# mKaloer/TFServingCache

Measured on NVIDIA H100. Metric: predict_qps, higher is better.
Workload: dtype f32

## Files before the change

### tfservingcache_b200/csrc/dense_tc.cu

```cuda
#include <cuda.h>
#include <cuda_runtime.h>

#include <atomic>
#include <cstdlib>
#include <mutex>
#include <unordered_map>

#include "kernels.h"
#include "tc_ptx.cuh"

namespace tfsc {

extern std::atomic<int64_t> g_launches_tc;
std::atomic<int64_t> g_launches_tc{0};

namespace tc {
constexpr int BK = 32;
constexpr int WG_COLS = 64;
constexpr int CONS_WG = 4;
constexpr int STRIP = WG_COLS * CONS_WG;
constexpr int SLABS = STRIP / 32;
constexpr int W_BYTES = SLABS * BK * 128;
constexpr int CONSUMERS = CONS_WG * 128;
constexpr int CONS_WARPS = CONSUMERS / 32;
constexpr int THREADS = CONSUMERS + 32;
}

template <int RP>
struct TcSmem {
  static constexpr int NS = 6;
  static constexpr int B_BYTES = 2 * RP * 128;
  static constexpr int W_TOTAL = NS * tc::W_BYTES;
  static constexpr int TOTAL = W_TOTAL + 2 * B_BYTES + 256 + 1024;
};

template <int RP>
__global__ void __launch_bounds__(tc::THREADS, 1)
dense_tc_kernel(const __grid_constant__ CUtensorMap wmap, const float* __restrict__ x, const float* __restrict__ bias,
                float* __restrict__ y, int rows, int K, int N, int relu, int splits, int chunk_k,
                unsigned int* __restrict__ counters, float* __restrict__ partials) {
  using S = TcSmem<RP>;
  constexpr int NS = S::NS;
  extern __shared__ __align__(1024) uint8_t smem_raw[];
  uint8_t* smem = reinterpret_cast<uint8_t*>((reinterpret_cast<uintptr_t>(smem_raw) + 1023) & ~(uintptr_t)1023);
  uint8_t* bprime = smem + S::W_TOTAL;
  uint64_t* bars = reinterpret_cast<uint64_t*>(bprime + 2 * S::B_BYTES);
  uint64_t* full = bars;
  uint64_t* empty = bars + NS;

  const int warp = threadIdx.x >> 5, lane = threadIdx.x & 31;
  const int wg = __shfl_sync(0xffffffffu, (int)(threadIdx.x >> 7), 0);
  const int strip = blockIdx.x, split = blockIdx.y;
  const int k_begin = split * chunk_k;
  const int k_end = min(K, k_begin + chunk_k);
  const int n_kblocks = (max(0, k_end - k_begin) + tc::BK - 1) / tc::BK;

  if (threadIdx.x == 0) {
    for (int s = 0; s < NS; ++s) {
      mbar_init(&full[s], 1);
      mbar_init(&empty[s], tc::CONS_WARPS);
    }
    asm volatile("fence.mbarrier_init.release.cluster;" ::: "memory");
    asm volatile("prefetch.tensormap [%0];" ::"l"(&wmap) : "memory");
  }
  __syncthreads();
  asm volatile("griddepcontrol.launch_dependents;" ::: "memory");

  if (wg == tc::CONS_WG) {
    for (int kb = 0; kb < n_kblocks; ++kb) {
      const int s = kb % NS, it = kb / NS;
      if (lane == 0) {
        if (it > 0) mbar_wait(&empty[s], (it - 1) & 1);
        mbar_expect_tx(&full[s], tc::W_BYTES);
#pragma unroll
        for (int g = 0; g < tc::BK / 4; ++g)
          tma_load_3d(smem + s * tc::W_BYTES + g * 4096, &wmap, &full[s], 0, k_begin + kb * tc::BK + g * 4, strip * tc::SLABS);
      }
      __syncwarp();
    }
  } else {
    const int ct = threadIdx.x;
    const int wq = warp & 3, g = lane >> 2, t = lane & 3;
    constexpr int XI = (RP * 8 + tc::CONSUMERS - 1) / tc::CONSUMERS;
    float4 xr[2][XI];
    auto load_x = [&](int kb, float4* dst) {
      const int k0 = k_begin + kb * tc::BK;
#pragma unroll
      for (int j = 0; j < XI; ++j) {
        const int idx = ct + j * tc::CONSUMERS;
        const int r = idx >> 3, c = idx & 7;
        float4 v = make_float4(0.f, 0.f, 0.f, 0.f);
        const int kk = k0 + c * 4;
        if (idx < RP * 8 && r < rows) {
          const float* src = x + (size_t)r * K + kk;
          if (kk + 3 < k_end) v = __ldg(reinterpret_cast<const float4*>(src));
          else {
            if (kk < k_end) v.x = __ldg(src);
            if (kk + 1 < k_end) v.y = __ldg(src + 1);
            if (kk + 2 < k_end) v.z = __ldg(src + 2);
          }
        }
        dst[j] = v;
      }
    };
    asm volatile("griddepcontrol.wait;" ::: "memory");
    if (n_kblocks > 0) load_x(0, xr[0]);
    if (n_kblocks > 1) load_x(1, xr[1]);
    const int n0 = wg * tc::WG_COLS + wq * 16 + g, slab = n0 >> 5, row = slab * 4 + t;
    auto w_off = [&](int n) { return (uint32_t)(row * 128 + ((((n & 31) >> 2) ^ (row & 7)) << 4) + (n & 3) * 4); };
    const uint32_t w_base = smem_u32(smem);
    const uint32_t off0 = w_off(n0), off1 = w_off(n0 + 8);
    const uint32_t bp_base = smem_u32(bprime);
    float acc_h[RP / 2], acc_s[RP / 2];
#pragma unroll
    for (int i = 0; i < RP / 2; ++i) acc_h[i] = acc_s[i] = 0.f;
    auto body = [&](int kb, float4* xcur) {
      const int s = kb % NS, it = kb / NS, cb = kb & 1;
      const uint32_t bp = bp_base + cb * S::B_BYTES;
#pragma unroll
      for (int j = 0; j < XI; ++j) {
        const int idx = ct + j * tc::CONSUMERS;
        if (idx < RP * 8) {
          const int r = idx >> 3, c = idx & 7, rl = r + RP;
          const float4 v = xcur[j];
          sts_f4(bp + (uint32_t)(((r >> 3) * 64 + (r & 7) * 8 + (c ^ (r & 7))) * 16), v);
          sts_f4(bp + (uint32_t)(((rl >> 3) * 64 + (rl & 7) * 8 + (c ^ (rl & 7))) * 16),
                 make_float4(tf32_lo(v.x), tf32_lo(v.y), tf32_lo(v.z), tf32_lo(v.w)));
        }
      }
      if (kb + 2 < n_kblocks) load_x(kb + 2, xcur);
      asm volatile("fence.proxy.async.shared::cta;" ::: "memory");
      named_bar_sync(1, tc::CONSUMERS);
      mbar_wait(&full[s], it & 1);
      const uint32_t wst = w_base + (uint32_t)(s * tc::W_BYTES);
      uint32_t hi[tc::BK / 8][4], lo[tc::BK / 8][4];
#pragma unroll
      for (int k8 = 0; k8 < tc::BK / 8; ++k8)
#pragma unroll
        for (int j = 0; j < 4; ++j) {
          const float v = lds_f32(wst + (uint32_t)((k8 * 2 + (j >> 1)) * 4096) + ((j & 1) ? off1 : off0));
          hi[k8][j] = tf32_hi_bits(v);
          lo[k8][j] = __float_as_uint(tf32_lo(v));
        }
      __syncwarp();
      if (lane == 0) mbar_arrive(&empty[s]);
      if constexpr (RP <= 32) {
        fence_regs(hi);
        fence_regs(lo);
      }
      fence_regs(acc_h);
      fence_regs(acc_s);
      wgmma_fence();
#pragma unroll
      for (int k8 = 0; k8 < tc::BK / 8; ++k8) {
        const uint64_t bh = gmma_desc_sw128(bp + k8 * 32), bl = gmma_desc_sw128(bp + RP * 128 + k8 * 32);
        wgmma_tf32_rs<RP>(acc_h, hi[k8], bh);
        wgmma_tf32_rs<RP>(acc_s, hi[k8], bl);
        wgmma_tf32_rs<RP>(acc_s, lo[k8], bh);
      }
      wgmma_commit();
      wgmma_wait_all();
      fence_regs(acc_h);
      fence_regs(acc_s);
    };
    for (int kb = 0; kb < n_kblocks; kb += 2) {
      body(kb, xr[0]);
      if (kb + 1 < n_kblocks) body(kb + 1, xr[1]);
    }
    float* my_partial = partials + ((size_t)(strip * splits + split) * RP) * tc::STRIP;
#pragma unroll
    for (int i = 0; i < RP / 2; ++i) {
      const int ncol = n0 + 8 * ((i >> 1) & 1), r = 8 * (i >> 2) + 2 * t + (i & 1);
      my_partial[(size_t)r * tc::STRIP + ncol] = acc_h[i] + acc_s[i];
    }
  }

  __shared__ unsigned int s_last;
  asm volatile("griddepcontrol.wait;" ::: "memory");
  __threadfence();
  __syncthreads();
  if (threadIdx.x == 0) {
    const unsigned int prev = atomicAdd(&counters[strip], 1u);
    s_last = (prev == (unsigned)splits - 1) ? 1u : 0u;
    if (s_last) counters[strip] = 0u;
  }
  __syncthreads();
  if (!s_last) return;
  __threadfence();
  const float* sp = partials + (size_t)strip * splits * RP * tc::STRIP;
  for (int idx = threadIdx.x; idx < rows * (tc::STRIP / 4); idx += tc::THREADS) {
    const int r = idx / (tc::STRIP / 4), c4 = idx - r * (tc::STRIP / 4);
    const int col = strip * tc::STRIP + c4 * 4;
    if (col >= N) continue;
    float4 acc = __ldcg(reinterpret_cast<const float4*>(sp + (size_t)r * tc::STRIP) + c4);
    for (int s2 = 1; s2 < splits; ++s2) {
      const float4 v = __ldcg(reinterpret_cast<const float4*>(sp + ((size_t)s2 * RP + r) * tc::STRIP) + c4);
      acc.x += v.x; acc.y += v.y; acc.z += v.z; acc.w += v.w;
    }
    const float4 bv = __ldg(reinterpret_cast<const float4*>(bias + col));
    acc.x += bv.x; acc.y += bv.y; acc.z += bv.z; acc.w += bv.w;
    if (relu) { acc.x = fmaxf(acc.x, 0.f); acc.y = fmaxf(acc.y, 0.f); acc.z = fmaxf(acc.z, 0.f); acc.w = fmaxf(acc.w, 0.f); }
    *reinterpret_cast<float4*>(y + (size_t)r * N + col) = acc;
  }
}

EncodeTiledFn tc_encode_fn() {
  static EncodeTiledFn fn = [] {
    void* p = nullptr;
    cudaDriverEntryPointQueryResult q;
    if (cudaGetDriverEntryPoint("cuTensorMapEncodeTiled", &p, cudaEnableDefault, &q) != cudaSuccess) p = nullptr;
    return reinterpret_cast<EncodeTiledFn>(p);
  }();
  return fn;
}

struct MapKey {
  const void* w;
  int k, n;
  bool operator==(const MapKey& o) const { return w == o.w && k == o.k && n == o.n; }
};
struct MapKeyHash {
  size_t operator()(const MapKey& m) const { return std::hash<const void*>()(m.w) ^ ((size_t)m.k * 1315423911u) ^ ((size_t)m.n << 20); }
};

static bool get_wmap(const float* w, int k, int n, CUtensorMap* out) {
  static std::mutex mu;
  static std::unordered_map<MapKey, CUtensorMap, MapKeyHash> cache;
  std::lock_guard<std::mutex> lk(mu);
  auto it = cache.find({w, k, n});
  if (it != cache.end()) {
    *out = it->second;
    return true;
  }
  EncodeTiledFn enc = tc_encode_fn();
  if (!enc) return false;
  CUtensorMap m;
  const cuuint64_t gdim[3] = {32, (cuuint64_t)k, (cuuint64_t)(n / 32)};
  const cuuint64_t gstride[2] = {(cuuint64_t)n * 4, 128};
  const cuuint32_t box[3] = {32, 4, (cuuint32_t)tc::SLABS};
  const cuuint32_t estr[3] = {1, 1, 1};
  CUresult r = enc(&m, CU_TENSOR_MAP_DATA_TYPE_FLOAT32, 3, const_cast<float*>(w), gdim, gstride, box, estr,
                   CU_TENSOR_MAP_INTERLEAVE_NONE, CU_TENSOR_MAP_SWIZZLE_128B, CU_TENSOR_MAP_L2_PROMOTION_L2_256B,
                   CU_TENSOR_MAP_FLOAT_OOB_FILL_NONE);
  if (r != CUDA_SUCCESS) return false;
  if (cache.size() > 4096) cache.clear();
  cache[{w, k, n}] = m;
  *out = m;
  return true;
}

struct TcPlan {
  int strips, splits, chunk_k;
};
static TcPlan plan_tc(int k, int n) {
  TcPlan p;
  p.strips = (n + tc::STRIP - 1) / tc::STRIP;
  int splits = device_sm_count() / p.strips;
  if (splits < 1) splits = 1;
  int max_splits = (k + 4 * tc::BK - 1) / (4 * tc::BK);
  if (splits > max_splits) splits = max_splits;
  if (splits < 1) splits = 1;
  int chunk = (k + splits - 1) / splits;
  chunk = (chunk + tc::BK - 1) / tc::BK * tc::BK;
  p.chunk_k = chunk;
  p.splits = (k + chunk - 1) / chunk;
  return p;
}

bool dense_tc_supported(int rows, int k, int n, const float* w, const float* x, const float* bias, const float* y) {
  return rows >= 1 && rows <= 64 && n % 32 == 0 && k % 4 == 0 && k >= 32 &&
         ((reinterpret_cast<uintptr_t>(w) & 15) == 0) && ((reinterpret_cast<uintptr_t>(x) & 15) == 0) &&
         ((reinterpret_cast<uintptr_t>(bias) & 15) == 0) && ((reinterpret_cast<uintptr_t>(y) & 15) == 0) && tc_encode_fn() != nullptr;
}

size_t dense_tc_workspace_bytes(int k, int n) {
  TcPlan p = plan_tc(k, n);
  size_t counters = ((size_t)p.strips * sizeof(unsigned int) + 255) & ~(size_t)255;
  return counters + (size_t)p.strips * p.splits * 64 * tc::STRIP * sizeof(float);
}

template <int RP>
static cudaError_t launch_tc_rp(const CUtensorMap& map, const float* x, const float* bias, float* y, int rows, int k, int n,
                                bool relu, void* workspace, const TcPlan& p, cudaStream_t s) {
  static bool attr[64] = {};
  int dev = 0;
  cudaGetDevice(&dev);
  if (!attr[dev & 63]) {
    cudaError_t e = cudaFuncSetAttribute(dense_tc_kernel<RP>, cudaFuncAttributeMaxDynamicSharedMemorySize, TcSmem<RP>::TOTAL);
    if (e != cudaSuccess) return e;
    attr[dev & 63] = true;
  }
  unsigned int* counters = static_cast<unsigned int*>(workspace);
  size_t coff = ((size_t)p.strips * sizeof(unsigned int) + 255) & ~(size_t)255;
  float* partials = reinterpret_cast<float*>(static_cast<char*>(workspace) + coff);
  static const bool pdl = [] {
    const char* e = getenv("TFSC_PDL");
    return !e || atoi(e) != 0;
  }();
  cudaLaunchConfig_t cfg = {};
  cfg.gridDim = dim3(p.strips, p.splits);
  cfg.blockDim = dim3(tc::THREADS);
  cfg.dynamicSmemBytes = TcSmem<RP>::TOTAL;
  cfg.stream = s;
  cudaLaunchAttribute at[1];
  at[0].id = cudaLaunchAttributeProgrammaticStreamSerialization;
  at[0].val.programmaticStreamSerializationAllowed = 1;
  cfg.attrs = at;
  cfg.numAttrs = pdl ? 1 : 0;
  cudaError_t e = cudaLaunchKernelEx(&cfg, dense_tc_kernel<RP>, map, x, bias, y, rows, k, n, relu ? 1 : 0, p.splits, p.chunk_k, counters,
                                     partials);
  g_launches_tc++;
  return e != cudaSuccess ? e : cudaGetLastError();
}

cudaError_t launch_dense_tc(const float* x, const float* w, const float* bias, float* y, int rows, int k, int n, bool relu,
                            void* workspace, size_t workspace_bytes, cudaStream_t s) {
  if (workspace_bytes < dense_tc_workspace_bytes(k, n)) return cudaErrorInvalidValue;
  CUtensorMap map;
  if (!get_wmap(w, k, n, &map)) return cudaErrorNotSupported;
  const TcPlan p = plan_tc(k, n);
  if (rows <= 16) return launch_tc_rp<16>(map, x, bias, y, rows, k, n, relu, workspace, p, s);
  if (rows <= 32) return launch_tc_rp<32>(map, x, bias, y, rows, k, n, relu, workspace, p, s);
  if (rows <= 48) return launch_tc_rp<48>(map, x, bias, y, rows, k, n, relu, workspace, p, s);
  return launch_tc_rp<64>(map, x, bias, y, rows, k, n, relu, workspace, p, s);
}

}
```

### tfservingcache_b200/csrc/kernels.cu

```cuda
#include "kernels.h"
#include "tc_ptx.cuh"

#include <atomic>
#include <cstdlib>

namespace tfsc {

static std::atomic<int64_t> g_launches{0};
extern std::atomic<int64_t> g_launches_tc;
extern std::atomic<int64_t> g_launches_nn;
extern std::atomic<int64_t> g_launches_cl;
int64_t kernel_launch_count() { return g_launches.load() + g_launches_tc.load() + g_launches_nn.load() + g_launches_cl.load(); }

int device_sm_count() {
  static std::atomic<int> cache[64] = {};
  int dev = 0;
  cudaGetDevice(&dev);
  int n = cache[dev & 63].load();
  if (n <= 0) {
    if (cudaDeviceGetAttribute(&n, cudaDevAttrMultiProcessorCount, dev) != cudaSuccess || n <= 0) n = 132;
    cache[dev & 63].store(n);
  }
  return n;
}

__global__ void __launch_bounds__(256) affine_kernel(const float* __restrict__ x, float* __restrict__ y, int64_t n,
                                                     const float* __restrict__ pa, const float* __restrict__ pb) {
  const float a = __ldg(pa), b = __ldg(pb);
  int64_t i = (int64_t)blockIdx.x * blockDim.x + threadIdx.x;
  const int64_t stride = (int64_t)gridDim.x * blockDim.x;
  const int64_t n4 = n >> 2;
  const bool vec = ((reinterpret_cast<uintptr_t>(x) | reinterpret_cast<uintptr_t>(y)) & 15) == 0;
  if (vec) {
    const float4* x4 = reinterpret_cast<const float4*>(x);
    float4* y4 = reinterpret_cast<float4*>(y);
    for (int64_t j = i; j < n4; j += stride) {
      float4 v = __ldg(x4 + j);
      v.x = fmaf(a, v.x, b); v.y = fmaf(a, v.y, b); v.z = fmaf(a, v.z, b); v.w = fmaf(a, v.w, b);
      y4[j] = v;
    }
    for (int64_t j = (n4 << 2) + i; j < n; j += stride) y[j] = fmaf(a, x[j], b);
  } else {
    for (int64_t j = i; j < n; j += stride) y[j] = fmaf(a, x[j], b);
  }
}

cudaError_t launch_affine(const float* x, float* y, int64_t n, const float* a, const float* b, cudaStream_t s) {
  if (n <= 0) return cudaSuccess;
  int64_t blocks = (n / 4 + 255) / 256;
  if (blocks < 1) blocks = 1;
  if (blocks > device_sm_count() * 8) blocks = device_sm_count() * 8;
  affine_kernel<<<(unsigned)blocks, 256, 0, s>>>(x, y, n, a, b);
  g_launches++;
  return cudaGetLastError();
}

constexpr int kThreads = 512;
constexpr int kColsPerThread = 8;
constexpr int kColGroups = 64;
constexpr int kStripCols = kColGroups * kColsPerThread;
constexpr int kKLanes = kThreads / kColGroups;
constexpr int kUnroll = 4;
constexpr int kMaxChunkK = 4096;

struct __align__(32) float8 { float v[8]; };

__device__ __forceinline__ float8 ld_stream(const float8* p) {
  float8 r;
  uint64_t pol;
  asm("createpolicy.fractional.L2::evict_first.b64 %0, 1.0;" : "=l"(pol));
  asm volatile("ld.global.nc.L1::no_allocate.L2::cache_hint.v4.f32 {%0,%1,%2,%3}, [%4], %5;"
               : "=f"(r.v[0]), "=f"(r.v[1]), "=f"(r.v[2]), "=f"(r.v[3])
               : "l"(p), "l"(pol));
  asm volatile("ld.global.nc.L1::no_allocate.L2::cache_hint.v4.f32 {%0,%1,%2,%3}, [%4+16], %5;"
               : "=f"(r.v[4]), "=f"(r.v[5]), "=f"(r.v[6]), "=f"(r.v[7])
               : "l"(p), "l"(pol));
  return r;
}

__device__ __forceinline__ void pdl_trigger() { asm volatile("griddepcontrol.launch_dependents;" ::: "memory"); }
__device__ __forceinline__ void pdl_wait() { asm volatile("griddepcontrol.wait;" ::: "memory"); }

template <int R, bool PDL = false>
__global__ void __launch_bounds__(kThreads, 1)
dense_stream_kernel(const float* __restrict__ x, const float* __restrict__ w, const float* __restrict__ bias,
                    float* __restrict__ y, int rows, int K, int N, int relu, int splits, int chunk_k,
                    unsigned int* __restrict__ counters, float* __restrict__ partials) {
  extern __shared__ __align__(32) float smem[];
  float* xs = smem;

  const int strip = blockIdx.x;
  const int split = blockIdx.y;
  const int tid = threadIdx.x;
  const int cg = tid % kColGroups;
  const int kl = tid / kColGroups;
  const int col0 = strip * kStripCols + cg * kColsPerThread;
  const bool col_ok = col0 < N;
  const int k_begin = split * chunk_k;
  const int k_end = min(K, k_begin + chunk_k);
  const int kc = max(0, k_end - k_begin);

  if (PDL) {
    pdl_trigger();
    pdl_wait();
  }
  for (int idx = tid; idx < kc * R; idx += kThreads) {
    const int r = idx / kc, k = idx - r * kc;
    xs[k * R + r] = (r < rows) ? __ldg(x + (size_t)r * K + k_begin + k) : 0.f;
  }
  __syncthreads();

  float acc[R][kColsPerThread];
#pragma unroll
  for (int r = 0; r < R; ++r)
#pragma unroll
    for (int c = 0; c < kColsPerThread; ++c) acc[r][c] = 0.f;

  if (col_ok) {
    const float8* wp = reinterpret_cast<const float8*>(w + (size_t)(k_begin + kl) * N + col0);
    const size_t row_stride8 = (size_t)N / 8 * kKLanes;
    int k = kl;
    for (; k + (kUnroll - 1) * kKLanes < kc; k += kUnroll * kKLanes) {
      float8 wv[kUnroll];
#pragma unroll
      for (int u = 0; u < kUnroll; ++u) wv[u] = ld_stream(wp + (size_t)u * row_stride8);
      wp += (size_t)kUnroll * row_stride8;
#pragma unroll
      for (int u = 0; u < kUnroll; ++u) {
        const float* xr = xs + (k + u * kKLanes) * R;
        float xv[R];
        if (R % 4 == 0) {
#pragma unroll
          for (int q = 0; q < R / 4; ++q) {
            const float4 t = *reinterpret_cast<const float4*>(xr + 4 * q);
            xv[4 * q + 0] = t.x; xv[4 * q + 1] = t.y; xv[4 * q + 2] = t.z; xv[4 * q + 3] = t.w;
          }
        } else if (R == 2) {
          const float2 t = *reinterpret_cast<const float2*>(xr);
          xv[0] = t.x; xv[1] = t.y;
        } else {
#pragma unroll
          for (int r = 0; r < R; ++r) xv[r] = xr[r];
        }
#pragma unroll
        for (int r = 0; r < R; ++r)
#pragma unroll
          for (int c = 0; c < kColsPerThread; ++c) acc[r][c] = fmaf(xv[r], wv[u].v[c], acc[r][c]);
      }
    }
    for (; k < kc; k += kKLanes) {
      const float8 wv = ld_stream(wp);
      wp += row_stride8;
      const float* xr = xs + k * R;
#pragma unroll
      for (int r = 0; r < R; ++r) {
        const float xv = xr[r];
#pragma unroll
        for (int c = 0; c < kColsPerThread; ++c) acc[r][c] = fmaf(xv, wv.v[c], acc[r][c]);
      }
    }
  }

  __syncthreads();
  float* red = smem;
#pragma unroll
  for (int r = 0; r < R; ++r) {
    float4* dst = reinterpret_cast<float4*>(red + ((size_t)(kl * R + r) * kStripCols) + cg * kColsPerThread);
    dst[0] = make_float4(acc[r][0], acc[r][1], acc[r][2], acc[r][3]);
    dst[1] = make_float4(acc[r][4], acc[r][5], acc[r][6], acc[r][7]);
  }
  __syncthreads();

  constexpr int kVecPerRow = kStripCols / 4;
  const float4* red4 = reinterpret_cast<const float4*>(red);
  float4* my_partial = reinterpret_cast<float4*>(partials + ((size_t)(strip * splits + split) * R) * kStripCols);
  for (int idx = tid; idx < R * kVecPerRow; idx += kThreads) {
    const int r = idx / kVecPerRow, c = idx - r * kVecPerRow;
    float4 s = red4[(size_t)(0 * R + r) * kVecPerRow + c];
#pragma unroll
    for (int l = 1; l < kKLanes; ++l) {
      const float4 t = red4[(size_t)(l * R + r) * kVecPerRow + c];
      s.x += t.x; s.y += t.y; s.z += t.z; s.w += t.w;
    }
    if (splits == 1) {
      const int col = strip * kStripCols + c * 4;
      if (r < rows && col < N) {
        const float4 bv = __ldg(reinterpret_cast<const float4*>(bias + col));
        s.x += bv.x; s.y += bv.y; s.z += bv.z; s.w += bv.w;
        if (relu) { s.x = fmaxf(s.x, 0.f); s.y = fmaxf(s.y, 0.f); s.z = fmaxf(s.z, 0.f); s.w = fmaxf(s.w, 0.f); }
        *reinterpret_cast<float4*>(y + (size_t)r * N + col) = s;
      }
    } else {
      my_partial[r * kVecPerRow + c] = s;
    }
  }
  if (splits == 1) return;

  __shared__ unsigned int s_last;
  __threadfence();
  __syncthreads();
  if (tid == 0) {
    const unsigned int prev = atomicAdd(&counters[strip], 1u);
    s_last = (prev == (unsigned)splits - 1) ? 1u : 0u;
    if (s_last) counters[strip] = 0u;
  }
  __syncthreads();
  if (!s_last) return;
  __threadfence();
  const float4* strip_partials = reinterpret_cast<const float4*>(partials + (size_t)strip * splits * R * kStripCols);
  for (int idx = tid; idx < R * kVecPerRow; idx += kThreads) {
    const int r = idx / kVecPerRow, c = idx - r * kVecPerRow;
    const int col = strip * kStripCols + c * 4;
    if (r >= rows || col >= N) continue;
    float4 s = __ldcg(strip_partials + (size_t)(0 * R + r) * kVecPerRow + c);
    for (int sp = 1; sp < splits; ++sp) {
      const float4 t = __ldcg(strip_partials + (size_t)(sp * R + r) * kVecPerRow + c);
      s.x += t.x; s.y += t.y; s.z += t.z; s.w += t.w;
    }
    const float4 bv = __ldg(reinterpret_cast<const float4*>(bias + col));
    s.x += bv.x; s.y += bv.y; s.z += bv.z; s.w += bv.w;
    if (relu) { s.x = fmaxf(s.x, 0.f); s.y = fmaxf(s.y, 0.f); s.z = fmaxf(s.z, 0.f); s.w = fmaxf(s.w, 0.f); }
    *reinterpret_cast<float4*>(y + (size_t)r * N + col) = s;
  }
}

constexpr int kBulkStageRows = 16;
constexpr int kBulkStages = 5;
constexpr int kBulkColGroups = kStripCols / 8;
constexpr int kBulkRingFloats = kBulkStages * kBulkStageRows * kStripCols;
constexpr size_t kBulkMaxSmem = 216 * 1024;

__device__ __forceinline__ void bulk_copy_g2s(void* dst, const void* src, uint32_t bytes, uint64_t* bar, uint64_t policy) {
  asm volatile(
      "cp.async.bulk.shared::cluster.global.mbarrier::complete_tx::bytes.L2::cache_hint [%0], [%1], %2, [%3], %4;" ::"r"(
          smem_u32(dst)),
      "l"(src), "r"(bytes), "r"(smem_u32(bar)), "l"(policy)
      : "memory");
}
__device__ __forceinline__ void lds_2x64(uint32_t saddr, uint64_t& lo, uint64_t& hi) {
  asm volatile("ld.shared.v2.b64 {%0,%1}, [%2];" : "=l"(lo), "=l"(hi) : "r"(saddr));
}
__device__ __forceinline__ void ffma2(uint64_t& acc, float xs, uint64_t w2) {
  float a0, a1, w0, w1;
  asm("mov.b64 {%0, %1}, %2;" : "=f"(a0), "=f"(a1) : "l"(acc));
  asm("mov.b64 {%0, %1}, %2;" : "=f"(w0), "=f"(w1) : "l"(w2));
  asm("mov.b64 %0, {%1, %2};" : "=l"(acc) : "f"(fmaf(xs, w0, a0)), "f"(fmaf(xs, w1, a1)));
}

template <int R>
__device__ __forceinline__ void bulk_row(uint64_t (&acc)[R][4], uint32_t wrow_saddr, const float* xr) {
  uint64_t w0, w1, w2, w3;
  lds_2x64(wrow_saddr, w0, w1);
  lds_2x64(wrow_saddr + (kStripCols / 2) * 4u, w2, w3);
  float xv[R];
  if (R % 4 == 0) {
#pragma unroll
    for (int q = 0; q < R / 4; ++q) {
      const float4 t = *reinterpret_cast<const float4*>(xr + 4 * q);
      xv[4 * q + 0] = t.x; xv[4 * q + 1] = t.y; xv[4 * q + 2] = t.z; xv[4 * q + 3] = t.w;
    }
  } else if (R == 2) {
    const float2 t = *reinterpret_cast<const float2*>(xr);
    xv[0] = t.x; xv[1] = t.y;
  } else {
#pragma unroll
    for (int r = 0; r < R; ++r) xv[r] = xr[r];
  }
#pragma unroll
  for (int r = 0; r < R; ++r) {
    ffma2(acc[r][0], xv[r], w0);
    ffma2(acc[r][1], xv[r], w1);
    ffma2(acc[r][2], xv[r], w2);
    ffma2(acc[r][3], xv[r], w3);
  }
}

template <int R, int KL>
__global__ void __launch_bounds__(kBulkColGroups * KL + 32, 1)
dense_bulk_kernel(const float* __restrict__ x, const float* __restrict__ w, const float* __restrict__ bias,
                  float* __restrict__ y, int rows, int K, int N, int relu, int splits, int chunk_k,
                  unsigned int* __restrict__ counters, float* __restrict__ partials) {
  constexpr int kBulkKLanes = KL, kBulkConsumers = kBulkColGroups * KL, kBulkThreads = kBulkConsumers + 32;
  extern __shared__ __align__(128) float smem_bulk[];
  float* smem = smem_bulk;
  float* ring = smem;
  float* xs = smem + kBulkRingFloats;
  __shared__ __align__(8) uint64_t full[kBulkStages];
  __shared__ __align__(8) uint64_t empty[kBulkStages];
  __shared__ unsigned int s_last;

  const int strip = blockIdx.x;
  const int split = blockIdx.y;
  const int tid = threadIdx.x;
  const int warp = tid >> 5, lane = tid & 31;
  const int k_begin = split * chunk_k;
  const int k_end = min(K, k_begin + chunk_k);
  const int kc = max(0, k_end - k_begin);
  const int strip_cols = min(kStripCols, N - strip * kStripCols);
  const int n_stage = (kc + kBulkStageRows - 1) / kBulkStageRows;

  if (tid == 0) {
#pragma unroll
    for (int s = 0; s < kBulkStages; ++s) {
      mbar_init(&full[s], 1);
      mbar_init(&empty[s], kBulkConsumers / 32);
    }
    asm volatile("fence.mbarrier_init.release.cluster;" ::: "memory");
  }
  __syncthreads();
  pdl_trigger();

  uint64_t acc[R][4];
#pragma unroll
  for (int r = 0; r < R; ++r)
#pragma unroll
    for (int c = 0; c < 4; ++c) acc[r][c] = 0ull;
  const int cg = tid % kBulkColGroups;
  const int kl = (tid / kBulkColGroups) % kBulkKLanes;

  if (warp == kBulkConsumers / 32) {
    uint64_t policy;
    asm volatile("createpolicy.fractional.L2::evict_first.b64 %0, 1.0;" : "=l"(policy));
    const uint32_t row_bytes = (uint32_t)strip_cols * 4u;
    const float* src0 = w + (size_t)k_begin * N + (size_t)strip * kStripCols;
    for (int it = 0; it < n_stage; ++it) {
      const int s = it % kBulkStages;
      if (it >= kBulkStages) mbar_wait(&empty[s], ((it / kBulkStages) - 1) & 1);
      const int rows_here = min(kBulkStageRows, kc - it * kBulkStageRows);
      if (lane == 0) mbar_expect_tx(&full[s], (uint32_t)rows_here * row_bytes);
      __syncwarp();
      if (lane < rows_here)
        bulk_copy_g2s(ring + ((size_t)s * kBulkStageRows + lane) * kStripCols,
                      src0 + (size_t)(it * kBulkStageRows + lane) * N, row_bytes, &full[s], policy);
    }
    pdl_wait();
  } else {
    pdl_wait();
    for (int idx = tid; idx < kc * R; idx += kBulkConsumers) {
      const int r = idx / kc, k = idx - r * kc;
      xs[k * R + r] = (r < rows) ? __ldg(x + (size_t)r * K + k_begin + k) : 0.f;
    }
    asm volatile("bar.sync 1, %0;" ::"r"(kBulkConsumers) : "memory");
    const uint32_t ring_s = smem_u32(ring) + (uint32_t)cg * 16u;
    for (int it = 0; it < n_stage; ++it) {
      const int s = it % kBulkStages;
      mbar_wait(&full[s], (it / kBulkStages) & 1);
      const int kk0 = it * kBulkStageRows + kl;
      const uint32_t base = ring_s + (uint32_t)((s * kBulkStageRows + kl) * kStripCols) * 4u;
      if (it * kBulkStageRows + kBulkStageRows <= kc) {
#pragma unroll
        for (int j = 0; j < kBulkStageRows / KL; ++j)
          bulk_row<R>(acc, base + (uint32_t)(j * KL * kStripCols) * 4u, xs + (size_t)(kk0 + j * KL) * R);
      } else {
#pragma unroll
        for (int j = 0; j < kBulkStageRows / KL; ++j)
          if (kk0 + j * KL < kc) bulk_row<R>(acc, base + (uint32_t)(j * KL * kStripCols) * 4u, xs + (size_t)(kk0 + j * KL) * R);
      }
      __syncwarp();
      if (lane == 0) mbar_arrive(&empty[s]);
    }
  }

  __syncthreads();
  float* red = smem;
  if (warp < kBulkConsumers / 32) {
#pragma unroll
    for (int r = 0; r < R; ++r) {
      float* dst = red + ((size_t)(kl * R + r) * kStripCols) + cg * 4;
      *reinterpret_cast<ulonglong2*>(dst) = make_ulonglong2(acc[r][0], acc[r][1]);
      *reinterpret_cast<ulonglong2*>(dst + kStripCols / 2) = make_ulonglong2(acc[r][2], acc[r][3]);
    }
  }
  __syncthreads();

  constexpr int kVecPerRow = kStripCols / 4;
  const float4* red4 = reinterpret_cast<const float4*>(red);
  float4* my_partial = reinterpret_cast<float4*>(partials + ((size_t)(strip * splits + split) * R) * kStripCols);
  for (int idx = tid; idx < R * kVecPerRow; idx += kBulkThreads) {
    const int r = idx / kVecPerRow, c = idx - r * kVecPerRow;
    float4 s = red4[(size_t)(0 * R + r) * kVecPerRow + c];
#pragma unroll
    for (int l = 1; l < kBulkKLanes; ++l) {
      const float4 t = red4[(size_t)(l * R + r) * kVecPerRow + c];
      s.x += t.x; s.y += t.y; s.z += t.z; s.w += t.w;
    }
    if (splits == 1) {
      const int col = strip * kStripCols + c * 4;
      if (r < rows && col < N) {
        const float4 bv = __ldg(reinterpret_cast<const float4*>(bias + col));
        s.x += bv.x; s.y += bv.y; s.z += bv.z; s.w += bv.w;
        if (relu) { s.x = fmaxf(s.x, 0.f); s.y = fmaxf(s.y, 0.f); s.z = fmaxf(s.z, 0.f); s.w = fmaxf(s.w, 0.f); }
        *reinterpret_cast<float4*>(y + (size_t)r * N + col) = s;
      }
    } else {
      my_partial[r * kVecPerRow + c] = s;
    }
  }
  if (splits == 1) return;

  __threadfence();
  __syncthreads();
  if (tid == 0) {
    const unsigned int prev = atomicAdd(&counters[strip], 1u);
    s_last = (prev == (unsigned)splits - 1) ? 1u : 0u;
    if (s_last) counters[strip] = 0u;
  }
  __syncthreads();
  if (!s_last) return;
  __threadfence();
  const float4* strip_partials = reinterpret_cast<const float4*>(partials + (size_t)strip * splits * R * kStripCols);
  for (int idx = tid; idx < R * kVecPerRow; idx += kBulkThreads) {
    const int r = idx / kVecPerRow, c = idx - r * kVecPerRow;
    const int col = strip * kStripCols + c * 4;
    if (r >= rows || col >= N) continue;
    float4 s = __ldcg(strip_partials + (size_t)(0 * R + r) * kVecPerRow + c);
#pragma unroll 8
    for (int sp = 1; sp < splits; ++sp) {
      const float4 t = __ldcg(strip_partials + (size_t)(sp * R + r) * kVecPerRow + c);
      s.x += t.x; s.y += t.y; s.z += t.z; s.w += t.w;
    }
    const float4 bv = __ldg(reinterpret_cast<const float4*>(bias + col));
    s.x += bv.x; s.y += bv.y; s.z += bv.z; s.w += bv.w;
    if (relu) { s.x = fmaxf(s.x, 0.f); s.y = fmaxf(s.y, 0.f); s.z = fmaxf(s.z, 0.f); s.w = fmaxf(s.w, 0.f); }
    *reinterpret_cast<float4*>(y + (size_t)r * N + col) = s;
  }
}

__global__ void __launch_bounds__(256)
dense_generic_kernel(const float* __restrict__ x, const float* __restrict__ w, const float* __restrict__ bias,
                     float* __restrict__ y, int rows, int K, int N, int relu) {
  const int n = blockIdx.x * blockDim.x + threadIdx.x;
  const int r = blockIdx.y;
  if (n >= N || r >= rows) return;
  float acc = 0.f;
  const float* xr = x + (size_t)r * K;
  for (int k = 0; k < K; ++k) acc = fmaf(__ldg(xr + k), __ldg(w + (size_t)k * N + n), acc);
  acc += __ldg(bias + n);
  if (relu) acc = fmaxf(acc, 0.f);
  y[(size_t)r * N + n] = acc;
}

struct DensePlan {
  int strips, splits, chunk_k;
};

static DensePlan plan_dense(int k, int n) {
  DensePlan p;
  p.strips = (n + kStripCols - 1) / kStripCols;
  int splits = device_sm_count() / p.strips;
  if (splits < 1) splits = 1;
  int min_splits = (k + kMaxChunkK - 1) / kMaxChunkK;
  if (splits < min_splits) splits = min_splits;
  if (splits > k / 64 && k >= 64) splits = k / 64;
  if (splits < 1) splits = 1;
  int chunk = (k + splits - 1) / splits;
  chunk = (chunk + kKLanes - 1) / kKLanes * kKLanes;
  p.chunk_k = chunk;
  p.splits = (k + chunk - 1) / chunk;
  return p;
}

static size_t stream_workspace_bytes(int k, int n) {
  DensePlan p = plan_dense(k, n);
  size_t counters = ((size_t)p.strips * sizeof(unsigned int) + 255) & ~(size_t)255;
  size_t partials = (size_t)p.strips * p.splits * kMaxRowsPerLaunch * kStripCols * sizeof(float);
  return counters + partials;
}

size_t dense_workspace_bytes(int rows, int k, int n) {
  (void)rows;
  size_t a = stream_workspace_bytes(k, n), b = dense_tc_workspace_bytes(k, n);
  return a > b ? a : b;
}

static int tc_min_rows() {
  static int v = [] {
    const char* e = getenv("TFSC_TC_MIN_ROWS");
    return e ? atoi(e) : 9;
  }();
  return v;
}

static bool pdl_enabled() {
  static bool v = [] {
    const char* e = getenv("TFSC_PDL");
    return e && atoi(e) != 0;
  }();
  return v;
}

template <typename... KArgs, typename... Args>
static cudaError_t launch_maybe_pdl(void (*kernel)(KArgs...), dim3 grid, int threads, size_t smem, cudaStream_t s, Args... args) {
  cudaLaunchConfig_t cfg = {};
  cfg.gridDim = grid;
  cfg.blockDim = dim3(threads);
  cfg.dynamicSmemBytes = smem;
  cfg.stream = s;
  cudaLaunchAttribute at[1];
  at[0].id = cudaLaunchAttributeProgrammaticStreamSerialization;
  at[0].val.programmaticStreamSerializationAllowed = 1;
  cfg.attrs = at;
  cfg.numAttrs = pdl_enabled() ? 1 : 0;
  return cudaLaunchKernelEx(&cfg, kernel, static_cast<KArgs>(args)...);
}

template <int R>
static cudaError_t launch_dense_r(const float* x, const float* w, const float* bias, float* y, int rows, int k, int n,
                                  bool relu, void* workspace, const DensePlan& p, cudaStream_t s) {
  size_t xs_bytes = (size_t)p.chunk_k * R * sizeof(float);
  size_t red_bytes = (size_t)kKLanes * R * kStripCols * sizeof(float);
  size_t smem = xs_bytes > red_bytes ? xs_bytes : red_bytes;
  static bool attr_set[64] = {};
  int dev = 0;
  cudaGetDevice(&dev);
  if (!attr_set[dev & 63]) {
    cudaError_t e = cudaFuncSetAttribute(dense_stream_kernel<R>, cudaFuncAttributeMaxDynamicSharedMemorySize, 200 * 1024);
    if (e != cudaSuccess) return e;
    attr_set[dev & 63] = true;
  }
  unsigned int* counters = static_cast<unsigned int*>(workspace);
  size_t coff = ((size_t)p.strips * sizeof(unsigned int) + 255) & ~(size_t)255;
  float* partials = reinterpret_cast<float*>(static_cast<char*>(workspace) + coff);
  dim3 grid(p.strips, p.splits);
  if (pdl_enabled()) {
    static bool attr_set_pdl[64] = {};
    if (!attr_set_pdl[dev & 63]) {
      cudaError_t e = cudaFuncSetAttribute(dense_stream_kernel<R, true>, cudaFuncAttributeMaxDynamicSharedMemorySize, 200 * 1024);
      if (e != cudaSuccess) return e;
      attr_set_pdl[dev & 63] = true;
    }
    cudaError_t le = launch_maybe_pdl(dense_stream_kernel<R, true>, grid, kThreads, smem, s, x, w, bias, y, rows, k, n, relu ? 1 : 0,
                                      p.splits, p.chunk_k, counters, partials);
    g_launches++;
    return le != cudaSuccess ? le : cudaGetLastError();
  }
  dense_stream_kernel<R><<<grid, kThreads, smem, s>>>(x, w, bias, y, rows, k, n, relu ? 1 : 0, p.splits, p.chunk_k,
                                                      counters, partials);
  g_launches++;
  return cudaGetLastError();
}

static bool bulk_fits(int R, const DensePlan& p) {
  return (size_t)kBulkRingFloats * sizeof(float) + (size_t)p.chunk_k * R * sizeof(float) <= kBulkMaxSmem;
}

template <int R, int KL>
static cudaError_t launch_dense_bulk_r(const float* x, const float* w, const float* bias, float* y, int rows, int k, int n,
                                       bool relu, void* workspace, const DensePlan& p, cudaStream_t s) {
  const size_t smem = (size_t)kBulkRingFloats * sizeof(float) + (size_t)p.chunk_k * R * sizeof(float);
  static bool attr_set[64] = {};
  int dev = 0;
  cudaGetDevice(&dev);
  if (!attr_set[dev & 63]) {
    cudaError_t e = cudaFuncSetAttribute(dense_bulk_kernel<R, KL>, cudaFuncAttributeMaxDynamicSharedMemorySize, (int)kBulkMaxSmem);
    if (e != cudaSuccess) return e;
    attr_set[dev & 63] = true;
  }
  unsigned int* counters = static_cast<unsigned int*>(workspace);
  size_t coff = ((size_t)p.strips * sizeof(unsigned int) + 255) & ~(size_t)255;
  float* partials = reinterpret_cast<float*>(static_cast<char*>(workspace) + coff);
  dim3 grid(p.strips, p.splits);
  cudaError_t le = launch_maybe_pdl(dense_bulk_kernel<R, KL>, grid, kBulkColGroups * KL + 32, smem, s, x, w, bias, y, rows, k, n,
                                    relu ? 1 : 0, p.splits, p.chunk_k, counters, partials);
  g_launches++;
  return le != cudaSuccess ? le : cudaGetLastError();
}

static int dense_variant_default() {
  static int v = [] {
    const char* e = getenv("TFSC_DENSE_VARIANT");
    return e ? atoi(e) : 0;
  }();
  return v;
}

cudaError_t launch_dense(const float* x, const float* w, const float* bias, float* y, int rows, int k, int n,
                         bool relu, void* workspace, size_t workspace_bytes, cudaStream_t s, int variant) {
  if (rows <= 0 || n <= 0) return cudaSuccess;
  if (variant == 0) variant = dense_variant_default();
  const bool stream_ok = (n % 8 == 0) && ((reinterpret_cast<uintptr_t>(w) & 31) == 0) &&
                         ((reinterpret_cast<uintptr_t>(bias) & 15) == 0) && ((reinterpret_cast<uintptr_t>(y) & 15) == 0) &&
                         k >= 1 && workspace && workspace_bytes >= dense_workspace_bytes(rows, k, n);
  if (!stream_ok) {
    for (int r0 = 0; r0 < rows; r0 += 65535) {
      int rr = rows - r0 < 65535 ? rows - r0 : 65535;
      dim3 grid((n + 255) / 256, rr);
      dense_generic_kernel<<<grid, 256, 0, s>>>(x + (size_t)r0 * k, w, bias, y + (size_t)r0 * n, rr, k, n, relu ? 1 : 0);
      g_launches++;
    }
    return cudaGetLastError();
  }
  const DensePlan p = plan_dense(k, n);
  int r_done = 0;
  const int tc_rows = variant == 3 ? 1 : tc_min_rows();
  if (variant != 1 && tc_rows > 0 && rows >= tc_rows && dense_tc_supported(rows > 64 ? 64 : rows, k, n, w, x, bias, y)) {
    while (rows - r_done >= tc_rows) {
      const int rr = rows - r_done < 64 ? rows - r_done : 64;
      cudaError_t e = launch_dense_tc(x + (size_t)r_done * k, w, bias, y + (size_t)r_done * n, rr, k, n, relu, workspace,
                                      workspace_bytes, s);
      if (e != cudaSuccess) return e;
      r_done += rr;
    }
  }
  for (int r0 = r_done; r0 < rows; r0 += kMaxRowsPerLaunch) {
    const int rr = rows - r0 < kMaxRowsPerLaunch ? rows - r0 : kMaxRowsPerLaunch;
    const float* xp = x + (size_t)r0 * k;
    float* yp = y + (size_t)r0 * n;
    cudaError_t e;
    if ((variant == 0 || variant == 5) && dense_cluster_supported(rr, k, n, w, xp, bias, yp)) {
      e = launch_dense_cluster(xp, w, bias, yp, rr, k, n, relu, s);
      if (e != cudaSuccess) return e;
      continue;
    }
    if ((variant == 2 || variant == 4) && bulk_fits(rr <= 2 ? rr : (rr <= 4 ? 4 : 8), p)) {
      if (variant == 2) {
        if (rr == 1) e = launch_dense_bulk_r<1, 8>(xp, w, bias, yp, rr, k, n, relu, workspace, p, s);
        else if (rr == 2) e = launch_dense_bulk_r<2, 8>(xp, w, bias, yp, rr, k, n, relu, workspace, p, s);
        else if (rr <= 4) e = launch_dense_bulk_r<4, 8>(xp, w, bias, yp, rr, k, n, relu, workspace, p, s);
        else e = launch_dense_bulk_r<8, 8>(xp, w, bias, yp, rr, k, n, relu, workspace, p, s);
      } else {
        if (rr == 1) e = launch_dense_bulk_r<1, 4>(xp, w, bias, yp, rr, k, n, relu, workspace, p, s);
        else if (rr == 2) e = launch_dense_bulk_r<2, 4>(xp, w, bias, yp, rr, k, n, relu, workspace, p, s);
        else if (rr <= 4) e = launch_dense_bulk_r<4, 4>(xp, w, bias, yp, rr, k, n, relu, workspace, p, s);
        else e = launch_dense_bulk_r<8, 4>(xp, w, bias, yp, rr, k, n, relu, workspace, p, s);
      }
      if (e != cudaSuccess) return e;
      continue;
    }
    if (rr == 1) e = launch_dense_r<1>(xp, w, bias, yp, rr, k, n, relu, workspace, p, s);
    else if (rr == 2) e = launch_dense_r<2>(xp, w, bias, yp, rr, k, n, relu, workspace, p, s);
    else if (rr <= 4) e = launch_dense_r<4>(xp, w, bias, yp, rr, k, n, relu, workspace, p, s);
    else e = launch_dense_r<8>(xp, w, bias, yp, rr, k, n, relu, workspace, p, s);
    if (e != cudaSuccess) return e;
  }
  return cudaSuccess;
}

}

extern "C" {
int64_t tfsc_kernel_launches(void) { return tfsc::kernel_launch_count(); }
}
```

### tfservingcache_b200/csrc/server.cu

```cuda
#include <cuda_runtime.h>

#include <chrono>
#include <cmath>
#include <map>
#include <memory>
#include <mutex>
#include <new>
#include <stdexcept>

#include "forward.h"
#include "inputs.h"
#include "json.h"
#include "kernels.h"
#include "node.h"
#include "parse.h"
#include "provider.h"
#include "ring.h"
#include "wire.h"

using namespace tfsc;

struct tfsc_server {
  Json cfg;
  std::unique_ptr<ModelProvider> provider;
  std::vector<std::unique_ptr<Node>> nodes;
  std::vector<std::string> local_members;
  std::mutex ring_mu;
  Ring ring;
  std::map<std::string, int> member_node;
  std::vector<std::string> member_list;
  std::map<std::string, int> member_rank;
  int replicas = 1;
  std::mutex pick_mu;
  std::unique_ptr<ReplicaPicker> picker;
  std::atomic<int64_t> req_rest{0}, req_grpc{0}, fail_rest{0}, fail_grpc{0};
  std::unique_ptr<Forwarder> fwd;
};

static int route(tfsc_server* s, const std::string& name, const std::string& version, std::vector<int>* nodes,
                 int* picked, std::vector<int>* ranks = nullptr) {
  std::vector<std::string> members;
  const std::string key = name + "##" + version;
  int n_members = 0;
  {
    std::lock_guard<std::mutex> lk(s->ring_mu);
    if (!s->ring.get_n(key, s->replicas < 1 ? 1 : s->replicas, &members)) return fail(TFSC_E_EMPTY_RING, "empty circle");
    n_members = s->ring.members();
    nodes->clear();
    for (auto& m : members) {
      auto it = s->member_node.find(m);
      nodes->push_back(it == s->member_node.end() ? -1 : it->second);
      if (ranks) {
        auto rt = s->member_rank.find(m);
        ranks->push_back(rt == s->member_rank.end() ? -1 : rt->second);
      }
    }
  }
  std::vector<int> ids;
  for (auto& m : members) ids.push_back((int)(crc32_ieee(m.data(), m.size()) & 0x7FFFFFFF));
  std::lock_guard<std::mutex> lk(s->pick_mu);
  *picked = s->picker->pick_ids(key, ids.data(), (int)nodes->size(), n_members);
  return (int)nodes->size();
}

static void set_members(tfsc_server* s, const std::vector<std::string>& members) {
  std::lock_guard<std::mutex> lk(s->ring_mu);
  s->ring.set(members);
  s->member_list = members;
  s->member_node.clear();
  for (size_t i = 0; i < s->local_members.size(); ++i) s->member_node[s->local_members[i]] = (int)i;
  s->member_rank.clear();
  if (s->fwd)
    for (size_t i = 0; i < members.size() && (int)i < s->fwd->world(); ++i)
      if (!s->member_node.count(members[i])) s->member_rank[members[i]] = (int)i;
}

template <typename F>
static int guarded(const char* what, F&& f) {
  try {
    return f();
  } catch (const std::bad_alloc&) {
    return fail(TFSC_E_EXHAUSTED, "%s: out of host memory", what);
  } catch (const std::length_error&) {
    return fail(TFSC_E_EXHAUSTED, "%s: request too large", what);
  } catch (const std::exception& e) {
    return fail(TFSC_E_INTERNAL, "%s: %s", what, e.what());
  } catch (...) {
    return fail(TFSC_E_INTERNAL, "%s: unknown exception", what);
  }
}

extern "C" {

static tfsc_server* server_create_impl(const char* config_json) {
  auto s = std::make_unique<tfsc_server>();
  std::string err;
  if (!config_json || !json_parse(config_json, &s->cfg, &err) || s->cfg.type != Json::Obj) {
    fail(TFSC_E_INVALID, "config: %s", err.empty() ? "expected a JSON object" : err.c_str());
    return nullptr;
  }
  int n_dev = 0;
  cudaError_t ce = cudaGetDeviceCount(&n_dev);
  if (ce != cudaSuccess || n_dev == 0) {
    cudaGetLastError();
    fail(TFSC_E_NO_DEVICE, "no CUDA device available (%s): this library has no CPU fallback",
         ce == cudaSuccess ? "device count is 0" : cudaGetErrorString(ce));
    return nullptr;
  }
  s->provider = create_provider(s->cfg, &err);
  if (!s->provider) {
    fail(TFSC_E_INVALID, "%s", err.c_str());
    return nullptr;
  }
  std::vector<int> devices;
  if (const Json* d = s->cfg.get("gpu.devices")) {
    for (auto& v : d->arr) devices.push_back((int)v.integer());
  }
  if (devices.empty())
    for (int i = 0; i < n_dev; ++i) devices.push_back(i);
  for (int d : devices) {
    cudaDeviceProp prop;
    if (d < 0 || d >= n_dev || cudaGetDeviceProperties(&prop, d) != cudaSuccess) {
      fail(TFSC_E_NO_DEVICE, "gpu.devices: device %d not present", d);
      return nullptr;
    }
    if (prop.major != 9 || prop.minor != 0) {
      fail(TFSC_E_NO_DEVICE, "device %d is sm_%d%d; this library is built for sm_90a (H100) only", d, prop.major,
           prop.minor);
      return nullptr;
    }
  }
  if (s->cfg.get_int("gpu.blockingSync", 1)) {
    for (int d : devices) {
      DeviceGuard g(d);
      if (cudaSetDeviceFlags(cudaDeviceScheduleBlockingSync) != cudaSuccess) cudaGetLastError();
    }
  }
  s->replicas = (int)std::max(s->cfg.get_num("proxy.replicasPerModel", 1), 1.0);
  const std::string policy = s->cfg.get_str("proxy.replicaPick", "random");
  if (policy != "random" && policy != "first" && policy != "hot-spread" && policy != "balanced" && policy != "hash") {
    fail(TFSC_E_INVALID, "unknown proxy.replicaPick '%s'", policy.c_str());
    return nullptr;
  }
  int64_t seed = s->cfg.get_int("proxy.seed", -1);
  s->picker = std::make_unique<ReplicaPicker>(
      policy, seed >= 0 ? (uint64_t)seed : (uint64_t)std::chrono::steady_clock::now().time_since_epoch().count(),
      s->cfg.get_num("proxy.hotFraction", 0.5));
  if (const Json* lm = s->cfg.get("gpu.localMembers"))
    for (auto& v : lm->arr) s->local_members.push_back(v.string());
  for (size_t i = 0; i < devices.size(); ++i) {
    NodeConfig nc;
    nc.device = devices[i];
    nc.host_cache_bytes = s->cfg.get_int("modelCache.size", (int64_t)1 << 40);
    nc.max_concurrent_models = (int)s->cfg.get_int("serving.maxConcurrentModels", 1 << 30);
    nc.arena_bytes = s->cfg.get_int("gpu.arenaBytes", 0);
    nc.max_batch = (int)s->cfg.get_int("gpu.maxBatch", 8);
    nc.max_request_rows = (int)s->cfg.get_int("gpu.maxRequestRows", 1024);
    nc.fetch_timeout_s = s->cfg.get_num("serving.modelFetchTimeout", 10.0);
    nc.slots = (int)s->cfg.get_int("gpu.stagingSlots", 4);
    nc.tick_us = (int)s->cfg.get_int("gpu.tickMicros", 0);
    auto node = std::make_unique<Node>(nc, s->provider.get());
    if (!node->init(&err)) {
      fail(TFSC_E_NO_DEVICE, "node %zu (device %d): %s", i, devices[i], err.c_str());
      return nullptr;
    }
    s->nodes.push_back(std::move(node));
    if (s->local_members.size() <= i) s->local_members.push_back("gpu" + std::to_string(devices[i]) + ":0:0");
  }
  for (int a : devices)
    for (int b : devices) {
      if (a == b) continue;
      int can = 0;
      if (cudaDeviceCanAccessPeer(&can, a, b) == cudaSuccess && can) {
        DeviceGuard g(a);
        cudaError_t pe = cudaDeviceEnablePeerAccess(b, 0);
        if (pe != cudaSuccess && pe != cudaErrorPeerAccessAlreadyEnabled) cudaGetLastError();
        else if (pe == cudaErrorPeerAccessAlreadyEnabled) cudaGetLastError();
      }
    }
  std::vector<std::string> members;
  if (const Json* m = s->cfg.get("gpu.members"))
    for (auto& v : m->arr) members.push_back(v.string());
  if (members.empty()) members = s->local_members;
  if (const Json* eps = s->cfg.get("cluster.endpoints")) {
    FwdConfig fc;
    for (auto& v : eps->arr) fc.endpoints.push_back(v.string());
    fc.rank = (int)s->cfg.get_int("cluster.rank", 0);
    fc.slot_bytes = (size_t)s->cfg.get_int("cluster.slotBytes", 1 << 20);
    fc.slots = (int)s->cfg.get_int("cluster.windowSlots", 128);
    fc.timeout_s = s->cfg.get_num("proxy.grpcTimeout", 10.0);
    fc.workers = (int)s->cfg.get_int("cluster.forwardWorkers", 8);
    if (fc.endpoints.size() != members.size()) {
      fail(TFSC_E_INVALID, "cluster.endpoints must list one endpoint per entry of gpu.members (%zu vs %zu)", fc.endpoints.size(),
           members.size());
      return nullptr;
    }
    s->fwd = std::make_unique<Forwarder>(fc, s->nodes[0].get());
    if (!s->fwd->init(&err)) {
      fail(TFSC_E_INVALID, "%s", err.c_str());
      return nullptr;
    }
  }
  set_members(s.get(), members);
  return s.release();
}

void tfsc_server_destroy(tfsc_server* s) { delete s; }
int tfsc_server_num_nodes(const tfsc_server* s) { return s ? (int)s->nodes.size() : 0; }

int tfsc_server_set_members(tfsc_server* s, const char* const* members, int n) {
  if (!s || n < 0) return fail(TFSC_E_INVALID, "set_members: bad arguments");
  std::vector<std::string> v;
  for (int i = 0; i < n; ++i) v.emplace_back(members[i]);
  set_members(s, v);
  return n;
}

int tfsc_route(tfsc_server* s, const char* model_name, const char* version, int* nodes, int cap, int* picked) {
  if (!s || !model_name || !version) return fail(TFSC_E_INVALID, "route: bad arguments");
  std::vector<int> v;
  int p = 0;
  int rc = route(s, model_name, version, &v, &p);
  if (rc < 0) return rc;
  for (int i = 0; i < rc && i < cap; ++i) nodes[i] = v[i];
  if (picked) *picked = p;
  return rc;
}

static int check_device_early() {
  int n = 0;
  if (cudaGetDeviceCount(&n) != cudaSuccess || n == 0) {
    cudaGetLastError();
    return fail(TFSC_E_NO_DEVICE, "no CUDA device available: this library has no CPU fallback");
  }
  return 0;
}

static Node* node_at(tfsc_server* s, int node) {
  if (!s || node < 0 || node >= (int)s->nodes.size()) {
    fail(TFSC_E_INVALID, "node index %d out of range", node);
    return nullptr;
  }
  return s->nodes[node].get();
}

int tfsc_model_ensure(tfsc_server* s, int node, const char* model_name, int64_t version) {
  Node* n = node_at(s, node);
  if (!n || !model_name) return TFSC_E_INVALID;
  std::string err;
  int rc = n->fetch({model_name, version}, nullptr, &err);
  if (rc < 0) return fail(rc, "%s", err.c_str());
  return rc;
}

int tfsc_model_ensure_async(tfsc_server* s, int node, const char* model_name, int64_t version) {
  Node* n = node_at(s, node);
  if (!n || !model_name) return TFSC_E_INVALID;
  std::string err;
  std::shared_ptr<DeviceModel> dm;
  int rc = n->fetch({model_name, version}, &dm, &err);
  if (rc < 0) return fail(rc, "%s", err.c_str());
  n->unpin(dm);
  return rc;
}

int tfsc_model_status(tfsc_server* s, int node, const char* model_name, int64_t version) {
  Node* n = node_at(s, node);
  if (!n || !model_name) return TFSC_E_INVALID;
  return n->status({model_name, version});
}

int tfsc_resident_list(tfsc_server* s, int node, char* buf, size_t cap) {
  Node* n = node_at(s, node);
  if (!n) return TFSC_E_INVALID;
  std::string l = n->resident_lines();
  int rc = copy_out(l, buf, cap);
  if (rc < 0) return rc;
  int c = 0;
  for (char ch : l) c += ch == '\n';
  return c;
}

int tfsc_host_list(tfsc_server* s, int node, char* buf, size_t cap) {
  Node* n = node_at(s, node);
  if (!n) return TFSC_E_INVALID;
  std::string l = n->host_lines();
  int rc = copy_out(l, buf, cap);
  if (rc < 0) return rc;
  int c = 0;
  for (char ch : l) c += ch == '\n';
  return c;
}

static int resolve(tfsc_server* s, const std::string& name, const std::string& version, Node** node, ModelId* id,
                   int* remote = nullptr) {
  std::vector<int> nodes, ranks;
  int picked = 0;
  int rc = route(s, name, version, &nodes, &picked, &ranks);
  if (rc < 0) return rc;
  int local = nodes[picked];
  if (remote) *remote = -1;
  if (local < 0) {
    if (!remote || ranks[picked] < 0)
      return fail(TFSC_E_NOT_FOUND, "owner of %s##%s is not a GPU of this process", name.c_str(), version.c_str());
    *remote = ranks[picked];
  }
  int64_t v;
  if (!parse_int64(version, &v))
    return fail(TFSC_E_INVALID, "strconv.ParseInt: parsing \"%s\": invalid syntax", version.c_str());
  *node = local >= 0 ? s->nodes[local].get() : nullptr;
  *id = {name, v};
  return 0;
}

static int run_predict(tfsc_server* s, Node* node, int remote, const ModelId& id, const std::vector<InTensor>& ts,
                       const InputLayout& l, const Node::OutAllocFn& alloc, std::string* err, int64_t deadline_ns = 0) {
  if (node) return node->predict_host(id, ts, l, alloc, nullptr, nullptr, err, deadline_ns);
  return s->fwd->forward(remote, id.name, id.version, ts, l, alloc, nullptr, deadline_ns, err);
}
static int run_predict_one(tfsc_server* s, Node* node, int remote, const ModelId& id, const void* x, int64_t n, int dtype,
                           const Node::OutAllocFn& alloc, std::string* err, int64_t deadline_ns = 0) {
  std::vector<InTensor> ts(1);
  ts[0].dtype = dtype;
  ts[0].data = x;
  ts[0].n = n;
  const InputLayout l = layout_inputs(&ts);
  return run_predict(s, node, remote, id, ts, l, alloc, err, deadline_ns);
}

static int abi_inputs(const tfsc_tensor* in, int n_in, bool need_data, std::vector<InTensor>* ts, InputLayout* l) {
  for (int i = 0; i < n_in; ++i) {
    const tfsc_tensor& x = in[i];
    if ((x.dtype != TFSC_DT_FLOAT && x.dtype != TFSC_DT_INT32) || x.rank < 0 || x.rank > 8)
      return fail(TFSC_E_INVALID, "predict: input must be DT_FLOAT or DT_INT32, rank <= 8");
    if (n_in > 1 && !x.name) return fail(TFSC_E_INVALID, "predict: every input needs a name when n_in > 1 (got %d inputs)", n_in);
    InTensor t;
    t.name = x.name ? x.name : "";
    t.dtype = x.dtype;
    t.data = x.data;
    t.shape.assign(x.shape, x.shape + x.rank);
    int64_t n = 1;
    for (auto d : t.shape) {
      if (d < 0 || (d != 0 && n > ((int64_t)1 << 40) / d)) return fail(TFSC_E_INVALID, "predict: bad input shape");
      n *= d;
    }
    if ((size_t)n * 4 != x.nbytes || (need_data && !x.data)) return fail(TFSC_E_INVALID, "predict: input nbytes does not match shape");
    t.n = x.data ? n : 0;
    ts->push_back(std::move(t));
  }
  *l = layout_inputs(ts);
  return 0;
}

static bool out_shape(const ModelDesc& d, int64_t rows, const std::vector<int64_t>& in_shape, std::vector<int64_t>* shape,
                      std::string* why) {
  shape->clear();
  int64_t per_row = 1;
  if (d.tmpl == Template::Affine) {
    *shape = in_shape;
  } else if (d.tmpl == Template::Graph) {
    if (in_shape.size() > d.input_shape.size())
      for (size_t i = 0; i + d.input_shape.size() < in_shape.size(); ++i) shape->push_back(in_shape[i]);
    for (auto v : d.output_shape) shape->push_back(v);
    per_row = d.out_dim;
  } else {
    if (in_shape.size() <= 1) {
      if (rows != 1 || in_shape.empty()) shape->push_back(rows);
    } else {
      for (size_t i = 0; i + 1 < in_shape.size(); ++i) shape->push_back(in_shape[i]);
    }
    shape->push_back(d.out_dim);
    per_row = d.out_dim;
  }
  int64_t on = 1;
  for (auto v : *shape) {
    if (v < 0 || (v != 0 && on > ((int64_t)1 << 40) / v)) {
      on = -1;
      break;
    }
    on *= v;
  }
  if (on != rows * per_row) {
    std::string sh = "[";
    for (size_t i = 0; i < in_shape.size(); ++i) sh += (i ? "," : "") + std::to_string(in_shape[i]);
    *why = "input shape " + sh + "] does not match the model signature: the trailing dimensions must hold exactly " +
           std::to_string(d.tmpl == Template::Affine ? 1 : d.in_dim) + " elements per row";
    return false;
  }
  return true;
}


struct OutputPlan {
  std::vector<ModelOutput> sel;
  std::vector<std::vector<int64_t>> shapes;
  int64_t out_dim = 0, rows = 0;
};

static int64_t product(const std::vector<int64_t>& v) {
  int64_t n = 1;
  for (auto x : v) n *= x;
  return n;
}

static bool batch_dims(const ModelDesc& d, int64_t rows, const std::vector<int64_t>& in_shape, std::vector<int64_t>* dims,
                       std::string* why) {
  dims->clear();
  if (d.tmpl == Template::Graph) {
    if (in_shape.size() > d.input_shape.size())
      for (size_t i = 0; i + d.input_shape.size() < in_shape.size(); ++i) dims->push_back(in_shape[i]);
  } else if (in_shape.size() <= 1) {
    if (rows != 1 || in_shape.empty()) dims->push_back(rows);
  } else {
    for (size_t i = 0; i + 1 < in_shape.size(); ++i) dims->push_back(in_shape[i]);
  }
  int64_t on = 1;
  for (auto v : *dims) {
    if (v < 0 || (v != 0 && on > ((int64_t)1 << 40) / v)) return false;
    on *= v;
  }
  if (on != rows) {
    std::string sh = "[";
    for (size_t i = 0; i < in_shape.size(); ++i) sh += (i ? "," : "") + std::to_string(in_shape[i]);
    *why = "input shape " + sh + "] does not match the model signature: the trailing dimensions must hold exactly " +
           std::to_string(d.in_dim) + " elements per row";
    return false;
  }
  return true;
}

static bool plan_outputs(const ModelDesc& d, int64_t rows, const std::vector<int64_t>& in_shape, const std::vector<std::string>& names,
                         OutputPlan* p, std::string* why) {
  std::vector<int64_t> dims;
  if (!batch_dims(d, rows, in_shape, &dims, why)) return false;
  p->sel.clear();
  p->shapes.clear();
  p->out_dim = d.out_dim;
  p->rows = rows;
  std::vector<std::string> want = names;
  if (want.empty())
    for (auto& o : d.outputs) want.push_back(o.name);
  for (size_t i = 0; i < want.size(); ++i) {
    const ModelOutput* o = d.output(want[i]);
    for (size_t j = 0; o && j < i; ++j)
      if (want[j] == want[i]) {
        *why = "output '" + want[i] + "' is requested twice; model outputs: " + expected_outputs(d);
        return false;
      }
    if (!o) {
      *why = "unknown output '" + want[i] + "'; model outputs: " + expected_outputs(d);
      return false;
    }
    p->sel.push_back(*o);
    std::vector<int64_t> sh = dims;
    const OutputForm f = output_form(o->kind, d.head_n, d.head_k);
    for (int r = 0; r < f.rank; ++r) sh.push_back(f.dims[r]);
    p->shapes.push_back(sh);
  }
  return true;
}

static void split_output(const OutputPlan& p, size_t i, const void* packed, void* dst) {
  const ModelOutput& o = p.sel[i];
  const char* src = static_cast<const char*>(packed);
  char* out = static_cast<char*>(dst);
  for (int64_t r = 0; r < p.rows; ++r)
    memcpy(out + (size_t)(r * o.width) * 4, src + (size_t)(r * p.out_dim + o.offset) * 4, (size_t)o.width * 4);
}

static std::string dtype_name(int dt) { return dt == TFSC_DT_INT64 ? "DT_INT64" : dt == TFSC_DT_INT32 ? "DT_INT32" : "DT_FLOAT"; }

static void* abi_outputs_alloc(const ModelDesc& d, int64_t rows, const std::vector<int64_t>& in_shape, const tfsc_tensor* out,
                               int n_out, OutputPlan* plan, std::vector<float>* packed, std::string* bad) {
  std::vector<std::string> names;
  for (int i = 0; i < n_out; ++i) {
    if (!out[i].name) {
      *bad = "predict: the model has several outputs, every out[i].name must name one of " + expected_outputs(d);
      return nullptr;
    }
    names.push_back(out[i].name);
  }
  if (!plan_outputs(d, rows, in_shape, names, plan, bad)) return nullptr;
  for (size_t i = 0; i < plan->sel.size(); ++i)
    if (!out[i].data || out[i].nbytes < (size_t)(rows * plan->sel[i].width) * 4 || plan->shapes[i].size() > 8) return nullptr;
  packed->assign((size_t)(rows * d.out_dim), 0.f);
  return packed->data();
}

static void abi_outputs_deliver(const OutputPlan& plan, const void* packed, tfsc_tensor* out) {
  for (size_t i = 0; i < plan.sel.size(); ++i) {
    split_output(plan, i, packed, out[i].data);
    out[i].dtype = output_dtype(plan.sel[i].kind);
    out[i].rank = (int32_t)plan.shapes[i].size();
    for (size_t j = 0; j < plan.shapes[i].size(); ++j) out[i].shape[j] = plan.shapes[i][j];
    out[i].nbytes = (size_t)(plan.rows * plan.sel[i].width) * 4;
  }
}

static int resolve_member(tfsc_server* s, int member, const std::string& name, const std::string& version, Node** node,
                          ModelId* id, int* remote) {
  std::string m;
  {
    std::lock_guard<std::mutex> lk(s->ring_mu);
    if (member < 0 || member >= (int)s->member_list.size()) return fail(TFSC_E_INVALID, "member index %d out of range", member);
    m = s->member_list[member];
    auto it = s->member_node.find(m);
    *node = it == s->member_node.end() ? nullptr : s->nodes[it->second].get();
    auto rt = s->member_rank.find(m);
    *remote = rt == s->member_rank.end() ? -1 : rt->second;
  }
  if (!*node && *remote < 0) return fail(TFSC_E_NOT_FOUND, "member %s is not served by this process and has no cluster endpoint", m.c_str());
  int64_t v;
  if (!parse_int64(version, &v)) return fail(TFSC_E_INVALID, "strconv.ParseInt: parsing \"%s\": invalid syntax", version.c_str());
  *id = {name, v};
  return 0;
}

static int predict_impl(tfsc_server* s, const char* model_name, const char* version, const tfsc_tensor* in, int n_in,
                        tfsc_tensor* out, int n_out, int64_t deadline_ns, int member = -1) {
  if (!s || !model_name || !version || !in || n_in < 1 || !out || n_out < 1)
    return fail(TFSC_E_INVALID, "predict: bad arguments");
  Node* node;
  ModelId id;
  int remote = -1;
  int rc = member >= 0 ? resolve_member(s, member, model_name, version, &node, &id, &remote)
                       : resolve(s, model_name, version, &node, &id, &remote);
  if (rc < 0) return rc;
  std::vector<InTensor> ts;
  InputLayout layout;
  if ((rc = abi_inputs(in, n_in, false, &ts, &layout)) < 0) return rc;
  const tfsc_tensor& x = in[0];
  const std::vector<int64_t>& ishape = ts[0].shape;
  std::string err, bad;
  tfsc_tensor* o = &out[0];
  OutputPlan plan;
  std::vector<float> packed;
  auto alloc = [&](const ModelDesc& d, int64_t rows) -> void* {
    if (d.inputs.empty() && x.name && d.input_name != x.name) {
      bad = "input '" + std::string(x.name) + "' does not match the model signature (expects '" + d.input_name + "')";
      return nullptr;
    }
    if (!d.outputs.empty()) return abi_outputs_alloc(d, rows, ishape, out, n_out, &plan, &packed, &bad);
    std::vector<int64_t> sh;
    if (!out_shape(d, rows, ishape, &sh, &bad)) return nullptr;
    int64_t on = 1;
    for (auto v : sh) on *= v;
    if (!o->data || o->nbytes < (size_t)on * 4 || sh.size() > 8) return nullptr;
    o->dtype = TFSC_DT_FLOAT;
    o->rank = (int32_t)sh.size();
    for (size_t i = 0; i < sh.size(); ++i) o->shape[i] = sh[i];
    o->nbytes = (size_t)on * 4;
    return o->data;
  };
  rc = run_predict(s, node, remote, id, ts, layout, alloc, &err, deadline_ns);
  if (rc < 0 && !bad.empty()) return fail(TFSC_E_INVALID, "%s", bad.c_str());
  if (rc < 0) return fail(rc, "%s", err.c_str());
  abi_outputs_deliver(plan, packed.data(), out);
  return 0;
}

static void set_resp_bytes(const std::string& body, void** resp, size_t* resp_len);

static int grpc_predict_impl(tfsc_server* s, const void* req, size_t req_len, void** resp, size_t* resp_len) {
  if (!s || !req || !resp || !resp_len) return fail(TFSC_E_INVALID, "grpc_predict: bad arguments");
  s->req_grpc++;
  PredictRequestView view;
  std::string err;
  if (!decode_predict_request(req, req_len, &view, &err)) {
    s->fail_grpc++;
    return fail(TFSC_E_INVALID, "%s", err.c_str());
  }
  const std::string version = std::to_string(view.version);
  Node* node;
  ModelId id;
  int remote = -1;
  int rc = resolve(s, view.model_name, version, &node, &id, &remote);
  if (rc < 0) {
    s->fail_grpc++;
    return rc;
  }
  if (view.inputs.empty()) {
    rc = node ? node->fetch(id, nullptr, &err) : 0;
    s->fail_grpc++;
    if (rc < 0) return fail(rc, "%s", err.c_str());
    return fail(TFSC_E_INVALID, "PredictRequest has no inputs");
  }
  const size_t n_in = view.inputs.size();
  std::vector<InTensor> ts(n_in);
  std::vector<std::vector<float>> scratch(n_in);
  std::vector<std::vector<int32_t>> iscratch(n_in);
  bool input_ok = true;
  for (size_t i = 0; i < n_in && input_ok; ++i) {
    const TensorView& v = view.inputs[i];
    ts[i].name = v.name;
    ts[i].shape = v.shape;
    if (v.dtype == TFSC_DT_INT32) {
      const int32_t* ip = nullptr;
      input_ok = tensor_i32(v, &ip, &ts[i].n, &iscratch[i], &err);
      ts[i].data = ip;
      ts[i].dtype = TFSC_DT_INT32;
    } else {
      const float* fp = nullptr;
      input_ok = tensor_f32(v, &fp, &ts[i].n, &scratch[i], &err);
      ts[i].data = fp;
      ts[i].dtype = TFSC_DT_FLOAT;
    }
  }
  const InputLayout layout = layout_inputs(&ts);
  const TensorView& tv = view.inputs[0];
  char* buf = nullptr;
  size_t total = 0;
  std::string bad_sig;
  OutputPlan plan;
  std::vector<float> packed;
  auto alloc = [&](const ModelDesc& d, int64_t rows) -> void* {
    if (d.inputs.empty() && (n_in != 1 || tv.name != d.input_name)) {
      bad_sig = "input keys do not match the model signature (expects '" + d.input_name + "')";
      return nullptr;
    }
    if (!d.outputs.empty()) {
      std::set<std::string> sel;
      for (auto& a : view.output_filter) {
        if (!d.output(a)) {
          std::string set;
          for (auto& o : d.outputs) set += (set.empty() ? "" : ",") + o.name;
          bad_sig = "output tensor alias not found in signature: " + a + " Outputs expected to be in the set {" + set + "}.";
          return nullptr;
        }
        if (!sel.insert(a).second) {
          bad_sig = "duplicate output tensor alias: " + a;
          return nullptr;
        }
      }
      if (!plan_outputs(d, rows, ts[0].shape, std::vector<std::string>(sel.begin(), sel.end()), &plan, &bad_sig)) return nullptr;
      packed.assign((size_t)(rows * d.out_dim), 0.f);
      return packed.data();
    }
    std::vector<int64_t> sh;
    if (!out_shape(d, rows, ts[0].shape, &sh, &bad_sig)) return nullptr;
    std::string prefix, suffix;
    predict_response_frame(view.model_name, id.version, view.signature_name.empty() ? "serving_default" : view.signature_name,
                           d.output_name, sh, &prefix, &suffix);
    int64_t on = 1;
    for (auto v : sh) on *= v;
    total = prefix.size() + (size_t)on * 4 + suffix.size();
    buf = (char*)malloc(total ? total : 1);
    if (!buf) return nullptr;
    memcpy(buf, prefix.data(), prefix.size());
    memcpy(buf + prefix.size() + (size_t)on * 4, suffix.data(), suffix.size());
    return buf + prefix.size();
  };
  if (!input_ok) {
    std::string e2;
    rc = node ? node->fetch(id, nullptr, &e2) : 0;
    s->fail_grpc++;
    if (rc < 0) return fail(rc, "%s", e2.c_str());
    return fail(TFSC_E_INVALID, "%s", err.c_str());
  }
  rc = run_predict(s, node, remote, id, ts, layout, alloc, &err);
  if (rc < 0) {
    free(buf);
    s->fail_grpc++;
    if (!bad_sig.empty()) return fail(TFSC_E_INVALID, "%s", bad_sig.c_str());
    return fail(rc, "%s", err.c_str());
  }
  if (!plan.sel.empty()) {
    std::vector<std::vector<char>> vals(plan.sel.size());
    std::vector<OutTensor> outs(plan.sel.size());
    for (size_t i = 0; i < plan.sel.size(); ++i) {
      vals[i].resize((size_t)(plan.rows * plan.sel[i].width) * 4);
      split_output(plan, i, packed.data(), vals[i].data());
      outs[i].name = plan.sel[i].name;
      outs[i].dtype = output_dtype(plan.sel[i].kind);
      outs[i].shape = plan.shapes[i];
      outs[i].data = vals[i].data();
      outs[i].n = product(plan.shapes[i]);
    }
    set_resp_bytes(encode_predict_response(view.model_name, id.version,
                                           view.signature_name.empty() ? "serving_default" : view.signature_name, outs),
                   resp, resp_len);
    return 0;
  }
  *resp = buf;
  *resp_len = total;
  return 0;
}

static void set_resp_bytes(const std::string& body, void** resp, size_t* resp_len) {
  char* b = (char*)malloc(body.size() + 1);
  memcpy(b, body.data(), body.size());
  b[body.size()] = 0;
  *resp = b;
  *resp_len = body.size();
}

static int run_examples(tfsc_server* s, const ExampleRequestView& view, int method, std::vector<float>* scores, int64_t* n_out,
                        int64_t* per_out, ModelId* id_out, std::string* sig_out, std::string* err, int* code) {
  const std::string version = std::to_string(view.version);
  Node* node;
  ModelId id;
  int remote = -1;
  int rc = resolve(s, view.model_name, version, &node, &id, &remote);
  if (rc < 0) {
    *err = tfsc_last_error();
    return rc;
  }
  if (!node) {
    *err = "model " + view.model_name + " is owned by rank " + std::to_string(remote) + "; Classify / Regress are served by the owner";
    return TFSC_E_NOT_FOUND;
  }
  ModelDesc d;
  rc = node->describe(id, &d, nullptr, err);
  if (rc < 0) return rc;
  if (!d.inputs.empty()) {
    *err = std::string(method == 1 ? "Classify" : "Regress") + " serves single-input models; " + view.model_name + " has inputs " +
           expected_inputs(d) + " (use Predict)";
    return TFSC_E_INVALID;
  }
  if (!d.outputs.empty()) {
    *err = std::string(method == 1 ? "Classify" : "Regress") + " serves single-output models; " + view.model_name + " has outputs " +
           expected_outputs(d) + " (use Predict)";
    return TFSC_E_INVALID;
  }
  const std::string want = view.signature_name.empty() ? "serving_default" : view.signature_name;
  const ExtraSignature* sg = nullptr;
  for (auto& e : d.extra_sigs)
    if (e.name == want) sg = &e;
  const char* mname = method == 1 ? "tensorflow/serving/classify" : "tensorflow/serving/regress";
  if (!sg) {
    if (want == "serving_default")
      *err = std::string("Expected ") + (method == 1 ? "classification" : "regression") + " signature method_name to be " + mname +
             ". Was: tensorflow/serving/predict";
    else
      *err = "Serving signature name: \"" + want + "\" not found in signature def";
    return TFSC_E_INVALID;
  }
  if (sg->method != method) {
    *err = std::string("Expected ") + (method == 1 ? "classification" : "regression") + " signature method_name to be " + mname +
           ". Was: " + (sg->method == 1 ? "tensorflow/serving/classify" : "tensorflow/serving/regress");
    return TFSC_E_INVALID;
  }
  if (view.examples.empty()) {
    *err = "Input is empty";
    return TFSC_E_INVALID;
  }
  const int64_t per_row = d.tmpl == Template::Affine ? 1 : d.in_dim;
  if (d.input_dtype != TFSC_DT_FLOAT) {
    *err = "the model's input is not a float tensor: no tf.Example signature";
    return TFSC_E_INVALID;
  }
  std::vector<float> x;
  x.reserve((size_t)view.examples.size() * per_row);
  for (size_t i = 0; i < view.examples.size(); ++i) {
    const std::vector<float>* f = view.examples[i].find(sg->feature);
    if (!f || (int64_t)f->size() != per_row) {
      *err = "example " + std::to_string(i) + ": feature '" + sg->feature + "' must hold " + std::to_string(per_row) +
             " float value(s), found " + (f ? std::to_string(f->size()) : std::string("none"));
      return TFSC_E_INVALID;
    }
    x.insert(x.end(), f->begin(), f->end());
  }
  const int64_t n = (int64_t)view.examples.size();
  const int64_t per = d.tmpl == Template::Affine ? 1 : d.out_dim;
  if (method == 2 && per != 1) {
    *err = "Expected output Tensor shape to be either [batch_size] or [batch_size, 1] but got [" + std::to_string(n) + "," +
           std::to_string(per) + "]";
    return TFSC_E_INVALID;
  }
  scores->assign((size_t)(n * per), 0.f);
  auto alloc = [&](const ModelDesc&, int64_t rows) -> void* { return rows == n ? scores->data() : nullptr; };
  rc = node->predict_host(id, x.data(), (int64_t)x.size(), TFSC_DT_FLOAT, alloc, nullptr, nullptr, err);
  if (rc < 0) return rc;
  *n_out = n;
  *per_out = per;
  *id_out = id;
  *sig_out = want;
  (void)code;
  return 0;
}

static int grpc_examples_impl(tfsc_server* s, int method, const void* req, size_t req_len, void** resp, size_t* resp_len) {
  if (!s || !req || !resp || !resp_len) return fail(TFSC_E_INVALID, "grpc_classify/regress: bad arguments");
  s->req_grpc++;
  ExampleRequestView view;
  std::string err;
  if (!decode_example_request(req, req_len, &view, &err)) {
    s->fail_grpc++;
    return fail(TFSC_E_INVALID, "%s", err.c_str());
  }
  std::vector<float> scores;
  int64_t n = 0, per = 0;
  ModelId id;
  std::string sig;
  int rc = run_examples(s, view, method, &scores, &n, &per, &id, &sig, &err, nullptr);
  if (rc < 0) {
    s->fail_grpc++;
    return fail(rc, "%s", err.c_str());
  }
  const std::string out = method == 1 ? encode_classification_response(view.model_name, id.version, sig, scores.data(), n, per)
                                      : encode_regression_response(view.model_name, id.version, sig, scores.data(), n);
  set_resp_bytes(out, resp, resp_len);
  return 0;
}

static int grpc_session_run_impl(tfsc_server* s, const void* req, size_t req_len, void** resp, size_t* resp_len) {
  if (!s || !req || !resp || !resp_len) return fail(TFSC_E_INVALID, "grpc_session_run: bad arguments");
  s->req_grpc++;
  SessionRunView view;
  std::string err;
  if (!decode_session_run_request(req, req_len, &view, &err)) {
    s->fail_grpc++;
    return fail(TFSC_E_INVALID, "%s", err.c_str());
  }
  Node* node;
  ModelId id;
  int remote = -1;
  int rc = resolve(s, view.model_name, std::to_string(view.version), &node, &id, &remote);
  if (rc < 0) {
    s->fail_grpc++;
    return rc;
  }
  auto strip = [](const std::string& t) { return t.size() > 2 && t.compare(t.size() - 2, 2, ":0") == 0 ? t.substr(0, t.size() - 2) : t; };
  if (view.feeds.size() != 1 || view.fetch.size() != 1 || !view.target.empty()) {
    ModelDesc d;
    const bool known = node && node->describe(id, &d, nullptr, &err) >= 0;
    s->fail_grpc++;
    if (known && !d.inputs.empty())
      return fail(TFSC_E_INVALID, "SessionRun serves single-input models; %s has inputs %s (use Predict)", view.model_name.c_str(),
                  expected_inputs(d).c_str());
    return fail(TFSC_E_INVALID, "SessionRun on a model template takes exactly one feed (the signature input) and one fetch (its output)");
  }
  const TensorView& tv = view.feeds[0];
  const void* xdata = nullptr;
  int64_t n = 0;
  std::vector<float> scratch;
  std::vector<int32_t> iscratch;
  bool ok;
  if (tv.dtype == TFSC_DT_INT32) {
    const int32_t* ip = nullptr;
    ok = tensor_i32(tv, &ip, &n, &iscratch, &err);
    xdata = ip;
  } else {
    const float* fp = nullptr;
    ok = tensor_f32(tv, &fp, &n, &scratch, &err);
    xdata = fp;
  }
  if (!ok) {
    s->fail_grpc++;
    return fail(TFSC_E_INVALID, "%s", err.c_str());
  }
  char* buf = nullptr;
  size_t total = 0;
  std::string bad;
  OutputPlan plan;
  std::vector<float> packed;
  auto alloc = [&](const ModelDesc& d, int64_t rows) -> void* {
    if (!d.outputs.empty()) {
      if (strip(tv.name) != d.input_name || !d.output(strip(view.fetch[0]))) {
        bad = "feed / fetch do not name the model's tensors (feed '" + d.input_name + ":0', fetch one of " + expected_outputs(d) + ")";
        return nullptr;
      }
      if (!plan_outputs(d, rows, tv.shape, {strip(view.fetch[0])}, &plan, &bad)) return nullptr;
      packed.assign((size_t)(rows * d.out_dim), 0.f);
      return packed.data();
    }
    if (strip(tv.name) != d.input_name || strip(view.fetch[0]) != d.output_name) {
      bad = "feed / fetch do not name the model's tensors (feed '" + d.input_name + ":0', fetch '" + d.output_name + ":0')";
      return nullptr;
    }
    std::vector<int64_t> sh;
    if (!out_shape(d, rows, tv.shape, &sh, &bad)) return nullptr;
    std::string prefix, suffix;
    session_run_response_frame(view.model_name, id.version, view.signature_name, view.fetch[0], sh, &prefix, &suffix);
    int64_t on = 1;
    for (auto v : sh) on *= v;
    total = prefix.size() + (size_t)on * 4 + suffix.size();
    buf = (char*)malloc(total ? total : 1);
    if (!buf) return nullptr;
    memcpy(buf, prefix.data(), prefix.size());
    memcpy(buf + prefix.size() + (size_t)on * 4, suffix.data(), suffix.size());
    return buf + prefix.size();
  };
  rc = run_predict_one(s, node, remote, id, xdata, n, tv.dtype == TFSC_DT_INT32 ? TFSC_DT_INT32 : TFSC_DT_FLOAT, alloc, &err);
  if (rc < 0) {
    free(buf);
    s->fail_grpc++;
    if (!bad.empty()) return fail(TFSC_E_INVALID, "%s", bad.c_str());
    return fail(rc, "%s", err.c_str());
  }
  if (!plan.sel.empty()) {
    std::vector<char> vals((size_t)(plan.rows * plan.sel[0].width) * 4);
    split_output(plan, 0, packed.data(), vals.data());
    OutTensor t;
    t.name = view.fetch[0];
    t.dtype = output_dtype(plan.sel[0].kind);
    t.shape = plan.shapes[0];
    t.data = vals.data();
    t.n = product(plan.shapes[0]);
    set_resp_bytes(encode_session_run_response(view.model_name, id.version, view.signature_name, t), resp, resp_len);
    return 0;
  }
  *resp = buf;
  *resp_len = total;
  return 0;
}

static const char* state_name(int st) {
  switch (st) {
    case TFSC_STATE_START: return "START";
    case TFSC_STATE_LOADING: return "LOADING";
    case TFSC_STATE_AVAILABLE: return "AVAILABLE";
    case TFSC_STATE_UNLOADING: return "UNLOADING";
    case TFSC_STATE_END: return "END";
    default: return "UNKNOWN";
  }
}

static int http_for(int rc) {
  switch (rc) {
    case TFSC_E_INVALID: return 400;
    case TFSC_E_NOT_FOUND: return 404;
    case TFSC_E_TIMEOUT: return 504;
    case TFSC_E_EXHAUSTED: return 507;
    case TFSC_E_EMPTY_RING: return 503;
    default: return 500;
  }
}

static void set_resp(const std::string& body, void** resp, size_t* resp_len) {
  char* b = (char*)malloc(body.size() + 1);
  memcpy(b, body.data(), body.size());
  b[body.size()] = 0;
  *resp = b;
  *resp_len = body.size();
}

static std::string error_json(const std::string& msg) {
  std::string s = "{ \"error\": ";
  json_escape(msg, &s);
  s += " }";
  return s;
}

static bool flatten(const Json& j, size_t depth, std::vector<int64_t>* shape, std::vector<float>* out, std::string* err) {
  if (j.type == Json::Num) {
    if (shape->size() > depth) {
      *err = "ragged tensor";
      return false;
    }
    out->push_back((float)j.num);
    return true;
  }
  if (j.type != Json::Arr) {
    *err = "tensor values must be numbers or nested arrays of numbers";
    return false;
  }
  if (shape->size() == depth) shape->push_back((int64_t)j.arr.size());
  else if ((*shape)[depth] != (int64_t)j.arr.size()) {
    *err = "ragged tensor";
    return false;
  }
  for (auto& e : j.arr)
    if (!flatten(e, depth + 1, shape, out, err)) return false;
  return true;
}

static void write_tensor_json(const float* v, const std::vector<int64_t>& shape, size_t dim, size_t* idx, std::string* s) {
  if (dim == shape.size()) {
    json_float(v[(*idx)++], s);
    return;
  }
  *s += "[";
  for (int64_t i = 0; i < shape[dim]; ++i) {
    if (i) *s += ", ";
    write_tensor_json(v, shape, dim + 1, idx, s);
  }
  *s += "]";
}

static void json_word_value(OutputKind k, const uint32_t* w, std::string* s) {
  const int dt = output_dtype(k);
  if (dt == TFSC_DT_INT64) {
    *s += std::to_string((int64_t)((uint64_t)w[0] | ((uint64_t)w[1] << 32)));
  } else if (dt == TFSC_DT_INT32) {
    *s += std::to_string((int32_t)w[0]);
  } else {
    float f;
    memcpy(&f, w, 4);
    json_float(f, s);
  }
}

static void json_nested(OutputKind k, const uint32_t* w, const std::vector<int64_t>& dims, size_t dim, int64_t* idx, int step,
                        std::string* s) {
  if (dim == dims.size()) {
    json_word_value(k, w + *idx * step, s);
    ++*idx;
    return;
  }
  *s += "[";
  for (int64_t i = 0; i < dims[dim]; ++i) {
    if (i) *s += ", ";
    json_nested(k, w, dims, dim + 1, idx, step, s);
  }
  *s += "]";
}

static std::string rest_multi_output_json(const OutputPlan& p, const float* packed, bool row_format) {
  const uint32_t* words = reinterpret_cast<const uint32_t*>(packed);
  std::string b = std::string("{\n    \"") + (row_format ? "predictions" : "outputs") + "\": " + (row_format ? "[" : "{");
  if (row_format) {
    for (int64_t r = 0; r < p.rows; ++r) {
      b += r ? ", {" : "{";
      for (size_t i = 0; i < p.sel.size(); ++i) {
        const ModelOutput& o = p.sel[i];
        if (i) b += ", ";
        json_escape(o.name, &b);
        b += ": ";
        const uint32_t* w = words + r * p.out_dim + o.offset;
        const size_t rank = (size_t)output_form(o.kind, 0, 0).rank;
        if (rank == 0) {
          json_word_value(o.kind, w, &b);
        } else {
          const std::vector<int64_t>& sh = p.shapes[i];
          int64_t idx = 0;
          json_nested(o.kind, w, std::vector<int64_t>(sh.end() - (ptrdiff_t)rank, sh.end()), 0, &idx, 1, &b);
        }
      }
      b += "}";
    }
    b += "]\n}";
    return b;
  }
  for (size_t i = 0; i < p.sel.size(); ++i) {
    const ModelOutput& o = p.sel[i];
    std::vector<uint32_t> vals((size_t)(p.rows * o.width));
    split_output(p, i, packed, vals.data());
    if (i) b += ", ";
    json_escape(o.name, &b);
    b += ": ";
    int64_t idx = 0;
    json_nested(o.kind, vals.data(), p.shapes[i], 0, &idx, output_dtype(o.kind) == TFSC_DT_INT64 ? 2 : 1, &b);
  }
  b += "}\n}";
  return b;
}

static int rest_handle_impl(tfsc_server* s, const char* method, const char* url, const void* body, size_t body_len,
                            int* http_status, void** resp, size_t* resp_len) {
  if (!s || !method || !url || !http_status || !resp || !resp_len) return fail(TFSC_E_INVALID, "rest_handle: bad arguments");
  s->req_rest++;
  std::string name, version;
  const std::string u(url);
  int st = match_rest_url(u, &name, &version);
  if (st != 200) {
    s->fail_rest++;
    *http_status = st;
    set_resp(rest_error_body(st), resp, resp_len);
    return 0;
  }
  size_t vpos = u.find(version, u.find('/', 11));
  std::string tail = u.substr(vpos + version.size());
  size_t qpos = tail.find('?');
  if (qpos != std::string::npos) tail.resize(qpos);
  Node* node;
  ModelId id;
  int remote = -1;
  int rc = resolve(s, name, version, &node, &id, &remote);
  auto fail_http = [&](int code, const std::string& msg) {
    s->fail_rest++;
    *http_status = code;
    set_resp(error_json(msg), resp, resp_len);
    return 0;
  };
  if (rc < 0) return fail_http(http_for(rc), tfsc_last_error());
  std::string err;
  const std::string m(method);
  if (!node && !(m == "POST" && tail == ":predict"))
    return fail_http(404, "model " + name + " is owned by rank " + std::to_string(remote) + "; ask that rank for " + tail);
  if (m == "GET" && (tail.empty() || tail == "/")) {
    rc = node->fetch(id, nullptr, &err);
    if (rc < 0) return fail_http(http_for(rc), err);
    int stt = node->status(id);
    std::string b = "{\n \"model_version_status\": [\n  {\n   \"version\": \"" + std::to_string(id.version) +
                    "\",\n   \"state\": \"" + state_name(stt) +
                    "\",\n   \"status\": {\n    \"error_code\": \"OK\",\n    \"error_message\": \"\"\n   }\n  }\n ]\n}\n";
    *http_status = 200;
    set_resp(b, resp, resp_len);
    return 0;
  }
  if (m == "POST" && tail == ":predict") {
    Json req;
    bool parsed = json_parse(std::string((const char*)body, body_len), &req, &err) && req.type == Json::Obj;
    const Json* instances = parsed ? req.get("instances") : nullptr;
    const Json* inputs = parsed ? req.get("inputs") : nullptr;
    std::vector<int64_t> shape;
    std::vector<float> flat;
    std::string input_key;
    std::vector<std::pair<std::string, Json>> columns;
    bool ok = parsed && ((instances != nullptr) != (inputs != nullptr));
    if (parsed && !ok) err = "JSON body must contain exactly one of 'instances' (row format) or 'inputs' (columnar)";
    if (ok && instances && instances->type == Json::Arr && !instances->arr.empty() && instances->arr[0].type == Json::Obj &&
        instances->arr[0].obj.size() > 1) {
      for (auto& kv : instances->arr[0].obj) {
        columns.emplace_back(kv.first, Json());
        columns.back().second.type = Json::Arr;
      }
      for (auto& inst : instances->arr) {
        if (inst.type != Json::Obj || inst.obj.size() != columns.size()) {
          ok = false;
          err = "every instance object must name the same inputs";
          break;
        }
        for (auto& col : columns) {
          const Json* v = inst.get(col.first);
          if (!v) {
            ok = false;
            err = "every instance object must name the same inputs (one lacks '" + col.first + "')";
            break;
          }
          col.second.arr.push_back(*v);
        }
        if (!ok) break;
      }
    } else if (ok && inputs && inputs->type == Json::Obj && inputs->obj.size() > 1) {
      for (auto& kv : inputs->obj) columns.emplace_back(kv.first, kv.second);
    } else if (ok && instances) {
      const Json* src = instances;
      Json unwrapped;
      if (instances->type == Json::Arr && !instances->arr.empty() && instances->arr[0].type == Json::Obj) {
        unwrapped.type = Json::Arr;
        for (auto& inst : instances->arr) {
          if (inst.type != Json::Obj || inst.obj.size() != 1) {
            ok = false;
            err = "each instance object must name exactly one input";
            break;
          }
          input_key = inst.obj[0].first;
          unwrapped.arr.push_back(inst.obj[0].second);
        }
        src = &unwrapped;
      }
      if (ok) ok = flatten(*src, 0, &shape, &flat, &err);
    } else if (ok) {
      const Json* src = inputs;
      if (inputs->type == Json::Obj) {
        if (inputs->obj.size() != 1) {
          ok = false;
          err = "'inputs' object must name exactly one input";
        } else {
          input_key = inputs->obj[0].first;
          src = &inputs->obj[0].second;
        }
      }
      if (ok) ok = flatten(*src, 0, &shape, &flat, &err);
    }
    std::vector<std::vector<int64_t>> col_shape(columns.size());
    std::vector<std::vector<int32_t>> col_ints(columns.size());
    for (size_t i = 0; ok && i < columns.size(); ++i) {
      std::vector<float> vals;
      ok = flatten(columns[i].second, 0, &col_shape[i], &vals, &err);
      if (ok && vals.empty()) {
        ok = false;
        err = "input '" + columns[i].first + "' is empty";
      }
      col_ints[i].resize(vals.size());
      for (size_t k = 0; k < vals.size(); ++k) col_ints[i][k] = (int32_t)llround((double)vals[k]);
    }
    if (!ok || (flat.empty() && columns.empty())) {
      std::string e2;
      rc = node ? node->fetch(id, nullptr, &e2) : 0;
      if (rc < 0) return fail_http(http_for(rc), e2);
      return fail_http(400, err.empty() ? "empty request" : err);
    }
    std::vector<float> y;
    std::vector<int64_t> oshape;
    std::string bad_sig;
    OutputPlan plan;
    std::vector<InTensor> ts(columns.size());
    for (size_t i = 0; i < columns.size(); ++i) {
      ts[i].name = columns[i].first;
      ts[i].dtype = TFSC_DT_INT32;
      ts[i].data = col_ints[i].data();
      ts[i].shape = col_shape[i];
      ts[i].n = (int64_t)col_ints[i].size();
    }
    const InputLayout layout = layout_inputs(&ts);
    if (!ts.empty()) shape = ts[0].shape;
    auto alloc = [&](const ModelDesc& d, int64_t rows) -> void* {
      if (d.inputs.empty() && !input_key.empty() && input_key != d.input_name) {
        bad_sig = "input '" + input_key + "' does not match the model signature (expects '" + d.input_name + "')";
        return nullptr;
      }
      if (!d.outputs.empty()) {
        if (!plan_outputs(d, rows, shape, {}, &plan, &bad_sig)) return nullptr;
        y.assign((size_t)(rows * d.out_dim), 0.f);
        return y.data();
      }
      if (!out_shape(d, rows, shape, &oshape, &bad_sig)) return nullptr;
      int64_t on = 1;
      for (auto v : oshape) on *= v;
      y.resize((size_t)on);
      return y.data();
    };
    if (!ts.empty()) rc = run_predict(s, node, remote, id, ts, layout, alloc, &err);
    else rc = run_predict_one(s, node, remote, id, flat.data(), (int64_t)flat.size(), TFSC_DT_FLOAT, alloc, &err);
    if (ts.empty() && rc == TFSC_E_INVALID && err.find("input dtype") == 0) {
      std::vector<int32_t> ints(flat.size());
      for (size_t i = 0; i < flat.size(); ++i) ints[i] = (int32_t)llround((double)flat[i]);
      err.clear();
      rc = run_predict_one(s, node, remote, id, ints.data(), (int64_t)ints.size(), TFSC_DT_INT32, alloc, &err);
    }
    if (rc < 0) return fail_http(bad_sig.empty() ? http_for(rc) : 400, bad_sig.empty() ? err : bad_sig);
    if (!plan.sel.empty()) {
      *http_status = 200;
      set_resp(rest_multi_output_json(plan, y.data(), instances != nullptr), resp, resp_len);
      return 0;
    }
    std::string b = std::string("{\n    \"") + (instances ? "predictions" : "outputs") + "\": ";
    size_t idx = 0;
    if (oshape.empty()) {
      json_float(y[0], &b);
      b += "\n}";
    } else {
      std::string t;
      write_tensor_json(y.data(), oshape, 0, &idx, &t);
      t.pop_back();
      b += t + "\n    ]\n}";
    }
    *http_status = 200;
    set_resp(b, resp, resp_len);
    return 0;
  }
  if (m == "GET" && tail == "/metadata") {
    ModelDesc d;
    rc = node->describe(id, &d, nullptr, &err);
    if (rc < 0) return fail_http(http_for(rc), err);
    std::string dim = d.tmpl == Template::Affine ? "" : std::to_string(d.in_dim);
    std::string odim = d.tmpl == Template::Affine ? "" : std::to_string(d.out_dim);
    auto tensor_info = [](const std::string& key, const std::vector<std::string>& dims, const char* dtype) {
      std::string t = "\"" + key + "\": {\"dtype\": \"" + dtype + "\", \"tensor_shape\": {\"dim\": [{\"size\": \"-1\", \"name\": \"\"}";
      for (auto& dim : dims) t += ", {\"size\": \"" + dim + "\", \"name\": \"\"}";
      t += "], \"unknown_rank\": false}, \"name\": \"" + key + ":0\"}";
      return t;
    };
    std::string ins;
    for (auto& mi : d.inputs)
      ins += (ins.empty() ? "" : ", ") + tensor_info(mi.name, {std::to_string(d.in_dim / (int64_t)d.inputs.size())}, "DT_INT32");
    if (d.inputs.empty())
      ins = tensor_info(d.input_name, dim.empty() ? std::vector<std::string>{} : std::vector<std::string>{dim},
                        d.input_dtype == TFSC_DT_INT32 ? "DT_INT32" : "DT_FLOAT");
    std::string outs;
    for (auto& mo : d.outputs) {
      const OutputForm f = output_form(mo.kind, d.head_n, d.head_k);
      std::vector<std::string> dims;
      for (int r = 0; r < f.rank; ++r) dims.push_back(std::to_string(f.dims[r]));
      outs += (outs.empty() ? "" : ", ") + tensor_info(mo.name, dims, dtype_name(f.dtype).c_str());
    }
    if (d.outputs.empty())
      outs = tensor_info(d.output_name, odim.empty() ? std::vector<std::string>{} : std::vector<std::string>{odim}, "DT_FLOAT");
    std::string b = "{\n\"model_spec\": {\"name\": ";
    json_escape(name, &b);
    b += ", \"signature_name\": \"\", \"version\": \"" + std::to_string(id.version) + "\"},\n\"metadata\": {\"signature_def\": {\"signature_def\": {\"serving_default\": {\"inputs\": {" +
         ins + "}, \"outputs\": {" + outs + "}, \"method_name\": \"tensorflow/serving/predict\"}}}}\n}\n";
    *http_status = 200;
    set_resp(b, resp, resp_len);
    return 0;
  }
  if (m == "POST" && (tail == ":classify" || tail == ":regress")) {
    const int method = tail == ":classify" ? 1 : 2;
    Json req;
    bool parsed = json_parse(std::string((const char*)body, body_len), &req, &err) && req.type == Json::Obj;
    const Json* examples = parsed ? req.get("examples") : nullptr;
    if (!parsed || !examples || examples->type != Json::Arr) {
      std::string e2;
      rc = node->fetch(id, nullptr, &e2);
      if (rc < 0) return fail_http(http_for(rc), e2);
      return fail_http(400, parsed ? "JSON body must contain an 'examples' list" : err);
    }
    ExampleRequestView view;
    view.model_name = name;
    view.version = id.version;
    view.has_version = true;
    view.signature_name = req.get_str("signature_name", "");
    auto add_features = [&](const Json& obj, ExampleView* ex) {
      if (obj.type != Json::Obj) return false;
      for (auto& kv : obj.obj) {
        std::vector<float> vals;
        if (kv.second.type == Json::Num) vals.push_back((float)kv.second.num);
        else if (kv.second.type == Json::Arr) {
          for (auto& e : kv.second.arr)
            if (e.type == Json::Num) vals.push_back((float)e.num);
            else return false;
        } else continue;
        if (!ex->find(kv.first)) ex->features.emplace_back(kv.first, vals);
      }
      return true;
    };
    bool ok = true;
    for (auto& e : examples->arr) {
      ExampleView ex;
      ok = ok && add_features(e, &ex);
      if (const Json* ctx = req.get("context")) ok = ok && add_features(*ctx, &ex);
      view.examples.push_back(std::move(ex));
    }
    if (!ok) return fail_http(400, "examples must be objects mapping feature names to numbers or lists of numbers");
    std::vector<float> scores;
    int64_t n = 0, per = 0;
    ModelId rid;
    std::string sig;
    rc = run_examples(s, view, method, &scores, &n, &per, &rid, &sig, &err, nullptr);
    if (rc < 0) return fail_http(rc == TFSC_E_INVALID ? 400 : http_for(rc), err);
    std::string b = "{\n    \"results\": [";
    for (int64_t i = 0; i < n; ++i) {
      if (i) b += ", ";
      if (method == 2) {
        json_float(scores[(size_t)i], &b);
      } else {
        b += "[";
        for (int64_t k = 0; k < per; ++k) {
          if (k) b += ", ";
          b += "[\"\", ";
          json_float(scores[(size_t)(i * per + k)], &b);
          b += "]";
        }
        b += "]";
      }
    }
    b += "]\n}";
    *http_status = 200;
    set_resp(b, resp, resp_len);
    return 0;
  }
  return fail_http(400, "Malformed request: " + m + " " + u);
}

tfsc_server* tfsc_server_create(const char* config_json) {
  tfsc_server* out = nullptr;
  guarded("server_create", [&] {
    out = server_create_impl(config_json);
    return 0;
  });
  return out;
}
int tfsc_predict(tfsc_server* s, const char* model_name, const char* version, const tfsc_tensor* in, int n_in,
                 tfsc_tensor* out, int n_out) {
  return guarded("predict", [&] { return predict_impl(s, model_name, version, in, n_in, out, n_out, 0); });
}
int tfsc_predict_deadline(tfsc_server* s, const char* model_name, const char* version, const tfsc_tensor* in, int n_in,
                          tfsc_tensor* out, int n_out, int64_t deadline_ns) {
  return guarded("predict", [&] { return predict_impl(s, model_name, version, in, n_in, out, n_out, deadline_ns); });
}
int tfsc_predict_member(tfsc_server* s, int member, const char* model_name, const char* version, const tfsc_tensor* in, int n_in,
                        tfsc_tensor* out, int n_out, int64_t deadline_ns) {
  return guarded("predict", [&] { return predict_impl(s, model_name, version, in, n_in, out, n_out, deadline_ns, member); });
}
int64_t tfsc_now_ns(void) { return Node::now_ns(); }
int tfsc_grpc_predict(tfsc_server* s, const void* req, size_t req_len, void** resp, size_t* resp_len) {
  return guarded("grpc_predict", [&] { return grpc_predict_impl(s, req, req_len, resp, resp_len); });
}
int tfsc_grpc_classify(tfsc_server* s, const void* req, size_t req_len, void** resp, size_t* resp_len) {
  return guarded("grpc_classify", [&] { return grpc_examples_impl(s, 1, req, req_len, resp, resp_len); });
}
int tfsc_grpc_regress(tfsc_server* s, const void* req, size_t req_len, void** resp, size_t* resp_len) {
  return guarded("grpc_regress", [&] { return grpc_examples_impl(s, 2, req, req_len, resp, resp_len); });
}
int tfsc_grpc_session_run(tfsc_server* s, const void* req, size_t req_len, void** resp, size_t* resp_len) {
  return guarded("grpc_session_run", [&] { return grpc_session_run_impl(s, req, req_len, resp, resp_len); });
}
int tfsc_rest_handle(tfsc_server* s, const char* method, const char* url, const void* body, size_t body_len,
                     int* http_status, void** resp, size_t* resp_len) {
  return guarded("rest_handle", [&] { return rest_handle_impl(s, method, url, body, body_len, http_status, resp, resp_len); });
}

struct tfsc_ticket {
  tfsc_server* srv = nullptr;
  Node* node = nullptr;
  PredictRequest req;
  char* staging = nullptr;
  size_t staging_bytes = 0, in_al = 0, out_bytes = 0;
  tfsc_tensor* out = nullptr;
  int n_out = 0;
  std::vector<int64_t> oshape;
  OutputPlan plan;
  std::vector<float> packed;
  std::thread remote_thread;
  std::mutex mu;
  std::condition_variable cv;
  int remote_rc = 1;
  std::string remote_err;
  std::vector<std::vector<char>> remote_x;
  std::vector<InTensor> remote_ts;
  InputLayout remote_l;
  bool delivered = false;
};

static int submit_impl(tfsc_server* s, const char* model_name, const char* version, const tfsc_tensor* in, int n_in,
                       tfsc_tensor* out, int n_out, int64_t deadline_ns, tfsc_ticket** ticket) {
  if (!s || !model_name || !version || !in || n_in < 1 || !out || n_out < 1 || !ticket)
    return fail(TFSC_E_INVALID, "predict_submit: bad arguments");
  *ticket = nullptr;
  Node* node;
  ModelId id;
  int remote = -1;
  int rc = resolve(s, model_name, version, &node, &id, &remote);
  if (rc < 0) return rc;
  std::vector<InTensor> ts;
  InputLayout layout;
  if ((rc = abi_inputs(in, n_in, true, &ts, &layout)) < 0) return rc;
  const tfsc_tensor& x = in[0];
  const std::vector<int64_t> ishape = ts[0].shape;
  auto t = std::make_unique<tfsc_ticket>();
  t->srv = s;
  t->node = node;
  t->out = &out[0];
  t->n_out = n_out;
  std::string err;
  if (!node) {
    for (auto& c : ts) {
      const char* p = static_cast<const char*>(c.data);
      t->remote_x.emplace_back(p, p + (size_t)c.n * 4);
      c.data = t->remote_x.back().data();
    }
    t->remote_ts = ts;
    t->remote_l = layout;
    tfsc_ticket* tp = t.get();
    const std::string xname = x.name ? x.name : "";
    const bool has_name = x.name != nullptr;
    t->remote_thread = std::thread([tp, s, remote, id, ishape, xname, has_name, deadline_ns] {
      std::string e2, bad;
      auto alloc = [&](const ModelDesc& d, int64_t rows) -> void* {
        if (d.inputs.empty() && has_name && d.input_name != xname) {
          bad = "input '" + xname + "' does not match the model signature (expects '" + d.input_name + "')";
          return nullptr;
        }
        if (!d.outputs.empty()) {
          void* y = abi_outputs_alloc(d, rows, ishape, tp->out, tp->n_out, &tp->plan, &tp->packed, &bad);
          tp->out_bytes = tp->packed.size() * 4;
          return y;
        }
        if (!out_shape(d, rows, ishape, &tp->oshape, &bad)) return nullptr;
        int64_t on = 1;
        for (auto v : tp->oshape) on *= v;
        if (!tp->out->data || tp->out->nbytes < (size_t)on * 4 || tp->oshape.size() > 8) return nullptr;
        tp->out_bytes = (size_t)on * 4;
        return tp->out->data;
      };
      int r = s->fwd->forward(remote, id.name, id.version, tp->remote_ts, tp->remote_l, alloc, nullptr, deadline_ns, &e2);
      std::lock_guard<std::mutex> lk(tp->mu);
      tp->remote_rc = r < 0 && !bad.empty() ? TFSC_E_INVALID : r;
      tp->remote_err = !bad.empty() ? bad : e2;
      tp->cv.notify_all();
    });
    *ticket = t.release();
    return 0;
  }
  rc = node->prepare(id, layout, &t->req, nullptr, &err);
  if (rc < 0) return fail(rc, "%s", err.c_str());
  const ModelDesc& d = t->req.dm->desc;
  std::string bad;
  if (d.inputs.empty() && x.name && d.input_name != x.name)
    bad = "input '" + std::string(x.name) + "' does not match the model signature (expects '" + d.input_name + "')";
  bool buffers_ok = true;
  if (bad.empty() && !d.outputs.empty()) {
    buffers_ok = abi_outputs_alloc(d, t->req.rows, ishape, out, n_out, &t->plan, &t->packed, &bad) != nullptr;
  } else if (bad.empty()) {
    out_shape(d, t->req.rows, ishape, &t->oshape, &bad);
  }
  if (!bad.empty()) {
    node->abandon(&t->req);
    return fail(TFSC_E_INVALID, "%s", bad.c_str());
  }
  int64_t on = 1;
  for (auto v : t->oshape) on *= v;
  t->out_bytes = d.outputs.empty() ? (size_t)on * 4 : t->packed.size() * 4;
  if (d.outputs.empty() ? (!out[0].data || out[0].nbytes < t->out_bytes || t->oshape.size() > 8) : !buffers_ok) {
    node->abandon(&t->req);
    return fail(TFSC_E_BUFFER, "output buffer too small");
  }
  t->in_al = ((size_t)layout.n_elems * 4 + 255) & ~(size_t)255;
  t->staging_bytes = t->in_al + t->out_bytes;
  t->staging = static_cast<char*>(node->staging_alloc(t->staging_bytes));
  if (!t->staging) {
    node->abandon(&t->req);
    return fail(TFSC_E_EXHAUSTED, "cannot pin %zu bytes of request staging", t->staging_bytes);
  }
  pack_rows(ts, layout, t->req.rows, t->staging);
  t->req.x = t->staging;
  t->req.y = t->staging + t->in_al;
  t->req.host_staged = true;
  t->req.deadline_ns = deadline_ns;
  node->enqueue(&t->req);
  *ticket = t.release();
  return 0;
}

static int wait_impl(tfsc_ticket* t, int64_t timeout_ns) {
  if (!t) return fail(TFSC_E_INVALID, "predict_wait: null ticket");
  int rc;
  std::string err;
  if (!t->node) {
    std::unique_lock<std::mutex> lk(t->mu);
    auto pred = [&] { return t->remote_rc != 1; };
    if (timeout_ns < 0) t->cv.wait(lk, pred);
    else if (!t->cv.wait_for(lk, std::chrono::nanoseconds(timeout_ns), pred))
      return fail(TFSC_E_TIMEOUT, "predict_wait: request still in flight");
    rc = t->remote_rc;
    err = t->remote_err;
  } else {
    std::unique_lock<std::mutex> lk(t->req.mu);
    auto pred = [&] { return t->req.rc != 1; };
    if (timeout_ns < 0) t->req.cv.wait(lk, pred);
    else if (!t->req.cv.wait_for(lk, std::chrono::nanoseconds(timeout_ns), pred))
      return fail(TFSC_E_TIMEOUT, "predict_wait: request still in flight");
    rc = t->req.rc;
    err = t->req.err;
    if (rc == 0 && !t->delivered)
      memcpy(t->plan.sel.empty() ? t->out->data : (void*)t->packed.data(), t->staging + t->in_al, t->out_bytes);
  }
  if (rc < 0) return fail(rc, "%s", err.c_str());
  if (!t->delivered && !t->plan.sel.empty()) {
    abi_outputs_deliver(t->plan, t->packed.data(), t->out);
    t->delivered = true;
  }
  if (!t->delivered) {
    t->out->dtype = TFSC_DT_FLOAT;
    t->out->rank = (int32_t)t->oshape.size();
    for (size_t i = 0; i < t->oshape.size(); ++i) t->out->shape[i] = t->oshape[i];
    t->out->nbytes = t->out_bytes;
    t->delivered = true;
  }
  return 0;
}

int tfsc_predict_submit(tfsc_server* s, const char* model_name, const char* version, const tfsc_tensor* in, int n_in,
                        tfsc_tensor* out, int n_out, int64_t deadline_ns, tfsc_ticket** ticket) {
  return guarded("predict_submit", [&] { return submit_impl(s, model_name, version, in, n_in, out, n_out, deadline_ns, ticket); });
}
int tfsc_predict_wait(tfsc_ticket* t, int64_t timeout_ns) {
  return guarded("predict_wait", [&] { return wait_impl(t, timeout_ns); });
}
void tfsc_predict_release(tfsc_ticket* t) {
  if (!t) return;
  if (t->node) {
    {
      std::unique_lock<std::mutex> lk(t->req.mu);
      t->req.cv.wait(lk, [&] { return t->req.rc != 1; });
    }
    t->node->staging_free(t->staging, t->staging_bytes);
  } else if (t->remote_thread.joinable()) {
    t->remote_thread.join();
  }
  delete t;
}

int tfsc_fwd_window(tfsc_server* s, void** dev_ptr, size_t* bytes, size_t* slot_bytes) {
  if (!s || !s->fwd) return fail(TFSC_E_INVALID, "fwd_window: the server has no cluster.endpoints");
  if (dev_ptr) *dev_ptr = s->fwd->window();
  if (bytes) *bytes = s->fwd->window_bytes();
  if (slot_bytes) *slot_bytes = s->fwd->slot_bytes();
  return s->fwd->rank();
}
int tfsc_device_memcpy(void* dst, const void* src, size_t nbytes) {
  cudaError_t e = cudaMemcpy(dst, src, nbytes, cudaMemcpyDefault);
  if (e != cudaSuccess) {
    cudaGetLastError();
    return fail(TFSC_E_INTERNAL, "device_memcpy: %s", cudaGetErrorString(e));
  }
  return 0;
}
int tfsc_fwd_peer_window(tfsc_server* s, int peer_rank, void** dev_ptr, size_t* bytes) {
  if (!s || !s->fwd || !dev_ptr) return fail(TFSC_E_INVALID, "fwd_peer_window: bad arguments / no cluster.endpoints");
  return guarded("fwd_peer_window", [&] {
    std::string err;
    char* p = s->fwd->peer_window(peer_rank, bytes, &err);
    if (!p) return fail(TFSC_E_INTERNAL, "%s", err.c_str());
    *dev_ptr = p;
    return 0;
  });
}

int tfsc_predict_device(tfsc_server* s, int node, const char* model_name, int64_t version, const void* x,
                        int64_t rows, void* y, void* stream) {
  Node* n = node_at(s, node);
  if (!n || !model_name) return TFSC_E_INVALID;
  std::string err;
  int rc = n->predict_device({model_name, version}, x, rows, y, (cudaStream_t)stream, &err);
  if (rc < 0) return fail(rc, "%s", err.c_str());
  return 0;
}

int tfsc_node_set_max_resident(tfsc_server* s, int node, int max_concurrent_models) {
  Node* n = node_at(s, node);
  if (!n) return TFSC_E_INVALID;
  if (max_concurrent_models < 1) return fail(TFSC_E_INVALID, "serving.maxConcurrentModels must be >= 1");
  n->set_max_concurrent_models(max_concurrent_models);
  return 0;
}

int tfsc_k_copy_segments(const tfsc_copy_seg* segs, int n, void* stream) {
  if (int rc = check_device_early()) return rc;
  if (!segs || n < 0) return fail(TFSC_E_INVALID, "copy_segments: bad arguments");
  static_assert(sizeof(tfsc_copy_seg) == sizeof(CopySeg), "ABI struct mirrors the kernel's segment");
  cudaError_t e = launch_copy_segments(reinterpret_cast<const CopySeg*>(segs), n, (cudaStream_t)stream);
  return e == cudaSuccess ? 0 : fail(TFSC_E_INTERNAL, "copy_segments: %s", cudaGetErrorString(e));
}

int tfsc_node_sync(tfsc_server* s, int node) {
  Node* n = node_at(s, node);
  if (!n) return TFSC_E_INVALID;
  return n->sync();
}

int tfsc_get_stats(tfsc_server* s, int node, tfsc_stats* out) {
  if (!s || !out) return fail(TFSC_E_INVALID, "get_stats: bad arguments");
  memset(out, 0, sizeof *out);
  if (node >= 0) {
    Node* n = node_at(s, node);
    if (!n) return TFSC_E_INVALID;
    n->stats(out);
  } else {
    for (auto& n : s->nodes) n->stats(out);
  }
  out->proxy_requests_rest = s->req_rest;
  out->proxy_requests_grpc = s->req_grpc;
  out->proxy_failures_rest = s->fail_rest;
  out->proxy_failures_grpc = s->fail_grpc;
  out->kernel_launches = kernel_launch_count();
  if (s->fwd) {
    const FwdStats& f = s->fwd->stats();
    out->fwd_out_requests = f.out_requests;
    out->fwd_in_requests = f.in_requests;
    out->fwd_out_failures = f.out_failures;
    out->fwd_peer_bytes_read = f.peer_bytes_read;
    out->fwd_peer_bytes_written = f.peer_bytes_written;
    out->fwd_rtt_seconds_sum = (double)f.rtt_ns_sum * 1e-9;
  }
  return 0;
}

static int check_device() {
  int n = 0;
  if (cudaGetDeviceCount(&n) != cudaSuccess || n == 0) {
    cudaGetLastError();
    return fail(TFSC_E_NO_DEVICE, "no CUDA device available: this library has no CPU fallback");
  }
  return 0;
}

int tfsc_k_affine(const float* x, float* y, int64_t n, const float* a, const float* b, void* stream) {
  if (int rc = check_device()) return rc;
  cudaError_t e = launch_affine(x, y, n, a, b, (cudaStream_t)stream);
  return e == cudaSuccess ? 0 : fail(TFSC_E_INTERNAL, "affine: %s", cudaGetErrorString(e));
}

int tfsc_k_dense(const float* x, const float* w, const float* b, float* y, int rows, int k, int n, int relu,
                 float* workspace, size_t workspace_bytes, void* stream) {
  if (int rc = check_device()) return rc;
  cudaError_t e = launch_dense(x, w, b, y, rows, k, n, relu != 0, workspace, workspace_bytes, (cudaStream_t)stream);
  return e == cudaSuccess ? 0 : fail(TFSC_E_INTERNAL, "dense: %s", cudaGetErrorString(e));
}

size_t tfsc_k_dense_workspace(int rows, int k, int n) { return dense_workspace_bytes(rows, k, n); }

int tfsc_k_dense_variant(int variant, const float* x, const float* w, const float* b, float* y, int rows, int k, int n,
                         int relu, float* workspace, size_t workspace_bytes, void* stream) {
  if (int rc = check_device()) return rc;
  if (variant < 0 || variant > 5) return fail(TFSC_E_INVALID, "dense: variant %d not in 0..5", variant);
  cudaError_t e = launch_dense(x, w, b, y, rows, k, n, relu != 0, workspace, workspace_bytes, (cudaStream_t)stream, variant);
  return e == cudaSuccess ? 0 : fail(TFSC_E_INTERNAL, "dense(variant %d): %s", variant, cudaGetErrorString(e));
}

int tfsc_k_dense_cluster_grid(int rows, int n, int* active_clusters, int* strip_cols) {
  if (int rc = check_device()) return rc;
  if (rows < 1 || rows > 8 || n < 1 || !active_clusters || !strip_cols) return fail(TFSC_E_INVALID, "dense_cluster_grid: rows in 1..8, n >= 1");
  cudaError_t e = dense_cluster_grid(rows, n, active_clusters, strip_cols);
  return e == cudaSuccess ? 0 : fail(TFSC_E_INTERNAL, "dense_cluster_grid: %s", cudaGetErrorString(e));
}

int tfsc_k_dense_tc(const float* x, const float* w, const float* b, float* y, int rows, int k, int n, int relu,
                    float* workspace, size_t workspace_bytes, void* stream) {
  if (int rc = check_device()) return rc;
  if (!dense_tc_supported(rows, k, n, w, x, b, y))
    return fail(TFSC_E_INVALID, "dense_tc: unsupported shape/alignment (rows<=64, n%%32==0, k%%4==0, 16B-aligned)");
  cudaError_t e = launch_dense_tc(x, w, b, y, rows, k, n, relu != 0, workspace, workspace_bytes, (cudaStream_t)stream);
  return e == cudaSuccess ? 0 : fail(TFSC_E_INTERNAL, "dense_tc: %s", cudaGetErrorString(e));
}

int tfsc_k_gemm(const float* a, const float* b, const float* bias, const float* r, float* c, int m, int n, int k, int lda,
                int act, void* stream) {
  if (int rc = check_device()) return rc;
  cudaError_t e = launch_gemm(a, b, bias, r, c, m, n, k, lda, act, (cudaStream_t)stream);
  return e == cudaSuccess ? 0 : fail(TFSC_E_INTERNAL, "gemm: %s", cudaGetErrorString(e));
}
int tfsc_k_gemm_tc(const float* a, const float* b, const float* bias, const float* r, float* c, int m, int n, int k, int lda,
                   int act, void* stream) {
  if (int rc = check_device()) return rc;
  if (!gemm_tc_supported(a, b, bias, r, c, m, n, k, lda))
    return fail(TFSC_E_INVALID, "gemm_tc: unsupported shape/alignment (m>=64, n>=64, n%%32==0, k>=32, lda%%4==0, 16B-aligned)");
  cudaError_t e = launch_gemm_tc(a, b, bias, r, c, m, n, k, lda, act, (cudaStream_t)stream);
  return e == cudaSuccess ? 0 : fail(TFSC_E_INTERNAL, "gemm_tc: %s", cudaGetErrorString(e));
}
int tfsc_k_conv_tc(const float* x, const float* w, const float* bias, const float* r, float* y, int batch, int h, int wd, int c,
                   int kh, int kw, int stride, int pad, int cout, int act, void* stream) {
  if (int rc = check_device()) return rc;
  const int oh = (h + 2 * pad - kh) / stride + 1, ow = (wd + 2 * pad - kw) / stride + 1;
  if (!conv_tc_supported(x, w, bias, r, y, batch, h, wd, c, kh, kw, stride, pad, oh, ow, cout))
    return fail(TFSC_E_INVALID, "conv_tc: unsupported shape/alignment (c %% 32 == 0, cout >= 64 and %% 32 == 0, batch*oh*ow >= 64, 16B-aligned)");
  cudaError_t e = launch_conv_tc(x, w, bias, r, y, batch, h, wd, c, kh, kw, stride, pad, oh, ow, cout, act, (cudaStream_t)stream);
  return e == cudaSuccess ? 0 : fail(TFSC_E_INTERNAL, "conv_tc: %s", cudaGetErrorString(e));
}
int tfsc_k_im2col(const float* x, float* col, int batch, int h, int w, int c, int kh, int kw, int stride, int pad, int ldc,
                  void* stream) {
  if (int rc = check_device()) return rc;
  const int oh = (h + 2 * pad - kh) / stride + 1, ow = (w + 2 * pad - kw) / stride + 1;
  cudaError_t e = launch_im2col(x, col, batch, h, w, c, kh, kw, stride, pad, oh, ow, ldc, (cudaStream_t)stream);
  return e == cudaSuccess ? 0 : fail(TFSC_E_INTERNAL, "im2col: %s", cudaGetErrorString(e));
}
int tfsc_k_maxpool(const float* x, float* y, int batch, int h, int w, int c, int kh, int kw, int stride, int pad, void* stream) {
  if (int rc = check_device()) return rc;
  const int oh = (h + 2 * pad - kh) / stride + 1, ow = (w + 2 * pad - kw) / stride + 1;
  cudaError_t e = launch_maxpool(x, y, batch, h, w, c, kh, kw, stride, pad, oh, ow, (cudaStream_t)stream);
  return e == cudaSuccess ? 0 : fail(TFSC_E_INTERNAL, "maxpool: %s", cudaGetErrorString(e));
}
int tfsc_k_avgpool(const float* x, float* y, int batch, int hw, int c, void* stream) {
  if (int rc = check_device()) return rc;
  cudaError_t e = launch_avgpool(x, y, batch, hw, c, (cudaStream_t)stream);
  return e == cudaSuccess ? 0 : fail(TFSC_E_INTERNAL, "avgpool: %s", cudaGetErrorString(e));
}
int tfsc_k_attention(const float* qkv, const int* ids, float* ctx, int batch, int seq, int hidden, int heads, void* stream) {
  if (int rc = check_device()) return rc;
  const bool al = ((reinterpret_cast<uintptr_t>(qkv) | reinterpret_cast<uintptr_t>(ctx)) & 15) == 0;
  if (!qkv || !ctx || batch < 1 || (int64_t)batch * heads > 65535 || !attention_supported(seq, hidden, heads, al))
    return fail(TFSC_E_INVALID, "attention: no kernel for batch %d, seq %d, hidden %d, heads %d", batch, seq, hidden, heads);
  cudaError_t e = launch_attention(qkv, ids, seq, ctx, batch, seq, hidden, heads, (cudaStream_t)stream);
  return e == cudaSuccess ? 0 : fail(TFSC_E_INTERNAL, "attention: %s", cudaGetErrorString(e));
}
int tfsc_k_attention_mask(const float* qkv, const int* mask, int mask_stride, float* ctx, int batch, int seq, int hidden, int heads,
                          void* stream) {
  if (int rc = check_device()) return rc;
  const bool al = ((reinterpret_cast<uintptr_t>(qkv) | reinterpret_cast<uintptr_t>(ctx)) & 15) == 0;
  if (!qkv || !ctx || batch < 1 || (int64_t)batch * heads > 65535 || !attention_supported(seq, hidden, heads, al))
    return fail(TFSC_E_INVALID, "attention_mask: no kernel for batch %d, seq %d, hidden %d, heads %d", batch, seq, hidden, heads);
  if (mask && mask_stride < seq) return fail(TFSC_E_INVALID, "attention_mask: mask_stride %d is below seq %d", mask_stride, seq);
  cudaError_t e = launch_attention(qkv, mask, mask_stride, ctx, batch, seq, hidden, heads, (cudaStream_t)stream);
  return e == cudaSuccess ? 0 : fail(TFSC_E_INTERNAL, "attention_mask: %s", cudaGetErrorString(e));
}
int tfsc_k_embed(const int* ids, const int* types, int stride, const float* word, const float* pos, const float* type,
                 const float* gamma, const float* beta, float* y, int batch, int seq, int hidden, int vocab, float eps, void* stream) {
  if (int rc = check_device()) return rc;
  if (!ids || !word || !pos || !type || !gamma || !beta || !y || batch < 0 || seq < 1 || vocab < 1 ||
      (int64_t)batch * seq > 0x7fffffff || !layernorm_supported(hidden))
    return fail(TFSC_E_INVALID, "embed: no kernel for batch %d, seq %d, hidden %d, vocab %d (hidden in 1..12272)", batch, seq, hidden,
                vocab);
  if (stride < seq) return fail(TFSC_E_INVALID, "embed: stride %d is below seq %d", stride, seq);
  cudaError_t e = launch_layernorm(nullptr, nullptr, ids, types, stride, word, pos, type, gamma, beta, y, batch * seq, seq, hidden,
                                   vocab, eps, (cudaStream_t)stream);
  return e == cudaSuccess ? 0 : fail(TFSC_E_INTERNAL, "embed: %s", cudaGetErrorString(e));
}
int tfsc_k_layernorm(const float* x, const float* res, const float* gamma, const float* beta, float* y, int tokens, int hidden,
                     float eps, void* stream) {
  if (int rc = check_device()) return rc;
  if (!x || !gamma || !beta || !y || tokens < 0 || !layernorm_supported(hidden))
    return fail(TFSC_E_INVALID, "layernorm: no kernel for %d tokens of hidden %d (hidden in 1..12272)", tokens, hidden);
  cudaError_t e = launch_layernorm(x, res, nullptr, nullptr, 0, nullptr, nullptr, nullptr, gamma, beta, y, tokens, 1, hidden, 0, eps,
                                   (cudaStream_t)stream);
  return e == cudaSuccess ? 0 : fail(TFSC_E_INTERNAL, "layernorm: %s", cudaGetErrorString(e));
}
int tfsc_k_classify_head(const float* logits, int rows, int n, int k, float* probs, int64_t* classes, int32_t* topk_idx,
                         float* topk_prob, void* stream) {
  if (int rc = check_device()) return rc;
  if (!logits || rows < 0 || !head_supported(n, k))
    return fail(TFSC_E_INVALID, "classify_head: no kernel for %d rows of %d logits, k = %d (1 <= n <= %d, 1 <= k <= min(n, %d))", rows,
                n, k, kHeadMaxN, kHeadMaxK);
  HeadOutputs o;
  o.probs = probs;
  o.probs_ld = n;
  o.classes = reinterpret_cast<int*>(classes);
  o.classes_ld = 2;
  o.topk_idx = topk_idx;
  o.topk_idx_ld = k;
  o.topk_prob = topk_prob;
  o.topk_prob_ld = k;
  cudaError_t e = launch_classify_head(logits, rows, n, k, o, (cudaStream_t)stream);
  return e == cudaSuccess ? 0 : fail(TFSC_E_INTERNAL, "classify_head: %s", cudaGetErrorString(e));
}
int tfsc_k_span_head(const float* logits, const int32_t* ids, const int32_t* mask, const int32_t* types, int stride, int rows, int S,
                     int max_answer_length, int k, int sep_id, float* start_logits, float* end_logits, int32_t* span_starts,
                     int32_t* span_ends, float* span_scores, void* stream) {
  if (int rc = check_device()) return rc;
  const bool spans = span_starts || span_ends || span_scores;
  if (!logits || rows < 0 || !span_supported(S, spans ? max_answer_length : 1, spans ? k : 1))
    return fail(TFSC_E_INVALID, "span_head: no kernel for %d rows of S = %d, max_answer_length = %d, k = %d (1 <= S <= %d, "
                "1 <= max_answer_length <= S, 1 <= k <= %d)", rows, S, max_answer_length, k, kSpanMaxS, kSpanMaxK);
  if (spans && (!ids || !types || stride < S))
    return fail(TFSC_E_INVALID, "span_head: spans need the ids and the segment ids, stride >= S (%d < %d)", stride, S);
  SpanInputs in;
  in.ids = ids;
  in.mask = mask;
  in.types = types;
  in.stride = stride;
  in.sep_id = sep_id < 0 ? -1 : sep_id;
  SpanOutputs o;
  o.start_logits = start_logits;
  o.start_ld = S;
  o.end_logits = end_logits;
  o.end_ld = S;
  o.starts = span_starts;
  o.starts_ld = k;
  o.ends = span_ends;
  o.ends_ld = k;
  o.scores = span_scores;
  o.scores_ld = k;
  cudaError_t e = launch_span_head(logits, in, rows, S, max_answer_length, k, o, (cudaStream_t)stream);
  return e == cudaSuccess ? 0 : fail(TFSC_E_INTERNAL, "span_head: %s", cudaGetErrorString(e));
}
int tfsc_k_encoder_head(const float* hidden, const float* pooled, const int32_t* ids, const int32_t* mask, int stride, int rows, int S,
                        int H, int normalize_cls, int normalize_mean, float* sequence_output, float* pooled_output,
                        float* cls_embedding, float* mean_embedding, void* stream) {
  if (int rc = check_device()) return rc;
  if (rows < 0 || !encoder_head_supported(S, H))
    return fail(TFSC_E_INVALID, "encoder_head: no kernel for %d rows of S = %d, H = %d (1 <= S <= %d, 1 <= H <= %d)", rows, S, H,
                kEncoderMaxS, kEncoderMaxH);
  if (!hidden && (sequence_output || cls_embedding || mean_embedding))
    return fail(TFSC_E_INVALID, "encoder_head: sequence_output, cls_embedding and mean_embedding need the hidden states");
  if (!pooled && pooled_output) return fail(TFSC_E_INVALID, "encoder_head: pooled_output needs the pooler output");
  if (mean_embedding && (!ids || stride < S))
    return fail(TFSC_E_INVALID, "encoder_head: mean_embedding needs the ids, stride >= S (%d < %d)", stride, S);
  EncoderInputs in;
  in.ids = ids;
  in.mask = mask;
  in.stride = stride;
  EncoderOutputs o;
  o.sequence = sequence_output;
  o.sequence_ld = (int64_t)S * H;
  o.pooled = pooled_output;
  o.pooled_ld = H;
  o.cls = cls_embedding;
  o.cls_ld = H;
  o.mean = mean_embedding;
  o.mean_ld = H;
  o.normalize_cls = normalize_cls != 0;
  o.normalize_mean = normalize_mean != 0;
  cudaError_t e = launch_encoder_head(hidden, pooled, in, rows, S, H, o, (cudaStream_t)stream);
  return e == cudaSuccess ? 0 : fail(TFSC_E_INTERNAL, "encoder_head: %s", cudaGetErrorString(e));
}
int tfsc_k_mask_gather(const float* hidden, const int32_t* ids, const int32_t* mask, int stride, int rows, int S, int H, int slots,
                       int mask_token_id, int32_t* positions, float* gathered, void* stream) {
  if (int rc = check_device()) return rc;
  if (rows < 0 || !mask_gather_supported(S, H, slots))
    return fail(TFSC_E_INVALID, "mask_gather: no kernel for %d rows of S = %d, H = %d, M = %d (1 <= M <= S <= %d, 1 <= H <= %d)",
                rows, S, H, slots, kMaskGatherMaxS, kMaskGatherMaxH);
  if (!ids || stride < S) return fail(TFSC_E_INVALID, "mask_gather: needs the ids, stride >= S (%d < %d)", stride, S);
  if (gathered && !hidden) return fail(TFSC_E_INVALID, "mask_gather: the gathered rows need the hidden states");
  cudaError_t e = launch_mask_gather(hidden, ids, mask, stride, rows, S, H, slots, mask_token_id, positions, gathered,
                                     (cudaStream_t)stream);
  return e == cudaSuccess ? 0 : fail(TFSC_E_INTERNAL, "mask_gather: %s", cudaGetErrorString(e));
}
int tfsc_k_fill_mask_head(const float* logits, int64_t ld, const int32_t* positions, int rows, int slots, int vocab, int k,
                          int32_t* top_ids, float* top_probs, float* top_logits, void* stream) {
  if (int rc = check_device()) return rc;
  if (rows < 0 || !fill_mask_supported(slots, vocab, k))
    return fail(TFSC_E_INVALID, "fill_mask_head: no kernel for %d rows of M = %d, vocab = %d, k = %d (1 <= M <= %d, 1 <= vocab <= %d, "
                "1 <= k <= min(vocab, %d))", rows, slots, vocab, k, kMaskGatherMaxS, kHeadMaxN, kHeadMaxK);
  if (!positions || ((top_ids || top_probs || top_logits) && (!logits || ld < vocab)))
    return fail(TFSC_E_INVALID, "fill_mask_head: needs the positions and the logits, ld >= vocab (%lld < %d)", (long long)ld, vocab);
  FillMaskOutputs o;
  o.ids = top_ids;
  o.ids_ld = (int64_t)slots * k;
  o.probs = top_probs;
  o.probs_ld = (int64_t)slots * k;
  o.logits = top_logits;
  o.logits_ld = (int64_t)slots * k;
  cudaError_t e = launch_fill_mask_head(logits, ld, positions, rows, slots, vocab, k, o, (cudaStream_t)stream);
  return e == cudaSuccess ? 0 : fail(TFSC_E_INTERNAL, "fill_mask_head: %s", cudaGetErrorString(e));
}
int tfsc_debug_gemm_trace(long long*) {
  return fail(TFSC_E_UNIMPLEMENTED, "no GEMM clock trace: the persistent GEMM kernel it timed is not part of the sm_90a build");
}

}
```

### tfservingcache_b200/csrc/tc_ptx.cuh

```cuda
#pragma once
#include <cuda.h>
#include <cuda_runtime.h>

#include <cstdint>

namespace tfsc {

__device__ __forceinline__ uint32_t smem_u32(const void* p) { return (uint32_t)__cvta_generic_to_shared(p); }
__device__ __forceinline__ void mbar_init(uint64_t* bar, uint32_t count) {
  asm volatile("mbarrier.init.shared::cta.b64 [%0], %1;" ::"r"(smem_u32(bar)), "r"(count));
}
__device__ __forceinline__ void mbar_expect_tx(uint64_t* bar, uint32_t bytes) {
  asm volatile("mbarrier.arrive.expect_tx.shared::cta.b64 _, [%0], %1;" ::"r"(smem_u32(bar)), "r"(bytes) : "memory");
}
__device__ __forceinline__ void mbar_arrive(uint64_t* bar) {
  asm volatile("mbarrier.arrive.shared::cta.b64 _, [%0];" ::"r"(smem_u32(bar)) : "memory");
}
__device__ __forceinline__ void mbar_wait(uint64_t* bar, uint32_t parity) {
  asm volatile(
      "{\n\t.reg .pred p;\n\t"
      "WAIT_%=:\n\t"
      "mbarrier.try_wait.parity.shared::cta.b64 p, [%0], %1;\n\t"
      "@p bra DONE_%=;\n\t"
      "bra WAIT_%=;\n\t"
      "DONE_%=:\n\t}" ::"r"(smem_u32(bar)),
      "r"(parity)
      : "memory");
}
__device__ __forceinline__ void tma_load_3d(void* dst, const CUtensorMap* map, uint64_t* bar, int c0, int c1, int c2) {
  asm volatile(
      "cp.async.bulk.tensor.3d.shared::cluster.global.mbarrier::complete_tx::bytes [%0], [%1, {%3, %4, %5}], [%2];" ::"r"(
          smem_u32(dst)),
      "l"(map), "r"(smem_u32(bar)), "r"(c0), "r"(c1), "r"(c2)
      : "memory");
}
__device__ __forceinline__ void tma_load_2d(void* dst, const CUtensorMap* map, uint64_t* bar, int c0, int c1) {
  asm volatile(
      "cp.async.bulk.tensor.2d.shared::cluster.global.mbarrier::complete_tx::bytes [%0], [%1, {%3, %4}], [%2];" ::"r"(
          smem_u32(dst)),
      "l"(map), "r"(smem_u32(bar)), "r"(c0), "r"(c1)
      : "memory");
}
__device__ __forceinline__ float lds_f32(uint32_t saddr) {
  float v;
  asm volatile("ld.shared.f32 %0, [%1];" : "=f"(v) : "r"(saddr));
  return v;
}
__device__ __forceinline__ float4 lds_f4(uint32_t saddr) {
  float4 v;
  asm volatile("ld.shared.v4.f32 {%0,%1,%2,%3}, [%4];" : "=f"(v.x), "=f"(v.y), "=f"(v.z), "=f"(v.w) : "r"(saddr));
  return v;
}
__device__ __forceinline__ void sts_f4(uint32_t saddr, float4 v) {
  asm volatile("st.shared.v4.f32 [%0], {%1,%2,%3,%4};" ::"r"(saddr), "f"(v.x), "f"(v.y), "f"(v.z), "f"(v.w) : "memory");
}
__device__ __forceinline__ float tf32_lo(float v) { return v - __uint_as_float(__float_as_uint(v) & 0xFFFFE000u); }
__device__ __forceinline__ uint32_t tf32_hi_bits(float v) { return __float_as_uint(v) & 0xFFFFE000u; }

__device__ __forceinline__ uint64_t gmma_desc_sw128(uint32_t saddr) {
  uint64_t d = 0;
  d |= (uint64_t)((saddr >> 4) & 0x3FFF);
  d |= (uint64_t)1 << 16;
  d |= (uint64_t)(1024 >> 4) << 32;
  d |= (uint64_t)1 << 62;
  return d;
}
__device__ __forceinline__ void wgmma_fence() { asm volatile("wgmma.fence.sync.aligned;" ::: "memory"); }
__device__ __forceinline__ void wgmma_commit() { asm volatile("wgmma.commit_group.sync.aligned;" ::: "memory"); }
__device__ __forceinline__ void wgmma_wait_all() { asm volatile("wgmma.wait_group.sync.aligned 0;" ::: "memory"); }
template <int NR>
__device__ __forceinline__ void fence_regs(float (&d)[NR]) {
#pragma unroll
  for (int i = 0; i < NR; ++i) asm volatile("" : "+f"(d[i])::"memory");
}

template <int K8>
__device__ __forceinline__ void fence_regs(uint32_t (&a)[K8][4]) {
#pragma unroll
  for (int k = 0; k < K8; ++k)
#pragma unroll
    for (int i = 0; i < 4; ++i) asm volatile("" : "+r"(a[k][i])::"memory");
}

__device__ __forceinline__ void wgmma_tf32_rs_n16(float (&d)[8], const uint32_t (&a)[4], uint64_t desc_b) {
  asm volatile(
      "{\n\t.reg .pred p;\n\tsetp.ne.b32 p, %13, 0;\n\t"
      "wgmma.mma_async.sync.aligned.m64n16k8.f32.tf32.tf32 {%0,%1,%2,%3,%4,%5,%6,%7}, {%8,%9,%10,%11}, %12, p, 1, 1;\n\t}"
      : "+f"(d[0]), "+f"(d[1]), "+f"(d[2]), "+f"(d[3]), "+f"(d[4]), "+f"(d[5]), "+f"(d[6]), "+f"(d[7])
      : "r"(a[0]), "r"(a[1]), "r"(a[2]), "r"(a[3]), "l"(desc_b), "r"(1));
}
__device__ __forceinline__ void wgmma_tf32_rs_n32(float (&d)[16], const uint32_t (&a)[4], uint64_t desc_b) {
  asm volatile(
      "{\n\t.reg .pred p;\n\tsetp.ne.b32 p, %21, 0;\n\t"
      "wgmma.mma_async.sync.aligned.m64n32k8.f32.tf32.tf32 {%0,%1,%2,%3,%4,%5,%6,%7,%8,%9,%10,%11,%12,%13,%14,%15}, {%16,%17,%18,%19}, %20, p, 1, 1;\n\t}"
      : "+f"(d[0]), "+f"(d[1]), "+f"(d[2]), "+f"(d[3]), "+f"(d[4]), "+f"(d[5]), "+f"(d[6]), "+f"(d[7]), "+f"(d[8]), "+f"(d[9]), "+f"(d[10]), "+f"(d[11]), "+f"(d[12]), "+f"(d[13]), "+f"(d[14]), "+f"(d[15])
      : "r"(a[0]), "r"(a[1]), "r"(a[2]), "r"(a[3]), "l"(desc_b), "r"(1));
}
__device__ __forceinline__ void wgmma_tf32_rs_n48(float (&d)[24], const uint32_t (&a)[4], uint64_t desc_b) {
  asm volatile(
      "{\n\t.reg .pred p;\n\tsetp.ne.b32 p, %29, 0;\n\t"
      "wgmma.mma_async.sync.aligned.m64n48k8.f32.tf32.tf32 {%0,%1,%2,%3,%4,%5,%6,%7,%8,%9,%10,%11,%12,%13,%14,%15,%16,%17,%18,%19,%20,%21,%22,%23}, {%24,%25,%26,%27}, %28, p, 1, 1;\n\t}"
      : "+f"(d[0]), "+f"(d[1]), "+f"(d[2]), "+f"(d[3]), "+f"(d[4]), "+f"(d[5]), "+f"(d[6]), "+f"(d[7]), "+f"(d[8]), "+f"(d[9]), "+f"(d[10]), "+f"(d[11]), "+f"(d[12]), "+f"(d[13]), "+f"(d[14]), "+f"(d[15]), "+f"(d[16]), "+f"(d[17]), "+f"(d[18]), "+f"(d[19]), "+f"(d[20]), "+f"(d[21]), "+f"(d[22]), "+f"(d[23])
      : "r"(a[0]), "r"(a[1]), "r"(a[2]), "r"(a[3]), "l"(desc_b), "r"(1));
}
__device__ __forceinline__ void wgmma_tf32_rs_n64(float (&d)[32], const uint32_t (&a)[4], uint64_t desc_b) {
  asm volatile(
      "{\n\t.reg .pred p;\n\tsetp.ne.b32 p, %37, 0;\n\t"
      "wgmma.mma_async.sync.aligned.m64n64k8.f32.tf32.tf32 {%0,%1,%2,%3,%4,%5,%6,%7,%8,%9,%10,%11,%12,%13,%14,%15,%16,%17,%18,%19,%20,%21,%22,%23,%24,%25,%26,%27,%28,%29,%30,%31}, {%32,%33,%34,%35}, %36, p, 1, 1;\n\t}"
      : "+f"(d[0]), "+f"(d[1]), "+f"(d[2]), "+f"(d[3]), "+f"(d[4]), "+f"(d[5]), "+f"(d[6]), "+f"(d[7]), "+f"(d[8]), "+f"(d[9]), "+f"(d[10]), "+f"(d[11]), "+f"(d[12]), "+f"(d[13]), "+f"(d[14]), "+f"(d[15]), "+f"(d[16]), "+f"(d[17]), "+f"(d[18]), "+f"(d[19]), "+f"(d[20]), "+f"(d[21]), "+f"(d[22]), "+f"(d[23]), "+f"(d[24]), "+f"(d[25]), "+f"(d[26]), "+f"(d[27]), "+f"(d[28]), "+f"(d[29]), "+f"(d[30]), "+f"(d[31])
      : "r"(a[0]), "r"(a[1]), "r"(a[2]), "r"(a[3]), "l"(desc_b), "r"(1));
}
__device__ __forceinline__ void wgmma_tf32_rs_n128(float (&d)[64], const uint32_t (&a)[4], uint64_t desc_b) {
  asm volatile(
      "{\n\t.reg .pred p;\n\tsetp.ne.b32 p, %69, 0;\n\t"
      "wgmma.mma_async.sync.aligned.m64n128k8.f32.tf32.tf32 {%0,%1,%2,%3,%4,%5,%6,%7,%8,%9,%10,%11,%12,%13,%14,%15,%16,%17,%18,%19,%20,%21,%22,%23,%24,%25,%26,%27,%28,%29,%30,%31,%32,%33,%34,%35,%36,%37,%38,%39,%40,%41,%42,%43,%44,%45,%46,%47,%48,%49,%50,%51,%52,%53,%54,%55,%56,%57,%58,%59,%60,%61,%62,%63}, {%64,%65,%66,%67}, %68, p, 1, 1;\n\t}"
      : "+f"(d[0]), "+f"(d[1]), "+f"(d[2]), "+f"(d[3]), "+f"(d[4]), "+f"(d[5]), "+f"(d[6]), "+f"(d[7]), "+f"(d[8]), "+f"(d[9]), "+f"(d[10]), "+f"(d[11]), "+f"(d[12]), "+f"(d[13]), "+f"(d[14]), "+f"(d[15]), "+f"(d[16]), "+f"(d[17]), "+f"(d[18]), "+f"(d[19]), "+f"(d[20]), "+f"(d[21]), "+f"(d[22]), "+f"(d[23]), "+f"(d[24]), "+f"(d[25]), "+f"(d[26]), "+f"(d[27]), "+f"(d[28]), "+f"(d[29]), "+f"(d[30]), "+f"(d[31]), "+f"(d[32]), "+f"(d[33]), "+f"(d[34]), "+f"(d[35]), "+f"(d[36]), "+f"(d[37]), "+f"(d[38]), "+f"(d[39]), "+f"(d[40]), "+f"(d[41]), "+f"(d[42]), "+f"(d[43]), "+f"(d[44]), "+f"(d[45]), "+f"(d[46]), "+f"(d[47]), "+f"(d[48]), "+f"(d[49]), "+f"(d[50]), "+f"(d[51]), "+f"(d[52]), "+f"(d[53]), "+f"(d[54]), "+f"(d[55]), "+f"(d[56]), "+f"(d[57]), "+f"(d[58]), "+f"(d[59]), "+f"(d[60]), "+f"(d[61]), "+f"(d[62]), "+f"(d[63])
      : "r"(a[0]), "r"(a[1]), "r"(a[2]), "r"(a[3]), "l"(desc_b), "r"(1));
}

template <int N>
__device__ __forceinline__ void wgmma_tf32_rs(float (&d)[N / 2], const uint32_t (&a)[4], uint64_t desc_b) {
  if constexpr (N == 16) wgmma_tf32_rs_n16(d, a, desc_b);
  else if constexpr (N == 32) wgmma_tf32_rs_n32(d, a, desc_b);
  else if constexpr (N == 48) wgmma_tf32_rs_n48(d, a, desc_b);
  else if constexpr (N == 64) wgmma_tf32_rs_n64(d, a, desc_b);
  else {
    static_assert(N == 128, "wgmma_tf32_rs: N in {16, 32, 48, 64, 128}");
    wgmma_tf32_rs_n128(d, a, desc_b);
  }
}
template <int N>
__device__ __forceinline__ void regs_release() { asm volatile("setmaxnreg.dec.sync.aligned.u32 %0;" ::"n"(N)); }
template <int N>
__device__ __forceinline__ void regs_acquire() { asm volatile("setmaxnreg.inc.sync.aligned.u32 %0;" ::"n"(N)); }
__device__ __forceinline__ void named_bar_sync(int id, int threads) {
  asm volatile("bar.sync %0, %1;" ::"r"(id), "r"(threads) : "memory");
}

typedef CUresult (*EncodeTiledFn)(CUtensorMap*, CUtensorMapDataType, cuuint32_t, void*, const cuuint64_t*,
                                  const cuuint64_t*, const cuuint32_t*, const cuuint32_t*, CUtensorMapInterleave,
                                  CUtensorMapSwizzle, CUtensorMapL2promotion, CUtensorMapFloatOOBfill);
EncodeTiledFn tc_encode_fn();

}
```

Baseline: 37840.

## Add stream-K persistent TF32 wgmma kernel with TMA x loads and larger row tiles

Adds a new dense TF32 tensor-core kernel. It spreads k-block work units evenly across CTAs in stream-K fashion, loads activations through a TMA tensor map with a separate warp computing the tf32 low parts, and keeps one wgmma group in flight. It also supports up to 128 rows per pass. The old kernel is kept as tc17 for small row counts, and the caller now splits rows into passes of at most 128. The aim is better SM load balance, fewer passes for large batches and overlap of fragment loads with MMA. The cost is much more complex fold/counter logic and heavier register pressure.

New measurement: 39180 (median of 6 runs). 3.6% higher.

```diff
diff --git a/tfservingcache_b200/csrc/dense_tc.cu b/tfservingcache_b200/csrc/dense_tc.cu
--- a/tfservingcache_b200/csrc/dense_tc.cu
+++ b/tfservingcache_b200/csrc/dense_tc.cu
@@ -15,6 +15,275 @@
 std::atomic<int64_t> g_launches_tc{0};
 
 namespace tc {
+constexpr int BK = 32;
+constexpr int WG_COLS = 64;
+constexpr int CONS_WG = 2;
+constexpr int STRIP = WG_COLS * CONS_WG;
+constexpr int SLABS = STRIP / 32;
+constexpr int KG_BYTES = SLABS * 512;
+constexpr int W_BYTES = (BK / 4) * KG_BYTES;
+constexpr int MAX_RP = 128;
+constexpr int CHAIN = 96;
+constexpr int MAX_FOLDS = 8;
+constexpr int MAX_SEGS = 8;
+constexpr int CONSUMERS = CONS_WG * 128;
+constexpr int CONS_WARPS = CONSUMERS / 32;
+constexpr int THREADS = CONSUMERS + 128;
+constexpr int LO_THREADS = 64;
+constexpr int PRODUCER_REGS = 56, CONSUMER_REGS = 224;
+constexpr int SMEM_MAX = 232448;
+}
+
+template <int RP>
+struct TcSmem {
+  static constexpr int B_BYTES = 2 * RP * 128;
+  static constexpr int NSB = RP <= 64 ? 4 : 3;
+  static constexpr int FREE = tc::SMEM_MAX - 1024 - 256 - 64 - NSB * B_BYTES;
+  static constexpr int NSW = FREE / tc::W_BYTES > 10 ? 10 : FREE / tc::W_BYTES;
+  static constexpr int W_TOTAL = NSW * tc::W_BYTES;
+  static constexpr int TOTAL = W_TOTAL + NSB * B_BYTES + 256 + 1024;
+  static_assert(RP % 16 == 0 && RP <= tc::MAX_RP, "RP: a multiple of 16 up to 128");
+  static_assert((2 * NSW + 3 * NSB) * 8 <= 256, "mbarriers");
+};
+
+__host__ __device__ __forceinline__ int tc_unit_begin(int c, int units, int ctas) { return (int)((long long)c * units / ctas); }
+__host__ __device__ __forceinline__ int tc_unit_owner(int u, int units, int ctas) {
+  return (int)(((long long)(u + 1) * ctas - 1) / units);
+}
+
+__host__ __device__ __forceinline__ int tc_segment_end(int u, int u1, int kbps) {
+  const int strip_end = (u / kbps + 1) * kbps, e = u + tc::CHAIN;
+  return min(u1, min(strip_end, e));
+}
+
+__device__ __noinline__ void tc_fold(int strip, int pt, int rows, int N, int relu, int kbps, int units, int ctas, int maxseg,
+                                     const float* __restrict__ bias, float* __restrict__ y, const float* __restrict__ partials) {
+  const int c_first = tc_unit_owner(strip * kbps, units, ctas), c_last = tc_unit_owner(strip * kbps + kbps - 1, units, ctas);
+  constexpr size_t SLOT = (size_t)tc::MAX_RP * tc::STRIP;
+  __threadfence();
+  for (int idx = pt; idx < rows * (tc::STRIP / 4); idx += 128) {
+    const int r = idx / (tc::STRIP / 4), c4 = idx - r * (tc::STRIP / 4);
+    const int col = strip * tc::STRIP + c4 * 4;
+    if (col >= N) continue;
+    const float* p = partials + (size_t)r * tc::STRIP + c4 * 4;
+    float4 acc = make_float4(0.f, 0.f, 0.f, 0.f);
+    bool first = true;
+    for (int c = c_first; c <= c_last; ++c) {
+      const int u1 = tc_unit_begin(c + 1, units, ctas);
+      for (int u = tc_unit_begin(c, units, ctas), j = 0; u < u1 && u < (strip + 1) * kbps; u = tc_segment_end(u, u1, kbps), ++j) {
+        if (u < strip * kbps) continue;
+        const float4 v = __ldcg(reinterpret_cast<const float4*>(p + (size_t)(c * maxseg + j) * SLOT));
+        if (first) acc = v;
+        else { acc.x += v.x; acc.y += v.y; acc.z += v.z; acc.w += v.w; }
+        first = false;
+      }
+    }
+    const float4 bv = __ldg(reinterpret_cast<const float4*>(bias + col));
+    acc.x += bv.x; acc.y += bv.y; acc.z += bv.z; acc.w += bv.w;
+    if (relu) { acc.x = fmaxf(acc.x, 0.f); acc.y = fmaxf(acc.y, 0.f); acc.z = fmaxf(acc.z, 0.f); acc.w = fmaxf(acc.w, 0.f); }
+    *reinterpret_cast<float4*>(y + (size_t)r * N + col) = acc;
+  }
+}
+
+template <int RP>
+__global__ void __launch_bounds__(tc::THREADS, 1)
+dense_tc_kernel(const __grid_constant__ CUtensorMap wmap, const __grid_constant__ CUtensorMap xmap,
+                const float* __restrict__ bias, float* __restrict__ y, int rows, int N, int relu, int kbps, int units,
+                int maxseg, unsigned int* __restrict__ counters, float* __restrict__ partials) {
+  using S = TcSmem<RP>;
+  constexpr int NSW = S::NSW, NSB = S::NSB;
+  extern __shared__ __align__(1024) uint8_t smem_raw[];
+  __shared__ int s_fold[tc::MAX_FOLDS];
+  __shared__ int s_nfold;
+  uint8_t* smem = reinterpret_cast<uint8_t*>((reinterpret_cast<uintptr_t>(smem_raw) + 1023) & ~(uintptr_t)1023);
+  uint8_t* bprime = smem + S::W_TOTAL;
+  uint64_t* bars = reinterpret_cast<uint64_t*>(bprime + NSB * S::B_BYTES);
+  uint64_t* wfull = bars;
+  uint64_t* wempty = wfull + NSW;
+  uint64_t* xfull = wempty + NSW;
+  uint64_t* xready = xfull + NSB;
+  uint64_t* xempty = xready + NSB;
+
+  const int warp = threadIdx.x >> 5, lane = threadIdx.x & 31;
+  const int wg = __shfl_sync(0xffffffffu, (int)(threadIdx.x >> 7), 0);
+  const int ctas = (int)gridDim.x, cta = (int)blockIdx.x;
+  const int u0 = tc_unit_begin(cta, units, ctas), nq = tc_unit_begin(cta + 1, units, ctas) - u0;
+
+  if (threadIdx.x == 0) {
+    for (int s = 0; s < NSW; ++s) {
+      mbar_init(&wfull[s], 1);
+      mbar_init(&wempty[s], tc::CONS_WARPS);
+    }
+    for (int s = 0; s < NSB; ++s) {
+      mbar_init(&xfull[s], 1);
+      mbar_init(&xready[s], tc::LO_THREADS);
+      mbar_init(&xempty[s], tc::CONS_WARPS);
+    }
+    asm volatile("fence.mbarrier_init.release.cluster;" ::: "memory");
+    asm volatile("prefetch.tensormap [%0];" ::"l"(&wmap) : "memory");
+    asm volatile("prefetch.tensormap [%0];" ::"l"(&xmap) : "memory");
+    s_nfold = 0;
+  }
+  __syncthreads();
+  asm volatile("griddepcontrol.launch_dependents;" ::: "memory");
+
+  if (wg == tc::CONS_WG) {
+    regs_release<tc::PRODUCER_REGS>();
+    if (warp == tc::CONS_WARPS) {
+      if (lane == 0)
+        for (int q = 0; q < nq; ++q) {
+          const int s = q % NSW, u = u0 + q, strip = u / kbps, kb = u - strip * kbps;
+          if (q >= NSW) mbar_wait(&wempty[s], (q / NSW - 1) & 1);
+          mbar_expect_tx(&wfull[s], tc::W_BYTES);
+#pragma unroll
+          for (int g = 0; g < tc::BK / 4; ++g)
+            tma_load_3d(smem + s * tc::W_BYTES + g * tc::KG_BYTES, &wmap, &wfull[s], 0, kb * tc::BK + g * 4, strip * tc::SLABS);
+        }
+    } else if (warp == tc::CONS_WARPS + 1) {
+      asm volatile("griddepcontrol.wait;" ::: "memory");
+      if (lane == 0)
+        for (int q = 0; q < nq; ++q) {
+          const int s = q % NSB, kb = (u0 + q) % kbps;
+          if (q >= NSB) mbar_wait(&xempty[s], (q / NSB - 1) & 1);
+          mbar_expect_tx(&xfull[s], RP * 128);
+          tma_load_2d(bprime + s * S::B_BYTES, &xmap, &xfull[s], kb * tc::BK, 0);
+        }
+    } else {
+      const int lt = threadIdx.x - (tc::CONSUMERS + 64);
+      const uint32_t bp_base = smem_u32(bprime);
+      for (int q = 0; q < nq; ++q) {
+        const int s = q % NSB;
+        mbar_wait(&xfull[s], (q / NSB) & 1);
+        const uint32_t bp = bp_base + (uint32_t)(s * S::B_BYTES);
+#pragma unroll 4
+        for (int i = lt; i < RP * 8; i += tc::LO_THREADS) {
+          const float4 v = lds_f4(bp + (uint32_t)(i * 16));
+          sts_f4(bp + (uint32_t)(RP * 128 + i * 16), make_float4(tf32_lo(v.x), tf32_lo(v.y), tf32_lo(v.z), tf32_lo(v.w)));
+        }
+        asm volatile("fence.proxy.async.shared::cta;" ::: "memory");
+        mbar_arrive(&xready[s]);
+      }
+    }
+    named_bar_sync(2, tc::THREADS);
+    for (int f = 0; f < s_nfold; ++f)
+      tc_fold(s_fold[f], threadIdx.x - tc::CONSUMERS, rows, N, relu, kbps, units, ctas, maxseg, bias, y, partials);
+  } else {
+    regs_acquire<tc::CONSUMER_REGS>();
+    asm volatile("griddepcontrol.wait;" ::: "memory");
+    const int ct = threadIdx.x;
+    const int wq = warp & 3, g = lane >> 2, t = lane & 3;
+    const int n0 = wg * tc::WG_COLS + wq * 16 + g, row = (n0 >> 5) * 4 + t;
+    auto w_off = [&](int n) { return (uint32_t)(row * 128 + ((((n & 31) >> 2) ^ (row & 7)) << 4) + (n & 3) * 4); };
+    const uint32_t w_base = smem_u32(smem), bp_base = smem_u32(bprime);
+    const uint32_t off0 = w_off(n0), off1 = w_off(n0 + 8);
+    float acc_h[RP / 2], acc_s[RP / 2];
+#pragma unroll
+    for (int i = 0; i < RP / 2; ++i) acc_h[i] = acc_s[i] = 0.f;
+
+    auto load_frags = [&](int q, uint32_t (&hi)[tc::BK / 8][4], uint32_t (&lo)[tc::BK / 8][4]) {
+      const int s = q % NSW;
+      mbar_wait(&wfull[s], (q / NSW) & 1);
+      const uint32_t wst = w_base + (uint32_t)(s * tc::W_BYTES);
+#pragma unroll
+      for (int k8 = 0; k8 < tc::BK / 8; ++k8)
+#pragma unroll
+        for (int j = 0; j < 4; ++j) {
+          const float v = lds_f32(wst + (uint32_t)((k8 * 2 + (j >> 1)) * tc::KG_BYTES) + ((j & 1) ? off1 : off0));
+          hi[k8][j] = tf32_hi_bits(v);
+          lo[k8][j] = __float_as_uint(tf32_lo(v));
+        }
+      __syncwarp();
+      if (lane == 0) mbar_arrive(&wempty[s]);
+    };
+
+    int seg_begin = 0, seg_end = tc_segment_end(u0, u0 + nq, kbps) - u0, strip = u0 / kbps, seg = 0, pending = -1;
+    auto write_partial = [&]() {
+      float* my_partial = partials + (size_t)(cta * maxseg + seg) * tc::MAX_RP * tc::STRIP;
+#pragma unroll
+      for (int i = 0; i < RP / 2; ++i) {
+        const int ncol = n0 + 8 * ((i >> 1) & 1), r = 8 * (i >> 2) + 2 * t + (i & 1);
+        if (r < rows) my_partial[(size_t)r * tc::STRIP + ncol] = acc_h[i] + acc_s[i];
+      }
+    };
+    auto release_x = [&](int q) {
+      __syncwarp();
+      if (lane == 0) mbar_arrive(&xempty[q % NSB]);
+    };
+    auto finish_segment = [&]() {
+      const int len = seg_end - seg_begin;
+      if (len == kbps) {
+#pragma unroll
+        for (int i = 0; i < RP / 2; ++i) {
+          const int col = strip * tc::STRIP + n0 + 8 * ((i >> 1) & 1), r = 8 * (i >> 2) + 2 * t + (i & 1);
+          if (r < rows && col < N) {
+            float v = acc_h[i] + acc_s[i] + __ldg(bias + col);
+            if (relu) v = fmaxf(v, 0.f);
+            y[(size_t)r * N + col] = v;
+          }
+        }
+      } else {
+        write_partial();
+        __threadfence();
+        named_bar_sync(1, tc::CONSUMERS);
+        if (ct == 0 && atomicAdd(&counters[strip], (unsigned)len) + (unsigned)len == (unsigned)kbps) {
+          counters[strip] = 0u;
+          s_fold[s_nfold++] = strip;
+        }
+      }
+#pragma unroll
+      for (int i = 0; i < RP / 2; ++i) acc_h[i] = acc_s[i] = 0.f;
+      seg_begin = seg_end;
+      seg_end = tc_segment_end(u0 + seg_begin, u0 + nq, kbps) - u0;
+      strip = (u0 + seg_begin) / kbps;
+      ++seg;
+    };
+
+    auto step = [&](int q, uint32_t (&hi)[tc::BK / 8][4], uint32_t (&lo)[tc::BK / 8][4], uint32_t (&nhi)[tc::BK / 8][4],
+                    uint32_t (&nlo)[tc::BK / 8][4]) {
+      const int sb = q % NSB;
+      mbar_wait(&xready[sb], (q / NSB) & 1);
+      const uint32_t bp = bp_base + (uint32_t)(sb * S::B_BYTES);
+      fence_regs(hi);
+      fence_regs(lo);
+      fence_regs(acc_h);
+      fence_regs(acc_s);
+      wgmma_fence();
+#pragma unroll
+      for (int k8 = 0; k8 < tc::BK / 8; ++k8) {
+        const uint64_t bh = gmma_desc_sw128(bp + k8 * 32), bl = gmma_desc_sw128(bp + RP * 128 + k8 * 32);
+        wgmma_tf32_rs<RP>(acc_h, hi[k8], bh);
+        wgmma_tf32_rs<RP>(acc_s, hi[k8], bl);
+        wgmma_tf32_rs<RP>(acc_s, lo[k8], bh);
+      }
+      wgmma_commit();
+      wgmma_wait_one();
+      fence_regs(acc_h);
+      fence_regs(acc_s);
+      if (pending >= 0) release_x(pending);
+      pending = q;
+      if (q + 1 < nq) load_frags(q + 1, nhi, nlo);
+      if (q + 1 == seg_end) {
+        wgmma_wait_all();
+        fence_regs(acc_h);
+        fence_regs(acc_s);
+        release_x(q);
+        pending = -1;
+        finish_segment();
+      }
+    };
+
+    uint32_t hi0[tc::BK / 8][4], lo0[tc::BK / 8][4], hi1[tc::BK / 8][4], lo1[tc::BK / 8][4];
+    load_frags(0, hi0, lo0);
+    for (int q = 0; q < nq; q += 2) {
+      step(q, hi0, lo0, hi1, lo1);
+      if (q + 1 < nq) step(q + 1, hi1, lo1, hi0, lo0);
+    }
+    asm volatile("bar.arrive 2, %0;" ::"n"(tc::THREADS) : "memory");
+  }
+
+}
+
+namespace tc17 {
 constexpr int BK = 32;
 constexpr int WG_COLS = 64;
 constexpr int CONS_WG = 4;
@@ -27,19 +296,19 @@
 }
 
 template <int RP>
-struct TcSmem {
+struct Tc17Smem {
   static constexpr int NS = 6;
   static constexpr int B_BYTES = 2 * RP * 128;
-  static constexpr int W_TOTAL = NS * tc::W_BYTES;
+  static constexpr int W_TOTAL = NS * tc17::W_BYTES;
   static constexpr int TOTAL = W_TOTAL + 2 * B_BYTES + 256 + 1024;
 };
 
 template <int RP>
-__global__ void __launch_bounds__(tc::THREADS, 1)
-dense_tc_kernel(const __grid_constant__ CUtensorMap wmap, const float* __restrict__ x, const float* __restrict__ bias,
+__global__ void __launch_bounds__(tc17::THREADS, 1)
+dense_tc17_kernel(const __grid_constant__ CUtensorMap wmap, const float* __restrict__ x, const float* __restrict__ bias,
                 float* __restrict__ y, int rows, int K, int N, int relu, int splits, int chunk_k,
                 unsigned int* __restrict__ counters, float* __restrict__ partials) {
-  using S = TcSmem<RP>;
+  using S = Tc17Smem<RP>;
   constexpr int NS = S::NS;
   extern __shared__ __align__(1024) uint8_t smem_raw[];
   uint8_t* smem = reinterpret_cast<uint8_t*>((reinterpret_cast<uintptr_t>(smem_raw) + 1023) & ~(uintptr_t)1023);
@@ -53,12 +322,12 @@
   const int strip = blockIdx.x, split = blockIdx.y;
   const int k_begin = split * chunk_k;
   const int k_end = min(K, k_begin + chunk_k);
-  const int n_kblocks = (max(0, k_end - k_begin) + tc::BK - 1) / tc::BK;
+  const int n_kblocks = (max(0, k_end - k_begin) + tc17::BK - 1) / tc17::BK;
 
   if (threadIdx.x == 0) {
     for (int s = 0; s < NS; ++s) {
       mbar_init(&full[s], 1);
-      mbar_init(&empty[s], tc::CONS_WARPS);
+      mbar_init(&empty[s], tc17::CONS_WARPS);
     }
     asm volatile("fence.mbarrier_init.release.cluster;" ::: "memory");
     asm volatile("prefetch.tensormap [%0];" ::"l"(&wmap) : "memory");
@@ -66,28 +335,28 @@
   __syncthreads();
   asm volatile("griddepcontrol.launch_dependents;" ::: "memory");
 
-  if (wg == tc::CONS_WG) {
+  if (wg == tc17::CONS_WG) {
     for (int kb = 0; kb < n_kblocks; ++kb) {
       const int s = kb % NS, it = kb / NS;
       if (lane == 0) {
         if (it > 0) mbar_wait(&empty[s], (it - 1) & 1);
-        mbar_expect_tx(&full[s], tc::W_BYTES);
-#pragma unroll
-        for (int g = 0; g < tc::BK / 4; ++g)
-          tma_load_3d(smem + s * tc::W_BYTES + g * 4096, &wmap, &full[s], 0, k_begin + kb * tc::BK + g * 4, strip * tc::SLABS);
+        mbar_expect_tx(&full[s], tc17::W_BYTES);
+#pragma unroll
+        for (int g = 0; g < tc17::BK / 4; ++g)
+          tma_load_3d(smem + s * tc17::W_BYTES + g * 4096, &wmap, &full[s], 0, k_begin + kb * tc17::BK + g * 4, strip * tc17::SLABS);
       }
       __syncwarp();
     }
   } else {
     const int ct = threadIdx.x;
     const int wq = warp & 3, g = lane >> 2, t = lane & 3;
-    constexpr int XI = (RP * 8 + tc::CONSUMERS - 1) / tc::CONSUMERS;
+    constexpr int XI = (RP * 8 + tc17::CONSUMERS - 1) / tc17::CONSUMERS;
     float4 xr[2][XI];
     auto load_x = [&](int kb, float4* dst) {
-      const int k0 = k_begin + kb * tc::BK;
+      const int k0 = k_begin + kb * tc17::BK;
 #pragma unroll
       for (int j = 0; j < XI; ++j) {
-        const int idx = ct + j * tc::CONSUMERS;
+        const int idx = ct + j * tc17::CONSUMERS;
         const int r = idx >> 3, c = idx & 7;
         float4 v = make_float4(0.f, 0.f, 0.f, 0.f);
         const int kk = k0 + c * 4;
@@ -106,7 +375,7 @@
     asm volatile("griddepcontrol.wait;" ::: "memory");
     if (n_kblocks > 0) load_x(0, xr[0]);
     if (n_kblocks > 1) load_x(1, xr[1]);
-    const int n0 = wg * tc::WG_COLS + wq * 16 + g, slab = n0 >> 5, row = slab * 4 + t;
+    const int n0 = wg * tc17::WG_COLS + wq * 16 + g, slab = n0 >> 5, row = slab * 4 + t;
     auto w_off = [&](int n) { return (uint32_t)(row * 128 + ((((n & 31) >> 2) ^ (row & 7)) << 4) + (n & 3) * 4); };
     const uint32_t w_base = smem_u32(smem);
     const uint32_t off0 = w_off(n0), off1 = w_off(n0 + 8);
@@ -119,7 +388,7 @@
       const uint32_t bp = bp_base + cb * S::B_BYTES;
 #pragma unroll
       for (int j = 0; j < XI; ++j) {
-        const int idx = ct + j * tc::CONSUMERS;
+        const int idx = ct + j * tc17::CONSUMERS;
         if (idx < RP * 8) {
           const int r = idx >> 3, c = idx & 7, rl = r + RP;
           const float4 v = xcur[j];
@@ -130,12 +399,12 @@
       }
       if (kb + 2 < n_kblocks) load_x(kb + 2, xcur);
       asm volatile("fence.proxy.async.shared::cta;" ::: "memory");
-      named_bar_sync(1, tc::CONSUMERS);
+      named_bar_sync(1, tc17::CONSUMERS);
       mbar_wait(&full[s], it & 1);
-      const uint32_t wst = w_base + (uint32_t)(s * tc::W_BYTES);
-      uint32_t hi[tc::BK / 8][4], lo[tc::BK / 8][4];
-#pragma unroll
-      for (int k8 = 0; k8 < tc::BK / 8; ++k8)
+      const uint32_t wst = w_base + (uint32_t)(s * tc17::W_BYTES);
+      uint32_t hi[tc17::BK / 8][4], lo[tc17::BK / 8][4];
+#pragma unroll
+      for (int k8 = 0; k8 < tc17::BK / 8; ++k8)
 #pragma unroll
         for (int j = 0; j < 4; ++j) {
           const float v = lds_f32(wst + (uint32_t)((k8 * 2 + (j >> 1)) * 4096) + ((j & 1) ? off1 : off0));
@@ -152,7 +421,7 @@
       fence_regs(acc_s);
       wgmma_fence();
 #pragma unroll
-      for (int k8 = 0; k8 < tc::BK / 8; ++k8) {
+      for (int k8 = 0; k8 < tc17::BK / 8; ++k8) {
         const uint64_t bh = gmma_desc_sw128(bp + k8 * 32), bl = gmma_desc_sw128(bp + RP * 128 + k8 * 32);
         wgmma_tf32_rs<RP>(acc_h, hi[k8], bh);
         wgmma_tf32_rs<RP>(acc_s, hi[k8], bl);
@@ -167,11 +436,11 @@
       body(kb, xr[0]);
       if (kb + 1 < n_kblocks) body(kb + 1, xr[1]);
     }
-    float* my_partial = partials + ((size_t)(strip * splits + split) * RP) * tc::STRIP;
+    float* my_partial = partials + ((size_t)(strip * splits + split) * RP) * tc17::STRIP;
 #pragma unroll
     for (int i = 0; i < RP / 2; ++i) {
       const int ncol = n0 + 8 * ((i >> 1) & 1), r = 8 * (i >> 2) + 2 * t + (i & 1);
-      my_partial[(size_t)r * tc::STRIP + ncol] = acc_h[i] + acc_s[i];
+      my_partial[(size_t)r * tc17::STRIP + ncol] = acc_h[i] + acc_s[i];
     }
   }
 
@@ -187,14 +456,14 @@
   __syncthreads();
   if (!s_last) return;
   __threadfence();
-  const float* sp = partials + (size_t)strip * splits * RP * tc::STRIP;
-  for (int idx = threadIdx.x; idx < rows * (tc::STRIP / 4); idx += tc::THREADS) {
-    const int r = idx / (tc::STRIP / 4), c4 = idx - r * (tc::STRIP / 4);
-    const int col = strip * tc::STRIP + c4 * 4;
+  const float* sp = partials + (size_t)strip * splits * RP * tc17::STRIP;
+  for (int idx = threadIdx.x; idx < rows * (tc17::STRIP / 4); idx += tc17::THREADS) {
+    const int r = idx / (tc17::STRIP / 4), c4 = idx - r * (tc17::STRIP / 4);
+    const int col = strip * tc17::STRIP + c4 * 4;
     if (col >= N) continue;
-    float4 acc = __ldcg(reinterpret_cast<const float4*>(sp + (size_t)r * tc::STRIP) + c4);
+    float4 acc = __ldcg(reinterpret_cast<const float4*>(sp + (size_t)r * tc17::STRIP) + c4);
     for (int s2 = 1; s2 < splits; ++s2) {
-      const float4 v = __ldcg(reinterpret_cast<const float4*>(sp + ((size_t)s2 * RP + r) * tc::STRIP) + c4);
+      const float4 v = __ldcg(reinterpret_cast<const float4*>(sp + ((size_t)s2 * RP + r) * tc17::STRIP) + c4);
       acc.x += v.x; acc.y += v.y; acc.z += v.z; acc.w += v.w;
     }
     const float4 bv = __ldg(reinterpret_cast<const float4*>(bias + col));
@@ -203,6 +472,7 @@
     *reinterpret_cast<float4*>(y + (size_t)r * N + col) = acc;
   }
 }
+
 
 EncodeTiledFn tc_encode_fn() {
   static EncodeTiledFn fn = [] {
@@ -216,18 +486,18 @@
 
 struct MapKey {
   const void* w;
-  int k, n;
-  bool operator==(const MapKey& o) const { return w == o.w && k == o.k && n == o.n; }
+  int k, n, slabs;
+  bool operator==(const MapKey& o) const { return w == o.w && k == o.k && n == o.n && slabs == o.slabs; }
 };
 struct MapKeyHash {
-  size_t operator()(const MapKey& m) const { return std::hash<const void*>()(m.w) ^ ((size_t)m.k * 1315423911u) ^ ((size_t)m.n << 20); }
+  size_t operator()(const MapKey& m) const { return std::hash<const void*>()(m.w) ^ ((size_t)m.k * 1315423911u) ^ ((size_t)m.n << 20) ^ ((size_t)m.slabs << 40); }
 };
 
-static bool get_wmap(const float* w, int k, int n, CUtensorMap* out) {
+static bool get_wmap(const float* w, int k, int n, int slabs, CUtensorMap* out) {
   static std::mutex mu;
   static std::unordered_map<MapKey, CUtensorMap, MapKeyHash> cache;
   std::lock_guard<std::mutex> lk(mu);
-  auto it = cache.find({w, k, n});
+  auto it = cache.find({w, k, n, slabs});
   if (it != cache.end()) {
     *out = it->second;
     return true;
@@ -237,50 +507,139 @@
   CUtensorMap m;
   const cuuint64_t gdim[3] = {32, (cuuint64_t)k, (cuuint64_t)(n / 32)};
   const cuuint64_t gstride[2] = {(cuuint64_t)n * 4, 128};
-  const cuuint32_t box[3] = {32, 4, (cuuint32_t)tc::SLABS};
+  const cuuint32_t box[3] = {32, 4, (cuuint32_t)slabs};
   const cuuint32_t estr[3] = {1, 1, 1};
   CUresult r = enc(&m, CU_TENSOR_MAP_DATA_TYPE_FLOAT32, 3, const_cast<float*>(w), gdim, gstride, box, estr,
                    CU_TENSOR_MAP_INTERLEAVE_NONE, CU_TENSOR_MAP_SWIZZLE_128B, CU_TENSOR_MAP_L2_PROMOTION_L2_256B,
                    CU_TENSOR_MAP_FLOAT_OOB_FILL_NONE);
   if (r != CUDA_SUCCESS) return false;
   if (cache.size() > 4096) cache.clear();
-  cache[{w, k, n}] = m;
+  cache[{w, k, n, slabs}] = m;
   *out = m;
   return true;
 }
 
+static bool get_xmap(const float* x, int rows, int k, int rp, CUtensorMap* out) {
+  EncodeTiledFn enc = tc_encode_fn();
+  if (!enc) return false;
+  const cuuint64_t gdim[2] = {(cuuint64_t)k, (cuuint64_t)rows};
+  const cuuint64_t gstride[1] = {(cuuint64_t)k * 4};
+  const cuuint32_t box[2] = {(cuuint32_t)tc::BK, (cuuint32_t)rp};
+  const cuuint32_t estr[2] = {1, 1};
+  return enc(out, CU_TENSOR_MAP_DATA_TYPE_FLOAT32, 2, const_cast<float*>(x), gdim, gstride, box, estr, CU_TENSOR_MAP_INTERLEAVE_NONE,
+             CU_TENSOR_MAP_SWIZZLE_128B, CU_TENSOR_MAP_L2_PROMOTION_L2_128B, CU_TENSOR_MAP_FLOAT_OOB_FILL_NONE) == CUDA_SUCCESS;
+}
+
 struct TcPlan {
-  int strips, splits, chunk_k;
+  int strips, kbps, units, ctas;
+  int maxseg, maxstrips;
 };
 static TcPlan plan_tc(int k, int n) {
   TcPlan p;
   p.strips = (n + tc::STRIP - 1) / tc::STRIP;
+  p.kbps = (k + tc::BK - 1) / tc::BK;
+  const long long units = (long long)p.strips * p.kbps;
+  p.units = units > (1LL << 30) ? (1 << 30) : (int)units;
+  const int sms = device_sm_count();
+  p.ctas = p.units < sms ? p.units : sms;
+  p.maxseg = p.maxstrips = 0;
+  for (int c = 0; c < p.ctas; ++c) {
+    const int u0 = tc_unit_begin(c, p.units, p.ctas), u1 = tc_unit_begin(c + 1, p.units, p.ctas);
+    int segs = 0;
+    for (int u = u0; u < u1 && segs <= tc::MAX_SEGS; u = tc_segment_end(u, u1, p.kbps)) ++segs;
+    const int strips = (u1 - 1) / p.kbps - u0 / p.kbps + 1;
+    if (segs > p.maxseg) p.maxseg = segs;
+    if (strips > p.maxstrips) p.maxstrips = strips;
+  }
+  return p;
+}
+
+static bool tc_plan_fits(int k, int n) {
+  if (k < 1 || n < 1) return false;
+  const TcPlan p = plan_tc(k, n);
+  return p.maxseg <= tc::MAX_SEGS && p.maxstrips <= tc::MAX_FOLDS;
+}
+
+bool dense_tc_supported(int rows, int k, int n, const float* w, const float* x, const float* bias, const float* y) {
+  return rows >= 1 && rows <= tc::MAX_RP && n % 32 == 0 && k % 4 == 0 && k >= 32 &&
+         (long long)((n + tc::STRIP - 1) / tc::STRIP) * ((k + tc::BK - 1) / tc::BK) < (1LL << 30) && tc_plan_fits(k, n) &&
+         ((reinterpret_cast<uintptr_t>(w) & 15) == 0) && ((reinterpret_cast<uintptr_t>(x) & 15) == 0) &&
+         ((reinterpret_cast<uintptr_t>(bias) & 15) == 0) && ((reinterpret_cast<uintptr_t>(y) & 15) == 0) && tc_encode_fn() != nullptr;
+}
+
+static size_t tc17_workspace_bytes(int k, int n);
+static size_t tc_counter_bytes(int n) { return ((size_t)((n + tc::STRIP - 1) / tc::STRIP) * sizeof(unsigned int) + 255) & ~(size_t)255; }
+
+size_t dense_tc_workspace_bytes(int k, int n) {
+  if (!tc_plan_fits(k, n)) return 0;
+  TcPlan p = plan_tc(k, n);
+  size_t counters = tc_counter_bytes(n);
+  const size_t ws = counters + (size_t)p.ctas * p.maxseg * tc::MAX_RP * tc::STRIP * sizeof(float);
+  const size_t ws17 = tc17_workspace_bytes(k, n);
+  return ws > ws17 ? ws : ws17;
+}
+
+struct Tc17Plan {
+  int strips, splits, chunk_k;
+};
+static Tc17Plan plan_tc17(int k, int n) {
+  Tc17Plan p;
+  p.strips = (n + tc17::STRIP - 1) / tc17::STRIP;
   int splits = device_sm_count() / p.strips;
   if (splits < 1) splits = 1;
-  int max_splits = (k + 4 * tc::BK - 1) / (4 * tc::BK);
+  int max_splits = (k + 4 * tc17::BK - 1) / (4 * tc17::BK);
   if (splits > max_splits) splits = max_splits;
   if (splits < 1) splits = 1;
   int chunk = (k + splits - 1) / splits;
-  chunk = (chunk + tc::BK - 1) / tc::BK * tc::BK;
+  chunk = (chunk + tc17::BK - 1) / tc17::BK * tc17::BK;
   p.chunk_k = chunk;
   p.splits = (k + chunk - 1) / chunk;
   return p;
 }
 
-bool dense_tc_supported(int rows, int k, int n, const float* w, const float* x, const float* bias, const float* y) {
-  return rows >= 1 && rows <= 64 && n % 32 == 0 && k % 4 == 0 && k >= 32 &&
-         ((reinterpret_cast<uintptr_t>(w) & 15) == 0) && ((reinterpret_cast<uintptr_t>(x) & 15) == 0) &&
-         ((reinterpret_cast<uintptr_t>(bias) & 15) == 0) && ((reinterpret_cast<uintptr_t>(y) & 15) == 0) && tc_encode_fn() != nullptr;
-}
-
-size_t dense_tc_workspace_bytes(int k, int n) {
-  TcPlan p = plan_tc(k, n);
-  size_t counters = ((size_t)p.strips * sizeof(unsigned int) + 255) & ~(size_t)255;
-  return counters + (size_t)p.strips * p.splits * 64 * tc::STRIP * sizeof(float);
-}
+static size_t tc17_workspace_bytes(int k, int n) {
+  Tc17Plan p = plan_tc17(k, n);
+  size_t counters = tc_counter_bytes(n);
+  return counters + (size_t)p.strips * p.splits * 64 * tc17::STRIP * sizeof(float);
+}
+
 
 template <int RP>
-static cudaError_t launch_tc_rp(const CUtensorMap& map, const float* x, const float* bias, float* y, int rows, int k, int n,
+static cudaError_t launch_tc17_rp(const CUtensorMap& map, const float* x, const float* bias, float* y, int rows, int k, int n,
+                                bool relu, void* workspace, const Tc17Plan& p, cudaStream_t s) {
+  static bool attr[64] = {};
+  int dev = 0;
+  cudaGetDevice(&dev);
+  if (!attr[dev & 63]) {
+    cudaError_t e = cudaFuncSetAttribute(dense_tc17_kernel<RP>, cudaFuncAttributeMaxDynamicSharedMemorySize, Tc17Smem<RP>::TOTAL);
+    if (e != cudaSuccess) return e;
+    attr[dev & 63] = true;
+  }
+  unsigned int* counters = static_cast<unsigned int*>(workspace);
+  size_t coff = tc_counter_bytes(n);
+  float* partials = reinterpret_cast<float*>(static_cast<char*>(workspace) + coff);
+  static const bool pdl = [] {
+    const char* e = getenv("TFSC_PDL");
+    return !e || atoi(e) != 0;
+  }();
+  cudaLaunchConfig_t cfg = {};
+  cfg.gridDim = dim3(p.strips, p.splits);
+  cfg.blockDim = dim3(tc17::THREADS);
+  cfg.dynamicSmemBytes = Tc17Smem<RP>::TOTAL;
+  cfg.stream = s;
+  cudaLaunchAttribute at[1];
+  at[0].id = cudaLaunchAttributeProgrammaticStreamSerialization;
+  at[0].val.programmaticStreamSerializationAllowed = 1;
+  cfg.attrs = at;
+  cfg.numAttrs = pdl ? 1 : 0;
+  cudaError_t e = cudaLaunchKernelEx(&cfg, dense_tc17_kernel<RP>, map, x, bias, y, rows, k, n, relu ? 1 : 0, p.splits, p.chunk_k, counters,
+                                     partials);
+  g_launches_tc++;
+  return e != cudaSuccess ? e : cudaGetLastError();
+}
+
+template <int RP>
+static cudaError_t launch_tc_rp(const CUtensorMap& wmap, const float* x, const float* bias, float* y, int rows, int k, int n,
                                 bool relu, void* workspace, const TcPlan& p, cudaStream_t s) {
   static bool attr[64] = {};
   int dev = 0;
@@ -290,15 +649,17 @@
     if (e != cudaSuccess) return e;
     attr[dev & 63] = true;
   }
+  CUtensorMap xmap;
+  if (!get_xmap(x, rows, k, RP, &xmap)) return cudaErrorNotSupported;
   unsigned int* counters = static_cast<unsigned int*>(workspace);
-  size_t coff = ((size_t)p.strips * sizeof(unsigned int) + 255) & ~(size_t)255;
+  size_t coff = tc_counter_bytes(n);
   float* partials = reinterpret_cast<float*>(static_cast<char*>(workspace) + coff);
   static const bool pdl = [] {
     const char* e = getenv("TFSC_PDL");
     return !e || atoi(e) != 0;
   }();
   cudaLaunchConfig_t cfg = {};
-  cfg.gridDim = dim3(p.strips, p.splits);
+  cfg.gridDim = dim3(p.ctas);
   cfg.blockDim = dim3(tc::THREADS);
   cfg.dynamicSmemBytes = TcSmem<RP>::TOTAL;
   cfg.stream = s;
@@ -307,8 +668,8 @@
   at[0].val.programmaticStreamSerializationAllowed = 1;
   cfg.attrs = at;
   cfg.numAttrs = pdl ? 1 : 0;
-  cudaError_t e = cudaLaunchKernelEx(&cfg, dense_tc_kernel<RP>, map, x, bias, y, rows, k, n, relu ? 1 : 0, p.splits, p.chunk_k, counters,
-                                     partials);
+  cudaError_t e = cudaLaunchKernelEx(&cfg, dense_tc_kernel<RP>, wmap, xmap, bias, y, rows, n, relu ? 1 : 0, p.kbps, p.units, p.maxseg,
+                                     counters, partials);
   g_launches_tc++;
   return e != cudaSuccess ? e : cudaGetLastError();
 }
@@ -317,12 +678,22 @@
                             void* workspace, size_t workspace_bytes, cudaStream_t s) {
   if (workspace_bytes < dense_tc_workspace_bytes(k, n)) return cudaErrorInvalidValue;
   CUtensorMap map;
-  if (!get_wmap(w, k, n, &map)) return cudaErrorNotSupported;
+  if (rows <= 64) {
+    if (!get_wmap(w, k, n, tc17::SLABS, &map)) return cudaErrorNotSupported;
+    const Tc17Plan p17 = plan_tc17(k, n);
+    if (rows <= 16) return launch_tc17_rp<16>(map, x, bias, y, rows, k, n, relu, workspace, p17, s);
+    if (rows <= 32) return launch_tc17_rp<32>(map, x, bias, y, rows, k, n, relu, workspace, p17, s);
+    if (rows <= 48) return launch_tc17_rp<48>(map, x, bias, y, rows, k, n, relu, workspace, p17, s);
+    return launch_tc17_rp<64>(map, x, bias, y, rows, k, n, relu, workspace, p17, s);
+  }
+  if (!get_wmap(w, k, n, tc::SLABS, &map)) return cudaErrorNotSupported;
   const TcPlan p = plan_tc(k, n);
-  if (rows <= 16) return launch_tc_rp<16>(map, x, bias, y, rows, k, n, relu, workspace, p, s);
-  if (rows <= 32) return launch_tc_rp<32>(map, x, bias, y, rows, k, n, relu, workspace, p, s);
-  if (rows <= 48) return launch_tc_rp<48>(map, x, bias, y, rows, k, n, relu, workspace, p, s);
-  return launch_tc_rp<64>(map, x, bias, y, rows, k, n, relu, workspace, p, s);
-}
-
-}
+  switch ((rows + 15) / 16) {
+    case 5: return launch_tc_rp<80>(map, x, bias, y, rows, k, n, relu, workspace, p, s);
+    case 6: return launch_tc_rp<96>(map, x, bias, y, rows, k, n, relu, workspace, p, s);
+    case 7: return launch_tc_rp<112>(map, x, bias, y, rows, k, n, relu, workspace, p, s);
+    default: return launch_tc_rp<128>(map, x, bias, y, rows, k, n, relu, workspace, p, s);
+  }
+}
+
+}
diff --git a/tfservingcache_b200/csrc/kernels.cu b/tfservingcache_b200/csrc/kernels.cu
--- a/tfservingcache_b200/csrc/kernels.cu
+++ b/tfservingcache_b200/csrc/kernels.cu
@@ -593,9 +593,10 @@
   const DensePlan p = plan_dense(k, n);
   int r_done = 0;
   const int tc_rows = variant == 3 ? 1 : tc_min_rows();
-  if (variant != 1 && tc_rows > 0 && rows >= tc_rows && dense_tc_supported(rows > 64 ? 64 : rows, k, n, w, x, bias, y)) {
-    while (rows - r_done >= tc_rows) {
-      const int rr = rows - r_done < 64 ? rows - r_done : 64;
+  if (variant != 1 && tc_rows > 0 && rows >= tc_rows && dense_tc_supported(rows > 128 ? 128 : rows, k, n, w, x, bias, y)) {
+    const int passes = (rows + 127) / 128;
+    for (int i = 0; i < passes; ++i) {
+      const int rr = rows / passes + (i < rows % passes ? 1 : 0);
       cudaError_t e = launch_dense_tc(x + (size_t)r_done * k, w, bias, y + (size_t)r_done * n, rr, k, n, relu, workspace,
                                       workspace_bytes, s);
       if (e != cudaSuccess) return e;
diff --git a/tfservingcache_b200/csrc/server.cu b/tfservingcache_b200/csrc/server.cu
--- a/tfservingcache_b200/csrc/server.cu
+++ b/tfservingcache_b200/csrc/server.cu
@@ -1682,7 +1682,7 @@
                     float* workspace, size_t workspace_bytes, void* stream) {
   if (int rc = check_device()) return rc;
   if (!dense_tc_supported(rows, k, n, w, x, b, y))
-    return fail(TFSC_E_INVALID, "dense_tc: unsupported shape/alignment (rows<=64, n%%32==0, k%%4==0, 16B-aligned)");
+    return fail(TFSC_E_INVALID, "dense_tc: unsupported shape/alignment (rows<=128, n%%32==0, k%%4==0, 16B-aligned)");
   cudaError_t e = launch_dense_tc(x, w, b, y, rows, k, n, relu != 0, workspace, workspace_bytes, (cudaStream_t)stream);
   return e == cudaSuccess ? 0 : fail(TFSC_E_INTERNAL, "dense_tc: %s", cudaGetErrorString(e));
 }
diff --git a/tfservingcache_b200/csrc/tc_ptx.cuh b/tfservingcache_b200/csrc/tc_ptx.cuh
--- a/tfservingcache_b200/csrc/tc_ptx.cuh
+++ b/tfservingcache_b200/csrc/tc_ptx.cuh
@@ -68,6 +68,7 @@
 __device__ __forceinline__ void wgmma_fence() { asm volatile("wgmma.fence.sync.aligned;" ::: "memory"); }
 __device__ __forceinline__ void wgmma_commit() { asm volatile("wgmma.commit_group.sync.aligned;" ::: "memory"); }
 __device__ __forceinline__ void wgmma_wait_all() { asm volatile("wgmma.wait_group.sync.aligned 0;" ::: "memory"); }
+__device__ __forceinline__ void wgmma_wait_one() { asm volatile("wgmma.wait_group.sync.aligned 1;" ::: "memory"); }
 template <int NR>
 __device__ __forceinline__ void fence_regs(float (&d)[NR]) {
 #pragma unroll
@@ -110,6 +111,27 @@
       : "+f"(d[0]), "+f"(d[1]), "+f"(d[2]), "+f"(d[3]), "+f"(d[4]), "+f"(d[5]), "+f"(d[6]), "+f"(d[7]), "+f"(d[8]), "+f"(d[9]), "+f"(d[10]), "+f"(d[11]), "+f"(d[12]), "+f"(d[13]), "+f"(d[14]), "+f"(d[15]), "+f"(d[16]), "+f"(d[17]), "+f"(d[18]), "+f"(d[19]), "+f"(d[20]), "+f"(d[21]), "+f"(d[22]), "+f"(d[23]), "+f"(d[24]), "+f"(d[25]), "+f"(d[26]), "+f"(d[27]), "+f"(d[28]), "+f"(d[29]), "+f"(d[30]), "+f"(d[31])
       : "r"(a[0]), "r"(a[1]), "r"(a[2]), "r"(a[3]), "l"(desc_b), "r"(1));
 }
+__device__ __forceinline__ void wgmma_tf32_rs_n80(float (&d)[40], const uint32_t (&a)[4], uint64_t desc_b) {
+  asm volatile(
+      "{\n\t.reg .pred p;\n\tsetp.ne.b32 p, %45, 0;\n\t"
+      "wgmma.mma_async.sync.aligned.m64n80k8.f32.tf32.tf32 {%0,%1,%2,%3,%4,%5,%6,%7,%8,%9,%10,%11,%12,%13,%14,%15,%16,%17,%18,%19,%20,%21,%22,%23,%24,%25,%26,%27,%28,%29,%30,%31,%32,%33,%34,%35,%36,%37,%38,%39}, {%40,%41,%42,%43}, %44, p, 1, 1;\n\t}"
+      : "+f"(d[0]), "+f"(d[1]), "+f"(d[2]), "+f"(d[3]), "+f"(d[4]), "+f"(d[5]), "+f"(d[6]), "+f"(d[7]), "+f"(d[8]), "+f"(d[9]), "+f"(d[10]), "+f"(d[11]), "+f"(d[12]), "+f"(d[13]), "+f"(d[14]), "+f"(d[15]), "+f"(d[16]), "+f"(d[17]), "+f"(d[18]), "+f"(d[19]), "+f"(d[20]), "+f"(d[21]), "+f"(d[22]), "+f"(d[23]), "+f"(d[24]), "+f"(d[25]), "+f"(d[26]), "+f"(d[27]), "+f"(d[28]), "+f"(d[29]), "+f"(d[30]), "+f"(d[31]), "+f"(d[32]), "+f"(d[33]), "+f"(d[34]), "+f"(d[35]), "+f"(d[36]), "+f"(d[37]), "+f"(d[38]), "+f"(d[39])
+      : "r"(a[0]), "r"(a[1]), "r"(a[2]), "r"(a[3]), "l"(desc_b), "r"(1));
+}
+__device__ __forceinline__ void wgmma_tf32_rs_n96(float (&d)[48], const uint32_t (&a)[4], uint64_t desc_b) {
+  asm volatile(
+      "{\n\t.reg .pred p;\n\tsetp.ne.b32 p, %53, 0;\n\t"
+      "wgmma.mma_async.sync.aligned.m64n96k8.f32.tf32.tf32 {%0,%1,%2,%3,%4,%5,%6,%7,%8,%9,%10,%11,%12,%13,%14,%15,%16,%17,%18,%19,%20,%21,%22,%23,%24,%25,%26,%27,%28,%29,%30,%31,%32,%33,%34,%35,%36,%37,%38,%39,%40,%41,%42,%43,%44,%45,%46,%47}, {%48,%49,%50,%51}, %52, p, 1, 1;\n\t}"
+      : "+f"(d[0]), "+f"(d[1]), "+f"(d[2]), "+f"(d[3]), "+f"(d[4]), "+f"(d[5]), "+f"(d[6]), "+f"(d[7]), "+f"(d[8]), "+f"(d[9]), "+f"(d[10]), "+f"(d[11]), "+f"(d[12]), "+f"(d[13]), "+f"(d[14]), "+f"(d[15]), "+f"(d[16]), "+f"(d[17]), "+f"(d[18]), "+f"(d[19]), "+f"(d[20]), "+f"(d[21]), "+f"(d[22]), "+f"(d[23]), "+f"(d[24]), "+f"(d[25]), "+f"(d[26]), "+f"(d[27]), "+f"(d[28]), "+f"(d[29]), "+f"(d[30]), "+f"(d[31]), "+f"(d[32]), "+f"(d[33]), "+f"(d[34]), "+f"(d[35]), "+f"(d[36]), "+f"(d[37]), "+f"(d[38]), "+f"(d[39]), "+f"(d[40]), "+f"(d[41]), "+f"(d[42]), "+f"(d[43]), "+f"(d[44]), "+f"(d[45]), "+f"(d[46]), "+f"(d[47])
+      : "r"(a[0]), "r"(a[1]), "r"(a[2]), "r"(a[3]), "l"(desc_b), "r"(1));
+}
+__device__ __forceinline__ void wgmma_tf32_rs_n112(float (&d)[56], const uint32_t (&a)[4], uint64_t desc_b) {
+  asm volatile(
+      "{\n\t.reg .pred p;\n\tsetp.ne.b32 p, %61, 0;\n\t"
+      "wgmma.mma_async.sync.aligned.m64n112k8.f32.tf32.tf32 {%0,%1,%2,%3,%4,%5,%6,%7,%8,%9,%10,%11,%12,%13,%14,%15,%16,%17,%18,%19,%20,%21,%22,%23,%24,%25,%26,%27,%28,%29,%30,%31,%32,%33,%34,%35,%36,%37,%38,%39,%40,%41,%42,%43,%44,%45,%46,%47,%48,%49,%50,%51,%52,%53,%54,%55}, {%56,%57,%58,%59}, %60, p, 1, 1;\n\t}"
+      : "+f"(d[0]), "+f"(d[1]), "+f"(d[2]), "+f"(d[3]), "+f"(d[4]), "+f"(d[5]), "+f"(d[6]), "+f"(d[7]), "+f"(d[8]), "+f"(d[9]), "+f"(d[10]), "+f"(d[11]), "+f"(d[12]), "+f"(d[13]), "+f"(d[14]), "+f"(d[15]), "+f"(d[16]), "+f"(d[17]), "+f"(d[18]), "+f"(d[19]), "+f"(d[20]), "+f"(d[21]), "+f"(d[22]), "+f"(d[23]), "+f"(d[24]), "+f"(d[25]), "+f"(d[26]), "+f"(d[27]), "+f"(d[28]), "+f"(d[29]), "+f"(d[30]), "+f"(d[31]), "+f"(d[32]), "+f"(d[33]), "+f"(d[34]), "+f"(d[35]), "+f"(d[36]), "+f"(d[37]), "+f"(d[38]), "+f"(d[39]), "+f"(d[40]), "+f"(d[41]), "+f"(d[42]), "+f"(d[43]), "+f"(d[44]), "+f"(d[45]), "+f"(d[46]), "+f"(d[47]), "+f"(d[48]), "+f"(d[49]), "+f"(d[50]), "+f"(d[51]), "+f"(d[52]), "+f"(d[53]), "+f"(d[54]), "+f"(d[55])
+      : "r"(a[0]), "r"(a[1]), "r"(a[2]), "r"(a[3]), "l"(desc_b), "r"(1));
+}
 __device__ __forceinline__ void wgmma_tf32_rs_n128(float (&d)[64], const uint32_t (&a)[4], uint64_t desc_b) {
   asm volatile(
       "{\n\t.reg .pred p;\n\tsetp.ne.b32 p, %69, 0;\n\t"
@@ -124,8 +146,11 @@
   else if constexpr (N == 32) wgmma_tf32_rs_n32(d, a, desc_b);
   else if constexpr (N == 48) wgmma_tf32_rs_n48(d, a, desc_b);
   else if constexpr (N == 64) wgmma_tf32_rs_n64(d, a, desc_b);
+  else if constexpr (N == 80) wgmma_tf32_rs_n80(d, a, desc_b);
+  else if constexpr (N == 96) wgmma_tf32_rs_n96(d, a, desc_b);
+  else if constexpr (N == 112) wgmma_tf32_rs_n112(d, a, desc_b);
   else {
-    static_assert(N == 128, "wgmma_tf32_rs: N in {16, 32, 48, 64, 128}");
+    static_assert(N == 128, "wgmma_tf32_rs: N in {16, 32, ..., 128} (multiples of 16)");
     wgmma_tf32_rs_n128(d, a, desc_b);
   }
 }
```
